# zwyang6/ExCEL

Measured on AMD Instinct MI355X. Metric: images/sec (CAM+PAR refine, 448x448), higher is better.
Workload: dtype bf16x3 (fp32 as bf16 hi+lo, fp32 accumulate)

## Files before the change

excel_amd/_lib.py:

```python
import ctypes as C
import os

_HERE = os.path.dirname(os.path.abspath(__file__))
LIB_PATH = os.path.join(_HERE, "csrc", "libexcel_hip.so")

c_f = C.c_void_p
c_i = C.c_int
c_ll = C.c_longlong
c_sz = C.c_size_t


class VitConfig(C.Structure):
    _fields_ = [("width", c_i), ("layers", c_i), ("heads", c_i), ("patch", c_i), ("out_dim", c_i),
                ("n_surgery", c_i), ("pos_grid", c_i)]


class VitBlockWeights(C.Structure):
    _fields_ = [(n, C.c_void_p) for n in (
        "ln1_w", "ln1_b", "in_proj_w", "in_proj_b", "out_proj_w", "out_proj_b",
        "ln2_w", "ln2_b", "fc1_w", "fc1_b", "fc2_w", "fc2_b")]


class VitWeights(C.Structure):
    _fields_ = [(n, C.c_void_p) for n in (
        "conv1_w", "class_emb", "pos_emb", "ln_pre_w", "ln_pre_b", "ln_post_w", "ln_post_b", "proj")] + \
        [("blocks", C.POINTER(VitBlockWeights))]


class DecoderConfig(C.Structure):
    _fields_ = [(n, c_i) for n in ("vit_layers", "vit_width", "embed", "dec_layers", "heads", "num_classes")]


class FuseLayerWeights(C.Structure):
    _fields_ = [(n, C.c_void_p) for n in ("proj_w", "proj_b", "proj2_w", "proj2_b")]


class DecoderBlockWeights(C.Structure):
    _fields_ = VitBlockWeights._fields_


class DecoderWeights(C.Structure):
    _fields_ = [("fuse", C.POINTER(FuseLayerWeights)), ("fuse_w", C.c_void_p), ("fuse_b", C.c_void_p),
                ("blocks", C.POINTER(DecoderBlockWeights)), ("pred_w", C.c_void_p), ("pred_b", C.c_void_p)]


class TextConfig(C.Structure):
    _fields_ = [(n, c_i) for n in ("vocab_size", "context_length", "width", "layers", "heads", "embed_dim")]


class TextWeights(C.Structure):
    _fields_ = [(n, C.c_void_p) for n in ("token_embedding", "positional_embedding", "ln_final_w", "ln_final_b", "text_projection")] + \
        [("blocks", C.POINTER(DecoderBlockWeights))]


class RaggedInfo(C.Structure):
    _fields_ = [("B", C.c_int32), ("total_tiles", C.c_int32), ("total_pix", C.c_int64), ("total_label_pix", C.c_int64),
                ("max_plane_pix", C.c_int64), ("table_ints", C.c_int64)]


class AugParams(C.Structure):
    _fields_ = [("ratio", C.c_double), ("flip", C.c_int32), ("h_pad", C.c_int32), ("w_pad", C.c_int32),
                ("cand_h", C.c_int32 * 10), ("cand_w", C.c_int32 * 10)]


class TrainAugInfo(C.Structure):
    _fields_ = [("B", C.c_int32), ("S", C.c_int32), ("max_h", C.c_int32), ("max_w2", C.c_int32), ("table_ints", C.c_int64),
                ("workspace_bytes", C.c_int64), ("total_label_pix", C.c_int64)]


SIGNATURES = {
    "excel_last_error": (C.c_char_p, []),
    "excel_abi_version": (c_i, []),
    "excel_build_id": (C.c_char_p, []),
    "excel_gemm_f32": (c_i, [c_f, c_f, c_f, c_f, c_f, c_i, c_i, c_i, c_i, c_i, c_i, c_i, c_i, c_i, c_i,
                             c_ll, c_ll, c_ll, c_ll, c_f]),
    "excel_split_bf16": (c_i, [c_f, c_f, c_ll, c_i, c_f]),
    "excel_gemm_bf16x3": (c_i, [c_f, c_f, c_f, c_f, c_f, c_i, c_i, c_i, c_i, c_i, c_f]),
    "excel_split_f16": (c_i, [c_f, c_f, c_ll, c_i, c_f]),
    "excel_gemm_f16x3": (c_i, [c_f, c_f, c_f, c_f, c_f, c_i, c_i, c_i, c_i, c_i, c_f]),
    "excel_pack_f16": (c_i, [c_f, c_f, c_ll, c_i, c_f, c_f]),
    "excel_gemm_f16x2": (c_i, [c_f, c_f, c_f, c_f, c_f, c_f, c_i, c_i, c_i, c_i, c_i, c_f]),
    "excel_gemm_plan": (c_i, [c_i, c_i, c_i, c_i, c_i, c_i, c_i, c_i, c_i, C.POINTER(C.c_int32)]),
    "excel_attn_plan": (c_i, [c_i, c_i, c_i, c_i, c_i, c_i, C.POINTER(C.c_int32)]),
    "excel_layernorm": (c_i, [c_f, c_f, c_f, c_f, c_i, c_i, C.c_float, c_f]),
    "excel_vit_create": (c_i, [C.POINTER(VitConfig), C.POINTER(VitWeights), C.POINTER(C.c_void_p)]),
    "excel_vit_destroy": (None, [C.c_void_p]),
    "excel_vit_workspace_bytes": (c_sz, [C.c_void_p, c_i, c_i]),
    "excel_vit_set_gemm_mode": (c_i, [C.c_void_p, c_i]),
    "excel_vit_get_gemm_mode": (c_i, [C.c_void_p]),
    "excel_vit_weights_fp16_exact": (c_i, [C.c_void_p]),
    "excel_vit_forward": (c_i, [C.c_void_p, c_f, c_i, c_i, c_f, c_sz, c_f, c_f, c_f, c_i, c_f, c_i, c_f, c_f]),
    "excel_vit_forward_ex": (c_i, [C.c_void_p, c_f, c_i, c_i, c_f, c_sz, c_f, c_f, c_f, c_i, c_f, c_i, c_f, c_f, c_i, c_f]),
    "excel_feature_affinity_workspace_bytes": (c_sz, [c_i, c_i, c_i]),
    "excel_feature_affinity": (c_i, [c_f, c_i, c_i, c_i, C.c_float, C.c_float, c_i, c_f, c_f, c_f]),
    "excel_feature_affinity_grouped_workspace_bytes": (c_sz, [c_i, c_i, c_i, c_i]),
    "excel_feature_affinity_grouped": (c_i, [c_f, c_i, c_i, c_i, c_i, c_i, C.c_float, C.c_float, c_i, c_f, c_f, c_f]),
    "excel_attn_select_workspace_bytes": (c_sz, [c_i, c_i]),
    "excel_attn_select_mean": (c_i, [c_f, c_i, c_i, c_i, c_i, c_i, c_f, c_f, c_f, c_f]),
    "excel_decoder_create": (c_i, [C.POINTER(DecoderConfig), C.POINTER(DecoderWeights), C.POINTER(C.c_void_p)]),
    "excel_decoder_destroy": (None, [C.c_void_p]),
    "excel_decoder_workspace_bytes": (c_sz, [C.c_void_p, c_i, c_i]),
    "excel_decoder_forward": (c_i, [C.c_void_p, c_f, c_i, c_i, c_f, c_sz, c_f, c_f, c_f]),
    "excel_text_create": (c_i, [C.POINTER(TextConfig), C.POINTER(TextWeights), C.POINTER(C.c_void_p)]),
    "excel_text_destroy": (None, [C.c_void_p]),
    "excel_text_workspace_bytes": (c_sz, [C.c_void_p, c_i]),
    "excel_text_encode": (c_i, [C.c_void_p, c_f, c_i, c_f, c_f, c_sz, c_f]),
    "excel_prompt_ensemble": (c_i, [c_f, c_i, c_i, c_f, c_f]),
    "excel_decoder_train_workspace_bytes": (c_sz, [C.c_void_p, c_i, c_i]),
    "excel_decoder_forward_train": (c_i, [C.c_void_p, c_f, c_i, c_i, c_f, c_sz, c_f, c_f, C.c_float, C.c_uint, c_f]),
    "excel_decoder_train_attn_fts": (c_i, [C.c_void_p, c_i, c_i, c_f, c_sz, c_f, c_f]),
    "excel_decoder_backward": (c_i, [C.c_void_p, c_f, c_i, c_i, c_f, c_sz, c_f, c_f, C.POINTER(DecoderWeights), C.c_float, C.c_uint, c_f]),
    "excel_adamw_step": (c_i, [c_f, c_f, c_f, c_f, c_ll, C.c_float, C.c_float, C.c_float, C.c_float, C.c_float, c_i, c_f]),
    "excel_train_losses_workspace_bytes": (c_sz, [c_i, c_i, c_i, c_i]),
    "excel_train_losses": (c_i, [c_f, c_f, c_f, c_f, c_i, c_i, c_i, c_i, c_i, c_i, c_i, c_i, C.c_float, C.c_float, c_f, c_f, c_f, c_f, c_f]),
    "excel_lam_to_label": (c_i, [c_f, c_f, c_f, c_i, c_i, c_i, c_i, C.c_float, C.c_float, C.c_float, c_i, c_i, c_f, c_f, c_f]),
    "excel_normalize_img_u8": (c_i, [c_f, c_i, c_i, c_i, C.POINTER(C.c_double), C.POINTER(C.c_double), c_f, c_f]),
    "excel_denormalize_img": (c_i, [c_f, c_i, c_i, c_i, C.POINTER(C.c_float), C.POINTER(C.c_float), c_f, c_f, c_f]),
    "excel_seg_scale_accumulate": (c_i, [c_f, c_f, c_i, c_i, c_i, c_i, c_i, c_i, c_i, c_i, C.c_float, c_f]),
    "excel_cam_workspace_bytes": (c_sz, [c_i, c_i, c_i]),
    "excel_patch_text_cam_workspace_bytes": (c_sz, [c_i, c_i, c_i, c_i]),
    "excel_patch_text_cam": (c_i, [c_f, c_f, c_i, c_i, c_i, c_i, c_i, C.c_float, c_i, c_f, c_f, c_f, c_f, c_f]),
    "excel_clip_feature_surgery": (c_i, [c_f, c_f, c_i, c_i, c_i, c_i, c_i, C.c_float, c_f, c_f, c_f, c_f]),
    "excel_dcrf_workspace_bytes": (c_sz, [c_i, c_i, c_i]),
    "excel_dcrf_inference": (c_i, [c_f, c_f, c_i, c_i, c_i, c_i, c_i, C.c_float, C.c_float, C.c_float, C.c_float, C.c_float, c_f, c_f, c_f]),
    "excel_dcrf_ragged_workspace_bytes": (c_i, [c_ll, c_i, C.POINTER(c_sz)]),
    "excel_dcrf_inference_ragged": (c_i, [c_f, c_f, c_i, c_f, C.POINTER(RaggedInfo), c_i, c_i, C.c_float, C.c_float, C.c_float, C.c_float, C.c_float,
                                          c_f, c_f, c_f, c_f]),
    "excel_dcrf_lam_ragged_workspace_bytes": (c_i, [C.POINTER(C.c_int32), C.POINTER(C.c_int32), c_i, C.POINTER(c_sz)]),
    "excel_dcrf_lam_ragged": (c_i, [c_f, c_f, c_f, C.POINTER(C.c_int32), c_f, c_f, C.POINTER(RaggedInfo), c_i, c_i, c_i, C.c_float, C.c_float,
                                    C.c_float, C.c_float, C.c_float, c_f, c_f, c_f, c_f]),
    "excel_attn_layer_mean": (c_i, [c_f, c_i, c_i, c_i, c_i, c_i, c_f, c_f]),
    "excel_trans_mat_workspace_bytes": (c_sz, [c_i, c_i]),
    "excel_compute_trans_mat": (c_i, [c_f, c_i, c_i, c_f, c_f, c_f]),
    "excel_cls_compact": (c_i, [c_f, c_i, c_i, c_i, c_f, c_f, c_f, c_f]),
    "excel_scoremap_box_mask": (c_i, [c_f, c_f, c_f, c_i, c_i, c_i, c_i, C.c_double, c_f, c_f, c_f]),
    "excel_refine_workspace_bytes": (c_sz, [c_i, c_i, c_i]),
    "excel_refine_cams_with_aff": (c_i, [c_f, c_f, c_f, c_f, c_i, c_i, c_i, c_i, C.c_double, c_f, c_f, c_f]),
    "excel_cam_upsample_bkg": (c_i, [c_f, c_f, c_i, c_i, c_i, c_i, c_i, c_f, c_f, c_i, c_f]),
    "excel_par_workspace_bytes": (c_sz, [c_i, c_i, c_i, c_i, c_i]),
    "excel_par_forward": (c_i, [c_f, c_i, c_i, c_f, c_f, c_i, c_i, c_i, c_i, C.POINTER(C.c_int32), c_i, c_i,
                                C.c_float, C.c_float, c_f, c_f, c_i, c_f]),
    "excel_ragged_plan": (c_i, [C.POINTER(C.c_int32), c_i, C.POINTER(RaggedInfo), C.POINTER(C.c_int32)]),
    "excel_normalize_resize_u8_ragged": (c_i, [c_f, c_f, c_i, c_i, C.POINTER(C.c_double), C.POINTER(C.c_double), c_f, c_f]),
    "excel_normalize_resize_u8_ragged_mirror": (c_i, [c_f, c_f, c_i, c_i, C.POINTER(C.c_double), C.POINTER(C.c_double), c_f, c_f]),
    "excel_cam_upsample_bkg_ragged": (c_i, [c_f, c_f, c_f, C.POINTER(RaggedInfo), c_i, c_i, c_f, c_f, c_i, c_f]),
    "excel_par_ragged_workspace_bytes": (c_sz, [c_ll, c_i]),
    "excel_par_forward_ragged": (c_i, [c_f, c_i, c_i, c_f, c_f, c_f, C.POINTER(RaggedInfo), c_i, C.POINTER(C.c_int32), c_i, c_i,
                                       C.c_float, C.c_float, c_f, c_f, c_f]),
    "excel_argmax_label_ragged": (c_i, [c_f, c_f, c_f, c_f, C.POINTER(RaggedInfo), c_i, c_i, c_f, c_f]),
    "excel_seg_msc_fuse_ragged": (c_i, [C.POINTER(C.c_void_p), C.POINTER(C.c_int32), C.POINTER(C.c_int32), c_i, c_i, c_f, C.POINTER(RaggedInfo),
                                        c_f, c_f, c_f]),
    "excel_seg_resize_argmax_ragged": (c_i, [c_f, c_f, C.POINTER(RaggedInfo), c_f, C.POINTER(RaggedInfo), c_i, c_f, c_f]),
    "excel_seg_resize_argmax_uniform": (c_i, [c_f, c_i, c_i, c_i, c_i, c_f, C.POINTER(RaggedInfo), c_f, c_f]),
    "excel_seg_softmax_resize": (c_i, [c_f, c_i, c_i, c_i, c_i, c_i, c_f, c_f]),
    "excel_seg_softmax_resize_ragged": (c_i, [c_f, c_f, C.POINTER(RaggedInfo), c_f, C.POINTER(RaggedInfo), c_i, c_f, c_f]),
    "excel_cam_overlay_ragged": (c_i, [c_f, c_f, c_i, c_f, c_f, c_f, C.POINTER(RaggedInfo), c_i, c_f, c_f, c_f]),
    "excel_cam_overlay": (c_i, [c_f, c_f, c_i, c_i, c_i, c_i, c_f, c_f, c_f]),
    "excel_train_panels_plan": (c_i, [c_i, c_i, c_i, c_i, c_i, C.POINTER(C.c_int64)]),
    "excel_train_panels": (c_i, [c_f, c_f, c_f, c_f, c_f, c_f, c_f, c_i, c_i, c_i, c_i, c_i, c_i, c_i, C.POINTER(C.c_float), C.POINTER(C.c_float),
                                 c_f, c_f, c_f, c_sz, c_f]),
    "excel_png_labels_bound_bytes": (c_sz, [c_i, c_i]),
    "excel_png_labels_workspace_bytes": (c_sz, [c_i, c_i]),
    "excel_png_encode_labels_ragged": (c_i, [c_f, c_f, C.POINTER(RaggedInfo), C.POINTER(C.c_int32), c_f, c_f, c_sz, c_f, c_f, c_sz, c_f]),
    "excel_jpeg_rgb_arena_bytes": (c_sz, [C.POINTER(C.c_int32), c_i]),
    "excel_jpeg_rgb_workspace_bytes": (c_sz, [C.POINTER(C.c_int32), c_i]),
    "excel_jpeg_encode_rgb_ragged": (c_i, [c_f, C.POINTER(C.c_int64), C.POINTER(C.c_int32), c_i, c_i, c_f, c_sz, c_f, c_f, c_sz, c_f]),
    "excel_train_aug_plan": (c_i, [C.POINTER(C.c_int32), C.POINTER(AugParams), c_i, c_i, C.POINTER(TrainAugInfo), C.POINTER(C.c_int32)]),
    "excel_train_augment_workspace_bytes": (c_sz, [C.POINTER(TrainAugInfo)]),
    "excel_train_augment": (c_i, [c_f, c_f, c_f, C.POINTER(TrainAugInfo), C.POINTER(C.c_double), C.POINTER(C.c_double), c_f, c_f, c_f, c_f, c_f]),
    "excel_train_augment_image": (c_i, [c_f, c_f, C.POINTER(TrainAugInfo), C.POINTER(C.c_double), C.POINTER(C.c_double), c_f, c_f, c_f, c_f]),
    "excel_argmax_label": (c_i, [c_f, c_f, c_f, c_i, c_i, c_i, c_ll, c_f, c_f, c_f]),
    "excel_confusion_accumulate": (c_i, [c_f, c_f, c_ll, c_i, c_f, c_f]),
    "excel_nonfinite_count": (c_i, [c_f, c_i, c_ll, c_f, c_i, c_f]),
    "excel_confusion_accumulate_masked": (c_i, [c_f, c_f, c_i, c_ll, c_f, C.POINTER(RaggedInfo), c_f, c_i, c_f, c_f]),
    "excel_attr_aggregate": (c_i, [c_f, c_f, c_i, c_i, c_i, c_i, C.c_double, c_f, c_f]),
    "excel_bilinear_resize": (c_i, [c_f, c_f, c_ll, c_i, c_i, c_i, c_i, c_i, c_f]),
    "excel_pos_embed_resize": (c_i, [c_f, c_i, c_i, c_i, c_f, c_f]),
    "excel_flip_max_normalize": (c_i, [c_f, c_f, c_i, c_i, c_i, c_f]),
    "excel_lam_scale_accumulate": (c_i, [c_f, c_f, c_i, c_i, c_i, c_i, c_i, c_i, c_f]),
    "excel_plane_minmax_normalize": (c_i, [c_f, c_ll, c_ll, c_f]),
    "excel_lam_tta_fuse": (c_i, [C.POINTER(C.c_void_p), C.POINTER(C.c_int32), c_i, c_i, c_i, c_i, c_i, c_f, c_f]),
    "excel_prof_enable": (c_i, [c_i]),
    "excel_prof_set_mask": (c_i, [C.c_ulonglong]),
    "excel_prof_set_sampling": (c_i, [c_i]),
    "excel_prof_num_categories": (c_i, []),
    "excel_prof_category_name": (C.c_char_p, [c_i]),
    "excel_prof_collect": (c_i, [C.POINTER(C.c_double), C.POINTER(C.c_longlong), C.POINTER(C.c_double)]),
}

_lib = None


def lib():
    global _lib
    if _lib is not None:
        return _lib
    import torch
    if not os.path.exists(LIB_PATH):
        raise RuntimeError(
            f"excel_amd: {LIB_PATH} is missing - the HIP extension is the only compute path. "
            "Build it with `python -m excel_amd.build` (or __graft_entry__.build()).")
    handle = C.CDLL(LIB_PATH)
    for name, (res, args) in SIGNATURES.items():
        fn = getattr(handle, name)
        fn.restype = res
        fn.argtypes = args
    _lib = handle
    return _lib


def build_id():
    return lib().excel_build_id().decode()


def check(rc, what):
    if rc != 0:
        msg = lib().excel_last_error()
        raise RuntimeError(f"{what} failed (rc={rc}): {msg.decode() if msg else '?'}")
```

excel_amd/csrc/abi.hip:

```cpp
#include "../../include/excel_hip.h"
#include "common.h"
#include "excel_internal.h"

#include <stdarg.h>
#include <map>
#include <vector>

static thread_local char g_err[512] = "";

void excel_set_error(const char* fmt, ...) {
    va_list ap;
    va_start(ap, fmt);
    vsnprintf(g_err, sizeof(g_err), fmt, ap);
    va_end(ap);
}

extern "C" const char* excel_last_error(void) { return g_err; }
extern "C" int excel_abi_version(void) { return 4; }
#ifndef EXCEL_BUILD_ID
#define EXCEL_BUILD_ID "unstamped"
#endif
extern "C" const char* excel_build_id(void) { return EXCEL_BUILD_ID; }

bool g_excel_prof_on = false;
// ... 580 lines not shown
    EXCEL_CHECK_ARG((P % 4) == 0, "compute_trans_mat: P must be a multiple of 4 (P=%d)", P);
    char* base = (char*)workspace;
    const size_t mat = align_up((size_t)B * P * P * sizeof(float), 256);
    float* T = (float*)base;
    float* Tsym = (float*)(base + mat);
    float* cs = (float*)(base + 2 * mat);
    TRY(excel_launch_trans_mat_sym(w_aff, T, Tsym, cs, B, P, ST(stream)));
    GemmArgs ga = gemm_args(Tsym, Tsym, trans_out, nullptr, nullptr, P, P, P, P, P, P, 0, GEMM_ACT_NONE);
    ga.sA = ga.sB = ga.sC = (long long)P * P;
    return excel_launch_gemm(ga, true, B, ST(stream));
}

extern "C" int excel_cls_compact(const float* onehot, int B, int F, int Smax, int32_t* cls_idx, int32_t* ncls, int32_t* nchan,
                                 void* stream) {
    EXCEL_CHECK_ARG(onehot && cls_idx && ncls && Smax >= 1, "cls_compact: bad argument");
    return excel_launch_cls_compact(onehot, B, F, Smax, cls_idx, ncls, nchan, ST(stream));
}

extern "C" int excel_scoremap_box_mask(const float* attr, const int32_t* cls_idx, const int32_t* ncls, int B, int g, int F, int Smax,
                                       double caa_thre, float* v_out, uint8_t* mask_out, void* stream) {
    EXCEL_CHECK_ARG(attr && cls_idx && ncls && v_out, "scoremap_box_mask: null argument");
    return excel_launch_bbox_mask(attr, cls_idx, ncls, B, g, F, Smax, caa_thre, v_out, mask_out, ST(stream));
}

extern "C" size_t excel_refine_workspace_bytes(int B, int P, int Smax) {
    return 2 * align_up((size_t)B * P * P * sizeof(float), 256) + align_up((size_t)B * P * sizeof(float), 256) +
           2 * align_up((size_t)B * Smax * P * sizeof(float), 256);
}

extern "C" int excel_refine_cams_with_aff(const float* attr, const float* w_aff, const int32_t* cls_idx, const int32_t* ncls, int B,
                                          int g, int F, int Smax, double caa_thre, float* refined, void* workspace, void* stream) {
    EXCEL_CHECK_ARG(attr && w_aff && cls_idx && ncls && refined && workspace, "refine_cams_with_aff: null argument");
    const int P = g * g;
    char* base = (char*)workspace;
    const size_t mat = align_up((size_t)B * P * P * sizeof(float), 256);
    const size_t vec = align_up((size_t)B * Smax * P * sizeof(float), 256);
    float* T = (float*)base;
    float* Tsym = (float*)(base + mat);
    float* cs = (float*)(base + 2 * mat);
    float* v = (float*)(base + 2 * mat + align_up((size_t)B * P * sizeof(float), 256));
    float* u = (float*)((char*)v + vec);
    hipStream_t st = ST(stream);
    TRY(excel_launch_trans_mat_sym(w_aff, T, Tsym, cs, B, P, st));
    TRY(excel_launch_bbox_mask(attr, cls_idx, ncls, B, g, F, Smax, caa_thre, v, nullptr, st));
    TRY(excel_launch_matvec(Tsym, v, ncls, u, B, P, Smax, st));
    TRY(excel_launch_matvec(Tsym, u, ncls, refined, B, P, Smax, st));
    return EXCEL_OK;
}

extern "C" int excel_cam_upsample_bkg(const float* refined, const int32_t* ncls, int B, int g, int Smax, int H, int W, float* cams,
                                      void* workspace, int flags, void* stream) {
    EXCEL_CHECK_ARG(refined && ncls && cams && workspace, "cam_upsample_bkg: null argument");
    return excel_launch_cam_upsample_bkg(refined, ncls, (float*)workspace, cams, B, g, Smax, H, W, (flags & EXCEL_CAMS_ZERO_UNUSED) ? 1 : 0, ST(stream));
}

extern "C" int excel_ragged_plan(const int32_t* hw, int B, excel_ragged_info* info, int32_t* table) {
    EXCEL_CHECK_ARG(hw && info && B >= 1, "ragged_plan: bad argument");
    long long pix = 0, lab = 0, tiles = 0, max_plane = 0;
    for (int b = 0; b < B; ++b) {
        const long long H = hw[2 * b], W = hw[2 * b + 1];
        EXCEL_CHECK_ARG(H >= 1 && W >= 1, "ragged_plan: image %d has size %lld x %lld", b, H, W);
        const long long Wp = (W + 3) / 4 * 4, plane = H * Wp, nt = ((W + 63) / 64) * ((H + 15) / 16);
        if (table) {
            int32_t* rec = table + EXCEL_RAG_REC * b;
            rec[0] = (int32_t)H; rec[1] = (int32_t)W; rec[2] = (int32_t)pix; rec[3] = (int32_t)tiles; rec[4] = (int32_t)lab; rec[5] = rec[6] = rec[7] = 0;
            for (long long t = 0; t < nt; ++t) table[EXCEL_RAG_REC * (B + 1) + tiles + t] = b;
        }
        pix += plane; lab += H * W; tiles += nt;
        if (plane > max_plane) max_plane = plane;
        EXCEL_CHECK_ARG(pix < (1LL << 31) && 3 * lab < (1LL << 31) && tiles < (1LL << 31), "ragged_plan: batch too large for 32-bit offsets");
    }
    if (table) {
        int32_t* rec = table + EXCEL_RAG_REC * B;
        rec[0] = rec[1] = 0; rec[2] = (int32_t)pix; rec[3] = (int32_t)tiles; rec[4] = (int32_t)lab; rec[5] = rec[6] = rec[7] = 0;
    }
    info->B = B; info->total_tiles = (int32_t)tiles; info->total_pix = pix; info->total_label_pix = lab; info->max_plane_pix = max_plane;
    info->table_ints = EXCEL_RAG_REC * (long long)(B + 1) + tiles;
    return EXCEL_OK;
}

static TileGeo ragged_geo(const int32_t* table, int B) {
    TileGeo g;
    g.tab = table; g.B = B; g.H = g.W = 0;
    return g;
}
static TileGeo uniform_geo(int B, int H, int W) {
    TileGeo g;
    g.tab = nullptr; g.B = B; g.H = H; g.W = W;
    return g;
}

extern "C" int excel_normalize_resize_u8_ragged(const uint8_t* hwc, const int32_t* table, int B, int S, const double* mean3, const double* std3,
                                                float* out, void* stream) {
    EXCEL_CHECK_ARG(hwc && table && out && mean3 && std3 && B > 0 && S > 0, "normalize_resize_u8_ragged: bad argument");
    return excel_launch_normalize_resize_u8_ragged(hwc, out, ragged_geo(table, B), S, mean3, std3, ST(stream));
}

extern "C" int excel_normalize_resize_u8_ragged_mirror(const uint8_t* hwc, const int32_t* table, int B, int S, const double* mean3,
                                                       const double* std3, float* out, void* stream) {
    EXCEL_CHECK_ARG(hwc && table && out && mean3 && std3 && B > 0 && S > 0, "normalize_resize_u8_ragged_mirror: bad argument");
    return excel_launch_normalize_resize_u8_ragged_mirror(hwc, out, ragged_geo(table, B), S, mean3, std3, ST(stream));
}

extern "C" int excel_cam_upsample_bkg_ragged(const float* refined, const int32_t* ncls, const int32_t* table, const excel_ragged_info* info, int g,
                                             int Smax, float* cams, void* workspace, int flags, void* stream) {
    EXCEL_CHECK_ARG(refined && ncls && table && info && cams && workspace, "cam_upsample_bkg_ragged: null argument");
    EXCEL_CHECK_ARG((((uintptr_t)cams) & 15) == 0, "cam_upsample_bkg_ragged: cams must be 16-byte aligned");
    return excel_launch_cam_upsample_bkg_ragged(refined, ncls, (float*)workspace, cams, g, Smax, ragged_geo(table, info->B), info->total_tiles,
                                                (flags & EXCEL_CAMS_ZERO_UNUSED) ? 1 : 0, ST(stream));
}

int excel_aug_plan(const int32_t* hw, const excel_aug_params* prm, int B, int S, excel_train_aug_info* info, int32_t* table);
int excel_launch_train_augment(const unsigned char* hwc, const unsigned char* labels, const int* table, const excel_train_aug_info& info,
                               const double* mean, const double* stdv, float* img, unsigned char* label, int* img_box, void* workspace,
                               hipStream_t st);
int excel_launch_train_augment_image(const unsigned char* hwc, const int* table, const excel_train_aug_info& info, const double* mean,
                                     const double* stdv, float* img, int* img_box, void* workspace, hipStream_t st);
extern "C" int excel_train_aug_plan(const int32_t* hw, const excel_aug_params* params, int B, int S, excel_train_aug_info* info, int32_t* table) {
    return excel_aug_plan(hw, params, B, S, info, table);
}

extern "C" size_t excel_train_augment_workspace_bytes(const excel_train_aug_info* info) {
    return info ? (size_t)info->workspace_bytes : 0;
}

extern "C" int excel_train_augment(const uint8_t* hwc, const uint8_t* labels, const int32_t* table, const excel_train_aug_info* info,
                                   const double* mean3, const double* std3, float* img, uint8_t* label, int32_t* img_box, void* workspace,
                                   void* stream) {
    EXCEL_CHECK_ARG(hwc && labels && table && info && mean3 && std3 && img && label && img_box && workspace, "train_augment: null argument");
    EXCEL_CHECK_ARG(info->B >= 1 && info->S >= 1 && info->max_h >= 1 && info->max_w2 >= 1 && info->workspace_bytes > 0,
                    "train_augment: info was not filled by excel_train_aug_plan");
    return excel_launch_train_augment(hwc, labels, table, *info, mean3, std3, img, label, img_box, workspace, ST(stream));
}

extern "C" int excel_train_augment_image(const uint8_t* hwc, const int32_t* table, const excel_train_aug_info* info, const double* mean3,
                                         const double* std3, float* img, int32_t* img_box, void* workspace, void* stream) {
    EXCEL_CHECK_ARG(hwc && table && info && mean3 && std3 && img && img_box && workspace, "train_augment_image: null argument");
    EXCEL_CHECK_ARG(info->B >= 1 && info->S >= 1 && info->max_h >= 1 && info->max_w2 >= 1 && info->workspace_bytes > 0,
                    "train_augment_image: info was not filled by excel_train_aug_plan");
    return excel_launch_train_augment_image(hwc, table, *info, mean3, std3, img, img_box, workspace, ST(stream));
}

extern "C" size_t excel_par_workspace_bytes(int B, int Cmax, int H, int W, int ndil) {
    const size_t hw = (size_t)H * W;
    return align_up((size_t)B * 8 * ndil * hw * sizeof(float), 256) + align_up((size_t)B * Cmax * hw * sizeof(float), 256) +
           align_up((size_t)B * 3 * hw * sizeof(float), 256);
}

template <class Step>
static int par_jacobi(const float* masks, float* out, float* pp, int n_iter, Step step) {
    const float* cur = masks;
    for (int it = 0; it < n_iter; ++it) {
        float* dst = (((n_iter - 1 - it) & 1) == 0) ? out : pp;
        TRY(step(cur, dst));
        cur = dst;
    }
    return EXCEL_OK;
}

extern "C" int excel_par_forward(const float* imgs, int h, int w, const float* masks, const int32_t* nchan, int B, int Cmax, int H,
                                 int W, const int32_t* dilations, int ndil, int n_iter, float w1, float w2, float* out,
                                 void* workspace, int flags, void* stream) {
    EXCEL_CHECK_ARG(imgs && masks && out && workspace && dilations, "par_forward: null argument");
    EXCEL_CHECK_ARG(n_iter >= 0 && ndil >= 1 && ndil <= 8, "par_forward: bad n_iter/ndil");
    EXCEL_CHECK_ARG(B > 0 && Cmax > 0 && H > 0 && W > 0 && h > 0 && w > 0, "par_forward: bad shape");
    const size_t hw = (size_t)H * W;
    char* base = (char*)workspace;
    float* aff = (float*)base;
    float* pp = (float*)(base + align_up((size_t)B * 8 * ndil * hw * sizeof(float), 256));
    float* guide = (float*)((char*)pp + align_up((size_t)B * Cmax * hw * sizeof(float), 256));
    hipStream_t st = ST(stream);
    const float* gimg = imgs;
    if (h != H || w != W) {
        TRY(excel_launch_bilinear_ac(imgs, guide, B * 3, h, w, H, W, st));
        gimg = guide;
    }
    const TileGeo geo = uniform_geo(B, H, W);
    const bool recompute = !(flags & EXCEL_PAR_STREAM_AFFINITIES) && n_iter > 0 && (W % 4) == 0 && (((uintptr_t)pp & 15) == 0) &&
                           excel_par_guide_supported(gimg, aff, masks, out, Cmax, (long long)hw, W, dilations, ndil);
    TRY(excel_launch_par_affinity(gimg, aff, geo, 0, dilations, ndil, w1, w2, st, recompute ? 1 : 0));
    if (n_iter == 0) {
        hipMemcpyAsync(out, masks, sizeof(float) * (size_t)B * Cmax * hw, hipMemcpyDeviceToDevice, st);
        return EXCEL_OK;
    }
    if (recompute)
        return par_jacobi(masks, out, pp, n_iter, [&](const float* cur, float* dst) {
            return excel_launch_par_iterate_guide(gimg, aff, cur, dst, nchan, Cmax, geo, 0, dilations, ndil, w1, w2, st);
        });
    return par_jacobi(masks, out, pp, n_iter, [&](const float* cur, float* dst) {
        return excel_launch_par_iterate(aff, cur, dst, nchan, B, Cmax, H, W, dilations, ndil, st);
    });
}

extern "C" size_t excel_par_ragged_workspace_bytes(long long total_pix, int Cmax) {
    return align_up((size_t)5 * total_pix * sizeof(float), 256) + align_up((size_t)Cmax * total_pix * sizeof(float), 256) +
           align_up((size_t)3 * total_pix * sizeof(float), 256);
}

extern "C" int excel_par_forward_ragged(const float* imgs, int h, int w, const float* masks, const int32_t* nchan, const int32_t* table,
                                        const excel_ragged_info* info, int Cmax, const int32_t* dilations, int ndil, int n_iter, float w1,
                                        float w2, float* out, void* workspace, void* stream) {
    EXCEL_CHECK_ARG(imgs && masks && out && workspace && dilations && table && info, "par_forward_ragged: null argument");
    EXCEL_CHECK_ARG(n_iter >= 1 && Cmax > 0 && h > 0 && w > 0 && info->B > 0, "par_forward_ragged: bad n_iter / shape");
    const size_t tp = (size_t)info->total_pix;
    char* base = (char*)workspace;
    float* stats = (float*)base;
    float* pp = (float*)(base + align_up(5 * tp * sizeof(float), 256));
    float* guide = (float*)((char*)pp + align_up((size_t)Cmax * tp * sizeof(float), 256));
    hipStream_t st = ST(stream);
    const TileGeo geo = ragged_geo(table, info->B);
    EXCEL_CHECK_ARG(excel_par_guide_supported(guide, stats, masks, out, Cmax, info->max_plane_pix, 4, dilations, ndil) && (((uintptr_t)pp & 15) == 0),
                    "par_forward_ragged: needs dilations [1,2,4,8,12,24], 16-byte aligned buffers and max(Cmax,5) * H * Wp * 4 < 2^31 per image "
                    "(Wp = W rounded up to 4)");
    TRY(excel_launch_bilinear_ac_ragged(imgs, guide, h, w, geo, info->total_tiles, st));
    TRY(excel_launch_par_affinity(guide, stats, geo, info->total_tiles, dilations, ndil, w1, w2, st, 1));
    return par_jacobi(masks, out, pp, n_iter, [&](const float* cur, float* dst) {
        return excel_launch_par_iterate_guide(guide, stats, cur, dst, nchan, Cmax, geo, info->total_tiles, dilations, ndil, w1, w2, st);
    });
}

extern "C" int excel_argmax_label_ragged(const float* cams, const int32_t* nchan, const int32_t* cls_idx, const int32_t* table,
                                         const excel_ragged_info* info, int Smax, int Cmax, uint8_t* labels_u8, void* stream) {
    EXCEL_CHECK_ARG(cams && table && info && labels_u8, "argmax_label_ragged: null argument");
    return excel_launch_argmax_label_ragged(cams, nchan, cls_idx, Smax, Cmax, ragged_geo(table, info->B), info->total_tiles, labels_u8, ST(stream));
}

extern "C" int excel_argmax_label(const float* cams, const int32_t* nchan, const int32_t* cls_idx, int B, int Smax, int Cmax,
                                  long long HW, uint8_t* labels_u8, int64_t* labels_i64, void* stream) {
    EXCEL_CHECK_ARG(cams && (labels_u8 || labels_i64), "argmax_label: null argument");
    return excel_launch_argmax_label(cams, nchan, cls_idx, B, Smax, Cmax, HW, labels_u8, (long long*)labels_i64, ST(stream));
}

extern "C" int excel_confusion_accumulate(const uint8_t* gt, const uint8_t* pred, long long n, int num_classes, int64_t* hist,
                                          void* stream) {
    EXCEL_CHECK_ARG(gt && pred && hist && n >= 0, "confusion_accumulate: null argument");
    if (n == 0) return EXCEL_OK;
    return excel_launch_confusion(gt, pred, n, num_classes, (unsigned long long*)hist, ST(stream));
}

extern "C" int excel_attr_aggregate(const float* text, const float* bank, int F, int T, int C, int K, double topK, float* out,
                                    void* stream) {
    EXCEL_CHECK_ARG(text && bank && out, "attr_aggregate: null argument");
    const int drop = (int)((1.0 - topK) * (double)K);
    return excel_launch_attr_aggregate(text, bank, F, T, C, K, drop, out, ST(stream));
}

extern "C" int excel_bilinear_resize(const float* in, float* out, long long planes, int h, int w, int H, int W, int align_corners,
                                     void* stream) {
    EXCEL_CHECK_ARG(in && out && planes > 0 && h > 0 && w > 0 && H > 0 && W > 0, "bilinear_resize: bad argument");
    return excel_launch_bilinear_resize(in, out, planes, h, w, H, W, align_corners, ST(stream));
}

extern "C" int excel_pos_embed_resize(const float* pos, int side, int g, int D, float* out, void* stream) {
    EXCEL_CHECK_ARG(pos && out && side > 0 && g > 0, "pos_embed_resize: bad argument");
    hipLaunchKernelGGL(pos_resize_kernel, dim3((unsigned)cdivl((long long)(g * g + 1) * D, 256)), dim3(256), 0, ST(stream), pos, out, side, g, D);
    EXCEL_CHECK_LAUNCH("pos_resize");
    return EXCEL_OK;
}

extern "C" int excel_flip_max_normalize(const float* attr, float* out, int B, int g, int F, void* stream) {
    EXCEL_CHECK_ARG(attr && out, "flip_max_normalize: null argument");
    return excel_launch_flip_max_normalize(attr, out, B, g, F, ST(stream));
}

extern "C" int excel_lam_scale_accumulate(const float* maps, float* acc, int B, int g, int F, int H, int W, int init, void* stream) {
    EXCEL_CHECK_ARG(maps && acc && B > 0 && g > 0, "lam_scale_accumulate: bad argument");
    return excel_launch_lam_scale_accumulate(maps, acc, B, g, F, H, W, init, ST(stream));
}

extern "C" int excel_plane_minmax_normalize(float* lam, long long planes, long long HW, void* stream) {
    EXCEL_CHECK_ARG(lam && planes > 0 && HW > 0, "plane_minmax_normalize: bad argument");
    return excel_launch_plane_minmax_normalize(lam, planes, HW, ST(stream));
}
```

excel_amd/csrc/excel_internal.h:

```cpp
#pragma once
#include <hip/hip_runtime.h>

enum { GEMM_ACT_NONE = 0, GEMM_ACT_QUICKGELU = 1, GEMM_ACT_RELU = 2 };
enum { GEMM_OUT_PLAIN = 0, GEMM_OUT_QKV_HEADMAJOR = 1, GEMM_OUT_SPLIT_BF16 = 2 };

struct GemmArgs {
    const float* A;
    const float* B;
    float* C;
    const float* bias;
    const float* res;
    int M, N, K;
    int Kld;
    int lda, ldb, ldc, ldr;
    long long sA, sB, sC, sR, sBias;
    int zdiv;
    long long sA2, sB2, sC2;
    int act;
    int out_mode;
    int tokN, heads, hd;
    float alpha;
};


struct GemmBfArgs {
    const unsigned short* A;
    const unsigned short* B;
    float* C;
    unsigned short* Cs;
    const float* bias;
    const float* res;
    int M, N, K;
    int lda, ldb, ldc, ldr;
    int act, out_mode;
    int tokN, heads, hd;
    unsigned short* qkv_split;
    int dbg;
    int batch;
    long long sA, sB, sC, sCs;
    int mix_tall, mix_short;
    int mix_first;
    int w_lo_zero;
    const unsigned short* Bh;
    int ldbh;
};

struct GemmShape {
    int M, N, K, lda, ldb, ldc, ldr, hd, out_mode, has_residual, batch;
    int f16;
    int w_lo_zero;
    int half_ok;
};
enum { GEMM_8WAVE = 0, GEMM_8WAVE_MIXED = 1, GEMM_W4 = 2, GEMM_W4_MIX = 3 };
struct GemmPlan {
    int kernel;
    int tile;
    int nt_m;
    int x2;
    int tall, shrt, second;
    int grid_x, grid_y, block;
};
constexpr int GEMM_W4_BN = 256;
GemmPlan gemm_plan(const GemmShape& s, int n_cu);
enum { ATTN_STRIP = 0, ATTN_TWOPASS_SPLIT = 1, ATTN_TWOPASS_F32 = 2 };
constexpr int ATTN_STRIP_MAX_TILES = 40;
struct AttnPlan {
    int path;
    int ntiles;
    int ntw, nw, nw_full;
    int rp_ntypes;
    int rp_grid[3];
    int grid[3], block;
    int split_c;
};
AttnPlan attn_plan(int B, int H, int N, int gemm_mode, int surgery, int want_w);
inline bool gemm_half_ok(bool aligned, int N, int K, int ldbh) {
    return aligned && ldbh >= K && (ldbh & 7) == 0 && (long long)N * ldbh * 2 < 0x7fffffffLL;
}

int excel_launch_gemm(const GemmArgs& p, bool b_kmajor, int batch, hipStream_t stream);
int excel_launch_attn_rowpass_f32(const float* qkvh, float* out, float* stats, int B, int H, int N, int hd, float scale,
                                  const AttnPlan& plan, hipStream_t st, int flash_nq);
int excel_launch_attn_accum_f32(const float* qkvh, const float* stats, float* a_sum, float* w_aff, float* attn_out, int B, int H,
                                int N, int NP, int hd, float scale, int surgery, float w_scale, float aff_scale, int aff_init,
                                const AttnPlan& plan, hipStream_t st, const float* ex_attn);

int excel_launch_trans_mat_sym(const float* W, float* T, float* Tsym, float* cs, int B, int P, hipStream_t st);
int excel_launch_cls_compact(const float* onehot, int B, int F, int Smax, int* cls_idx, int* ncls, int* nchan, hipStream_t st);
int excel_launch_bbox_mask(const float* attr, const int* cls_idx, const int* ncls, int B, int g, int F, int Smax, double thre,
                           float* v_out, unsigned char* mask_out, hipStream_t st);
int excel_launch_matvec(const float* T, const float* v, const int* ncls, float* u, int B, int P, int Smax, hipStream_t st);
int excel_launch_cam_upsample_bkg(const float* r, const int* ncls, float* rn, float* cams, int B, int g, int Smax, int H, int W,
                                  int zero_unused, hipStream_t st);
struct TileGeo;
int excel_launch_par_affinity(const float* img, float* aff, const TileGeo& geo, int total_tiles, const int* dil, int ndil, float w1, float w2,
                              hipStream_t st, int compact = 0);
int excel_par_guide_supported(const void* guide, const void* stats, const void* in, const void* out, int Cmax, long long max_plane, int Wp,
                              const int* dil, int ndil);
int excel_launch_par_iterate_guide(const float* guide, const float* stats, const float* in, float* out, const int* nchan, int Cmax,
                                   const TileGeo& geo, int total_tiles, const int* dil, int ndil, float w1, float w2, hipStream_t st);
int excel_launch_par_iterate(const float* aff, const float* in, float* out, const int* nchan, int B, int Cmax, int H, int W,
                             const int* dil, int ndil, hipStream_t st);
int excel_launch_bilinear_ac_ragged(const float* in, float* out, int h, int w, const TileGeo& geo, int total_tiles, hipStream_t st);
int excel_launch_argmax_label_ragged(const float* cams, const int* nchan, const int* cls_idx, int Smax, int Cmax, const TileGeo& geo,
                                     int total_tiles, unsigned char* lab8, hipStream_t st);
int excel_launch_cam_upsample_bkg_ragged(const float* r, const int* ncls, float* rn, float* cams, int g, int Smax, const TileGeo& geo,
                                         int total_tiles, int zero_unused, hipStream_t st);
int excel_launch_normalize_resize_u8_ragged(const unsigned char* hwc, float* out, const TileGeo& geo, int S, const double* mean, const double* stdv,
                                            hipStream_t st);
int excel_launch_normalize_resize_u8_ragged_mirror(const unsigned char* hwc, float* out, const TileGeo& geo, int S, const double* mean,
                                                   const double* stdv, hipStream_t st);
int excel_launch_bilinear_ac(const float* in, float* out, int planes, int h, int w, int H, int W, hipStream_t st);
int excel_launch_argmax_label(const float* cams, const int* nchan, const int* cls_idx, int B, int Smax, int Cmax, long long HW,
                              unsigned char* lab8, long long* lab64, hipStream_t st);
int excel_launch_confusion(const unsigned char* gt, const unsigned char* pred, long long n, int nc, unsigned long long* hist,
                           hipStream_t st);
int excel_launch_attr_aggregate(const float* text, const float* bank, int F, int T, int C, int K, int drop, float* out,
                                hipStream_t st);
int excel_launch_bilinear_resize(const float* in, float* out, long long planes, int h, int w, int H, int W, int align_corners,
                                 hipStream_t st);
int excel_launch_flip_max_normalize(const float* attr, float* out, int B, int g, int F, hipStream_t st);
int excel_launch_lam_scale_accumulate(const float* maps, float* acc, int B, int g, int F, int H, int W, int init, hipStream_t st);
int excel_launch_plane_minmax_normalize(float* lam, long long planes, long long HW, hipStream_t st);
int excel_launch_seg_scale_accumulate(const float* segs, float* acc, int B, int nc, int h, int w, int H, int W, int flip_mean, int init,
                                      float scale, hipStream_t st);
int excel_launch_denormalize(const float* img, unsigned char* out8, float* outf, int B, long long HW, const float* mean, const float* stdv,
                             hipStream_t st);
int excel_launch_normalize_u8(const unsigned char* hwc, float* out, int B, long long HW, const double* mean, const double* stdv, hipStream_t st);
int excel_launch_lam_to_label(const float* cam, const float* cls, const int* box, int B, int F, int H, int W, float bkg, float high, float low,
                              int ignore_mid, int ignore, float* valid, unsigned char* lab, hipStream_t st);
size_t excel_train_losses_ws_bytes(int B, int nc, int H, int W);
int excel_launch_train_losses(const float* seg, const float* attn_pred, const unsigned char* pseudo, const unsigned char* aff_labels, int B, int nc,
                              int g_h, int g_w, int H, int W, int radius, int ignore, float w_seg, float w_diver, float* losses, float* d_seg,
                              float* d_attn_pred, void* ws, hipStream_t st);
size_t excel_feature_affinity_ws_bytes(int B, int C, int P);
int excel_launch_feature_affinity(const float* feats, int B, int C, int P, float beta, float gamma, int mode, float* out, void* ws,
                                  hipStream_t st);
size_t excel_feature_affinity_grouped_ws_bytes(int B, int C, int P, int group);
int excel_launch_feature_affinity_grouped(const float* feats, int B, int C, int P, int group, int member_stride, float beta, float gamma,
                                          int mode, float* out, void* ws, hipStream_t st);
size_t excel_attn_select_ws_bytes(int B, int n_layers);
int excel_launch_attn_select_mean(const float* attn, int Lw, int B, int N, int first_layer, int n_layers, const float* seg_attn,
                                  float* out, void* ws, hipStream_t st);

namespace excel_bf16 {
#include "excel_split_api.inc"
}
namespace excel_f16 {
#include "excel_split_api.inc"
}
#ifdef EXCEL_SPLIT_F16
#define EXCEL_SPLIT_NS excel_f16
#else
#define EXCEL_SPLIT_NS excel_bf16
#endif
using namespace excel_bf16;

struct BilinearTap { int y0, y1, x0, x1; float ly, lx; };
__device__ __forceinline__ BilinearTap bilinear_tap(int x, int y, int h, int w, int H, int W, int align_corners) {
    float fy, fx;
    if (align_corners) {
        fy = ((H > 1) ? (float)(h - 1) / (float)(H - 1) : 0.f) * (float)y;
        fx = ((W > 1) ? (float)(w - 1) / (float)(W - 1) : 0.f) * (float)x;
    } else {
        fy = fmaxf(__fsub_rn(__fmul_rn((float)h / (float)H, (float)y + 0.5f), 0.5f), 0.f);
        fx = fmaxf(__fsub_rn(__fmul_rn((float)w / (float)W, (float)x + 0.5f), 0.5f), 0.f);
    }
    BilinearTap t;
    t.y0 = min((int)fy, h - 1); t.x0 = min((int)fx, w - 1);
    t.y1 = min(t.y0 + 1, h - 1); t.x1 = min(t.x0 + 1, w - 1);
    t.ly = fy - (float)t.y0; t.lx = fx - (float)t.x0;
    return t;
}
__device__ __forceinline__ float bilinear_blend(const BilinearTap& t, float p00, float p01, float p10, float p11) {
    const float top = fmaf(t.lx, p01, __fmul_rn(1.f - t.lx, p00));
    const float bot = fmaf(t.lx, p11, __fmul_rn(1.f - t.lx, p10));
    return fmaf(t.ly, bot, __fmul_rn(1.f - t.ly, top));
}
```

excel_amd/csrc/par.hip:

```cpp
#include <stdlib.h>
#include <type_traits>
#include <utility>
#include "common.h"
#include "excel_internal.h"

struct ParDil {
    int d[8];
    float pos_sm[64];
};

#define PAR_LOG2E_3 0.48089834696298783f
#ifndef PAR_MASK_DEPTH
#define PAR_MASK_DEPTH 1
#endif

template <int ND, bool RAGGED>
__global__ __launch_bounds__(256) void par_affinity_kernel(const float* __restrict__ img, float* __restrict__ aff, ParDil dl, TileGeo geo,
                                                           float w1, int COMPACT) {
    constexpr int NT = 8 * ND;
    int b, H, W, Wp, x, y;
    long long base, HW;
    const int wave = __builtin_amdgcn_readfirstlane((int)(threadIdx.x >> 6));
    if (RAGGED) {
        const Tile t = tile_of<true>(geo);
        b = t.b; H = t.H; W = t.W; Wp = t.Wp; base = t.base; HW = t.HW;
        x = t.x0 + (threadIdx.x & 63);
        y = t.y0 + blockIdx.y * 4 + wave;
    } else {
        b = blockIdx.z; H = geo.H; W = geo.W; Wp = geo.W; HW = (long long)H * W; base = (long long)b * HW;
        x = blockIdx.x * 64 + (threadIdx.x & 63);
        y = blockIdx.y * 4 + wave;
    }
    if (y >= H) return;
    const bool in_x = x < W;
    const int xc = min(x, W - 1);
    int xo[ND][2];
#pragma unroll
    for (int di = 0; di < ND; ++di) { xo[di][0] = max(xc - dl.d[di], 0); xo[di][1] = min(xc + dl.d[di], W - 1); }
    float acc[NT];
#pragma unroll
    for (int t = 0; t < NT; ++t) acc[t] = 0.f;
    const long long pix = (long long)y * Wp + x;
    float* st = aff + 5 * base + pix;
#pragma unroll 1
    for (int c = 0; c < 3; ++c) {
        const float* ch = img + 3 * base + c * HW;
        const float* row0 = ch + (long long)y * Wp;
        const float ctr = row0[xc];
        float nb[NT];
        float sum = 0.f;
#pragma unroll
        for (int di = 0; di < ND; ++di) {
            const int d = dl.d[di];
            const float* rup = ch + (long long)max(y - d, 0) * Wp;
            const float* rdn = ch + (long long)min(y + d, H - 1) * Wp;
            nb[di * 8 + 0] = rup[xo[di][0]]; nb[di * 8 + 1] = rup[xc]; nb[di * 8 + 2] = rup[xo[di][1]];
            nb[di * 8 + 3] = row0[xo[di][0]]; nb[di * 8 + 4] = row0[xo[di][1]];
            nb[di * 8 + 5] = rdn[xo[di][0]]; nb[di * 8 + 6] = rdn[xc]; nb[di * 8 + 7] = rdn[xo[di][1]];
#pragma unroll
            for (int k = 0; k < 8; ++k) sum += nb[di * 8 + k];
        }
        const float mean = sum / (float)NT;
        float var = 0.f;
#pragma unroll
        for (int t = 0; t < NT; ++t) { const float dv = nb[t] - mean; var = fmaf(dv, dv, var); }
        const float den = sqrtf(var / (float)(NT - 1)) + 1e-8f;
        const float k = 1.f / (den * w1);
        const float k2 = __fmul_rn(k * k, PAR_LOG2E_3);
        if (COMPACT && in_x) st[c * HW] = k2;
#pragma unroll
        for (int t = 0; t < NT; ++t) {
            const float dv = nb[t] - ctr;
            acc[t] = fmaf(-(dv * dv), k2, acc[t]);
        }
    }
    float m = -INFINITY;
#pragma unroll
    for (int t = 0; t < NT; ++t) m = fmaxf(m, acc[t]);
    float s = 0.f;
#pragma unroll
    for (int t = 0; t < NT; ++t) { acc[t] = __builtin_amdgcn_exp2f(__fsub_rn(acc[t], m)); s += acc[t]; }
    const float inv_s = 1.f / s;
    if (!in_x) return;
    if (COMPACT) {
        st[3 * HW] = m;
        st[4 * HW] = inv_s;
        return;
    }
    float* out = aff + (long long)NT * base + pix;
#pragma unroll
    for (int t = 0; t < NT; ++t) out[(long long)t * HW] = fmaf(acc[t], inv_s, dl.pos_sm[t]);
}

#define PAR_CCH 8
__global__ __launch_bounds__(256) void par_iterate_stream_kernel(const float* __restrict__ aff, const float* __restrict__ in,
                                                                 float* __restrict__ out, const int* __restrict__ nchan, ParDil dl,
                                                                 int ndil, int Cmax, int H, int W) {
    const int b = blockIdx.z;
    const int x = blockIdx.x * 64 + (threadIdx.x & 63);
    const int y = blockIdx.y * 4 + (threadIdx.x >> 6);
    if (x >= W || y >= H) return;
    const int nch = nchan ? min(nchan[b], Cmax) : Cmax;
    const long long HW = (long long)H * W;
    const float* a = aff + (long long)b * 8 * ndil * HW + (long long)y * W + x;
    const float* ib = in + (long long)b * Cmax * HW;
    float* ob = out + (long long)b * Cmax * HW + (long long)y * W + x;
    const int dils[8] = {dl.d[0], dl.d[1], dl.d[2], dl.d[3], dl.d[4], dl.d[5], dl.d[6], dl.d[7]};
    for (int c0 = 0; c0 < nch; c0 += PAR_CCH) {
        float acc[PAR_CCH];
#pragma unroll
        for (int c = 0; c < PAR_CCH; ++c) acc[c] = 0.f;
#pragma unroll 1
        for (int di = 0; di < ndil; ++di) {
            int d = dils[0];
#pragma unroll
            for (int q = 1; q < 8; ++q) d = (di == q) ? dils[q] : d;
#pragma unroll
            for (int k = 0; k < 8; ++k) {
                const int dy = (k < 3) ? -1 : (k < 5 ? 0 : 1);
                const int dx = (k == 0 || k == 3 || k == 5) ? -1 : ((k == 1 || k == 6) ? 0 : 1);
                const int yy = min(max(y + dy * d, 0), H - 1);
                const int xx = min(max(x + dx * d, 0), W - 1);
                const float wgt = a[(long long)(di * 8 + k) * HW];
                const float* src = ib + (long long)yy * W + xx;
#pragma unroll
                for (int c = 0; c < PAR_CCH; ++c)
                    if (c0 + c < nch) acc[c] = fmaf(src[(long long)(c0 + c) * HW], wgt, acc[c]);
            }
        }
#pragma unroll
        for (int c = 0; c < PAR_CCH; ++c)
            if (c0 + c < nch) ob[(long long)(c0 + c) * HW] = acc[c];
    }
}

#define PG_TP 128
template <int DI> struct ParD { static constexpr int v = DI == 0 ? 1 : DI == 1 ? 2 : DI == 2 ? 4 : DI == 3 ? 8 : DI == 4 ? 12 : 24; };
template <class F, int... I> __device__ __forceinline__ void static_for_seq(F&& f, std::integer_sequence<int, I...>) { (f(std::integral_constant<int, I>{}), ...); }
template <int N, class F> __device__ __forceinline__ void static_for(F&& f) { static_for_seq(f, std::make_integer_sequence<int, N>{}); }
template <int OFF> __device__ __forceinline__ f32x2 lds_read8_imm(unsigned base) {
    static_assert(OFF >= 0 && OFF < 65536 && (OFF & 7) == 0, "ds_read_b64 immediate offset");
    f32x2 v;
    asm volatile("ds_read_b64 %0, %1 offset:%2" : "=v"(v) : "v"(base), "n"(OFF) : "memory");
    return v;
}

template <bool RAGGED>
__global__ __launch_bounds__(512, 4) void par_iterate_guide_kernel(const float* __restrict__ guide, const float* __restrict__ stats,
                                                                    const float* __restrict__ in, float* __restrict__ out,
                                                                    const int* __restrict__ nchan, ParDil dl, int Cmax, TileGeo geo, int dbg) {
    constexpr int ND = 6, HALO = 24, TR = 16 + 2 * HALO, TP = PG_TP, NG = 3 * ND;
    __shared__ __attribute__((aligned(1024))) float tile[2 * TR * TP];
    Tile tg;
    if (RAGGED) {
        tg = tile_of_ragged(geo, (EXCEL_DBG(dbg) & 32) ? (int)blockIdx.x : xcd_remap(blockIdx.x, gridDim.x));
    } else {
        tg = tile_of<false>(geo);
        if (!(EXCEL_DBG(dbg) & 32)) {
            const int nx = gridDim.x, ny = gridDim.y, per = nx * ny;
            const int id = xcd_remap(blockIdx.x + nx * (blockIdx.y + ny * blockIdx.z), per * (int)gridDim.z);
            const int bb = id / per, rem = id - bb * per, tyy = rem / nx;
            tg.b = bb; tg.x0 = (rem - tyy * nx) * 64; tg.y0 = tyy * 16; tg.base = (long long)bb * tg.HW; tg.lab = tg.base;
        }
    }
    const int b = tg.b, x0 = tg.x0, y0 = tg.y0, H = tg.H, W = tg.W, Wp = tg.Wp;
    const long long HW = tg.HW;
    const int tid = threadIdx.x, lane = tid & 63, tx = tid & 31, ty = tid >> 5;
    const int wave = __builtin_amdgcn_readfirstlane(tid >> 6);
    const int px = x0 + 2 * tx, py = y0 + ty;
    const int nch = nchan ? min(nchan[b], Cmax) : Cmax;
    const long long pix = (long long)min(py, H - 1) * Wp + min(px, Wp - 2);
    const float* st_b = stats + 5 * tg.base + pix;

    typedef __attribute__((address_space(3))) unsigned char* lds_bptr;
    const __amdgpu_buffer_rsrc_t rs_g = __builtin_amdgcn_make_buffer_rsrc((void*)(guide + 3 * tg.base), 0, (int)(3 * HW * 4), 0x00020000);
    const __amdgpu_buffer_rsrc_t rs_m = __builtin_amdgcn_make_buffer_rsrc((void*)(in + (long long)Cmax * tg.base), 0, (int)((long long)Cmax * HW * 4), 0x00020000);
    const int xoffA = min(max(x0 - HALO + lane, 0), W - 1) * 4, xoffB = min(max(x0 - HALO + 64 + lane, 0), W - 1) * 4;
    const unsigned tile_b = lds_addr(tile);
    constexpr int RPW = TR / 8;
#ifdef PAR_ALL_INTERIOR
    const bool interior = true;
#else
    const bool interior = x0 - HALO >= 0 && x0 + 64 + HALO <= W;
#endif
    const int x4off = min(x0 - HALO + 4 * (lane & 31), Wp - 4) * 4;
    auto stage = [&](int p, int buf) {
        const bool is_g = p < 3;
        const int plane_off = (is_g ? p : p - 3) * (int)(HW * 4);
        unsigned dst = tile_b + (buf * TR + wave * RPW) * (TP * 4);
        asm volatile("" : "+s"(dst));
        if ((EXCEL_DBG(dbg) & 8) && (wave == 0 || wave == 7)) return;
        if (interior) {
            int half = lane >> 5;
            asm volatile("" : "+v"(half));
#pragma unroll
            for (int j = 0; j < RPW / 2; ++j) {
                const int gy = min(max(y0 - HALO + wave * RPW + 2 * j + half, 0), H - 1);
                const int voff = gy * Wp * 4 + x4off;
                if (is_g) __builtin_amdgcn_raw_ptr_buffer_load_lds(rs_g, (lds_bptr)(unsigned long long)(dst + j * (2 * TP * 4)), 16, voff, plane_off, 0, 0);
                else __builtin_amdgcn_raw_ptr_buffer_load_lds(rs_m, (lds_bptr)(unsigned long long)(dst + j * (2 * TP * 4)), 16, voff, plane_off, 0, 0);
            }
            return;
        }
#pragma unroll 4
        for (int rr = 0; rr < RPW; ++rr) {
            const int gy = min(max(y0 - HALO + wave * RPW + rr, 0), H - 1);
            const int soff = plane_off + gy * Wp * 4;
            if (is_g) {
                __builtin_amdgcn_raw_ptr_buffer_load_lds(rs_g, (lds_bptr)(unsigned long long)(dst + rr * (TP * 4)), 4, xoffA, soff, 0, 0);
                __builtin_amdgcn_raw_ptr_buffer_load_lds(rs_g, (lds_bptr)(unsigned long long)(dst + rr * (TP * 4) + 256), 4, xoffB, soff, 0, 0);
            } else {
                __builtin_amdgcn_raw_ptr_buffer_load_lds(rs_m, (lds_bptr)(unsigned long long)(dst + rr * (TP * 4)), 4, xoffA, soff, 0, 0);
                __builtin_amdgcn_raw_ptr_buffer_load_lds(rs_m, (lds_bptr)(unsigned long long)(dst + rr * (TP * 4) + 256), 4, xoffB, soff, 0, 0);
            }
        }
    };

    f32x2 wall[ND][8];
#pragma unroll
    for (int di = 0; di < ND; ++di)
#pragma unroll
        for (int k = 0; k < 8; ++k) wall[di][k] = f32x2{0.f, 0.f};

    const unsigned org = tile_b + (ty * TP + 2 * tx) * 4;
    auto taps = [&](auto depth_c, int buf, auto&& fn, auto&& pin) {
        constexpr int DEPTH = decltype(depth_c)::value, NS = DEPTH + 1;
        unsigned base = org + buf * (TR * TP * 4);
        asm volatile("" : "+v"(base));
        f32x2 sl[NS][3];
        auto nreads = [](int G) constexpr { return (G % 3 != 1 || G / 3 == 0) ? 3 : 2; };
        auto issue = [&](auto g) {
            constexpr int G = decltype(g)::value, r = G % 3, d = ParD<G / 3>::v, s = G % NS;
            constexpr int row = (HALO + (r - 1) * d) * TP * 4, cl = (d == 1) ? HALO - 2 : HALO - d, cr = (d == 1) ? HALO + 2 : HALO + d;
            sl[s][0] = lds_read8_imm<row + cl * 4>(base);
            if constexpr (r != 1 || d == 1) sl[s][1] = lds_read8_imm<row + HALO * 4>(base);
            sl[s][2] = lds_read8_imm<row + cr * 4>(base);
        };
        static_for<DEPTH>([&](auto g) { issue(g); });
        static_for<NG>([&](auto g) {
            constexpr int G = decltype(g)::value, di = G / 3, r = G % 3, d = ParD<di>::v, s = G % NS;
            constexpr bool mid = (r != 1 || d == 1);
            if constexpr (G + DEPTH < NG) issue(std::integral_constant<int, G + DEPTH>{});
            constexpr int last = (G + DEPTH < NG) ? G + DEPTH : NG - 1;
            constexpr int nxt = [&]() constexpr { int n = 0; for (int q = G + 1; q <= last; ++q) n += nreads(q); return n; }();
            static_assert(nxt <= 15, "lgkmcnt is a 4-bit counter");
            if constexpr (mid) asm volatile("s_waitcnt lgkmcnt(%3)" : "+v"(sl[s][0]), "+v"(sl[s][1]), "+v"(sl[s][2]) : "n"(nxt) : "memory");
            else asm volatile("s_waitcnt lgkmcnt(%2)" : "+v"(sl[s][0]), "+v"(sl[s][2]) : "n"(nxt) : "memory");
            constexpr int k0 = (r == 0) ? 0 : (r == 1 ? 3 : 5);
            const f32x2 L = sl[s][0], R = sl[s][2];
            if constexpr (d == 1) {
                const f32x2 M = sl[s][1];
                fn(di, k0, f32x2{L[1], M[0]});
                if constexpr (r != 1) fn(di, k0 + 1, M);
                fn(di, k0 + (r != 1 ? 2 : 1), f32x2{M[1], R[0]});
            } else {
                fn(di, k0, L);
                if constexpr (r != 1) fn(di, k0 + 1, sl[s][1]);
                fn(di, k0 + (r != 1 ? 2 : 1), R);
            }
            pin();
            __builtin_amdgcn_sched_barrier(0);
        });
    };

    auto far_taps = [&](const float* plane) -> f32x2 {
        f32x2 sum = {0.f, 0.f};
        const int yu = max(py - 24, 0), yd = min(py + 24, H - 1), ym = min(py, H - 1);
        const int xl = max(min(px, Wp - 2) - 24, 0), xr = min(min(px, Wp - 2) + 24, Wp - 2), xm = min(px, Wp - 2);
        const int ys[8] = {yu, yu, yu, ym, ym, yd, yd, yd}, xs[8] = {xl, xm, xr, xl, xr, xl, xm, xr};
#pragma unroll
        for (int k = 0; k < 8; ++k) {
            const float2 v = *reinterpret_cast<const float2*>(plane + (long long)ys[k] * Wp + (xs[k] & ~1));
            sum += f32x2{v.x, v.y};
        }
        return sum;
    };
    const int np = 3 + nch;
    auto stat_load = [&](int plane) -> f32x2 { return *reinterpret_cast<const f32x2*>(st_b + (long long)plane * HW); };
    f32x2 st_nxt = stat_load(0), st_nx2 = f32x2{0.f, 0.f};
    __builtin_amdgcn_sched_barrier(0);
    stage(0, 0);
#pragma unroll 1
    for (int p = 0; p < 3; ++p) {
        asm volatile("s_waitcnt vmcnt(0)" : "+v"(st_nxt) :: "memory");
        __builtin_amdgcn_s_barrier();
        const f32x2 nk2 = -st_nxt;
        st_nxt = stat_load(p + 1);
        if (p == 2) st_nx2 = stat_load(4);
        f32x2 ctr;
        asm volatile("ds_read_b64 %0, %1 offset:%2" : "=v"(ctr) : "v"(org + (p & 1) * (TR * TP * 4)), "n"((HALO * TP + HALO) * 4) : "memory");
        __builtin_amdgcn_sched_barrier(0);
        stage(p + 1, (p + 1) & 1);
        asm volatile("s_waitcnt lgkmcnt(0)" : "+v"(ctr) :: "memory");
        if (EXCEL_DBG(dbg) & 1) continue;
        f32x2 nctr = -ctr;
        if (EXCEL_DBG(dbg) & 16) nctr += 1e-30f * far_taps(guide + 3 * tg.base + (long long)p * HW);
        asm volatile("" : "+v"(nctr));
        taps(std::integral_constant<int, 1>{}, p & 1, [&](int di, int k, const f32x2 nb) {
            const f32x2 dv = nb + nctr;
            wall[di][k] = __builtin_elementwise_fma(dv * dv, nk2, wall[di][k]);
        }, [] {});
    }
    if (!(EXCEL_DBG(dbg) & 2)) {
        f32x2 nm2 = -st_nxt;
        asm volatile("" : "+v"(nm2));
        const f32x2 is2 = st_nx2;
#pragma unroll
        for (int di = 0; di < ND; ++di)
#pragma unroll
            for (int k = 0; k < 8; ++k) {
                const f32x2 z = wall[di][k] + nm2;
                const f32x2 e = {__builtin_amdgcn_exp2f(z[0]), __builtin_amdgcn_exp2f(z[1])};
                const float ps = dl.pos_sm[di * 8 + k];
                wall[di][k] = __builtin_elementwise_fma(e, is2, f32x2{ps, ps});
            }
    }
    const bool valid = px < W && py < H;
    float* out_px = out + (long long)Cmax * tg.base + (long long)py * Wp + px;
#ifndef PAR_STORE_WAIT
#define PAR_STORE_WAIT 1
#endif
    const bool wstore = PAR_STORE_WAIT && __builtin_amdgcn_ballot_w64(valid) != 0 && !EXCEL_DBG(dbg);
    for (int p = 3; p < np; ++p) {
        if (p > 3 && wstore) asm volatile("s_waitcnt vmcnt(1)" ::: "memory");
        else asm volatile("s_waitcnt vmcnt(0)" ::: "memory");
        __builtin_amdgcn_s_barrier();
        if (p + 1 < np) stage(p + 1, (p + 1) & 1);
        if (EXCEL_DBG(dbg) & 4) continue;
        f32x2 acc = {0.f, 0.f};
        if (EXCEL_DBG(dbg) & 16) acc = 1e-30f * far_taps(in + (long long)Cmax * tg.base + (long long)(p - 3) * HW);
        taps(std::integral_constant<int, PAR_MASK_DEPTH>{}, p & 1, [&](int di, int k, const f32x2 nb) { acc = __builtin_elementwise_fma(nb, wall[di][k], acc); },
             [&] { asm volatile("" : "+v"(acc)); });
        if (valid) *reinterpret_cast<f32x2*>(out_px + (long long)(p - 3) * HW) = acc;
    }
}

template <bool RAGGED>
__global__ __launch_bounds__(512, 4) void par_stats_tile_kernel(const float* __restrict__ guide, float* __restrict__ stats, TileGeo geo, float w1) {
    constexpr int ND = 6, HALO = 24, TR = 16 + 2 * HALO, TP = PG_TP, NG = 3 * ND, NT = 8 * ND;
    __shared__ __attribute__((aligned(1024))) float tile[2 * TR * TP];
    const Tile tg = tile_of<RAGGED>(geo);
    const int x0 = tg.x0, y0 = tg.y0, H = tg.H, W = tg.W, Wp = tg.Wp;
    const long long HW = tg.HW;
    const int tid = threadIdx.x, lane = tid & 63, tx = tid & 31, ty = tid >> 5;
    const int wave = __builtin_amdgcn_readfirstlane(tid >> 6);
    const int px = x0 + 2 * tx, py = y0 + ty;

    typedef __attribute__((address_space(3))) unsigned char* lds_bptr;
    const __amdgpu_buffer_rsrc_t rs_g = __builtin_amdgcn_make_buffer_rsrc((void*)(guide + 3 * tg.base), 0, (int)(3 * HW * 4), 0x00020000);
    const int xoffA = min(max(x0 - HALO + lane, 0), W - 1) * 4, xoffB = min(max(x0 - HALO + 64 + lane, 0), W - 1) * 4;
    const unsigned tile_b = lds_addr(tile);
    constexpr int RPW = TR / 8;
    const bool interior = x0 - HALO >= 0 && x0 + 64 + HALO <= W;
    const int x4off = min(x0 - HALO + 4 * (lane & 31), Wp - 4) * 4;
    auto stage = [&](int p, int buf) {
        const int plane_off = p * (int)(HW * 4);
        unsigned dst = tile_b + (buf * TR + wave * RPW) * (TP * 4);
        asm volatile("" : "+s"(dst));
        if (interior) {
            int half = lane >> 5;
            asm volatile("" : "+v"(half));
#pragma unroll
            for (int j = 0; j < RPW / 2; ++j) {
                const int gy = min(max(y0 - HALO + wave * RPW + 2 * j + half, 0), H - 1);
                __builtin_amdgcn_raw_ptr_buffer_load_lds(rs_g, (lds_bptr)(unsigned long long)(dst + j * (2 * TP * 4)), 16, gy * Wp * 4 + x4off, plane_off, 0, 0);
            }
            return;
        }
#pragma unroll 4
        for (int rr = 0; rr < RPW; ++rr) {
            const int gy = min(max(y0 - HALO + wave * RPW + rr, 0), H - 1);
            const int soff = plane_off + gy * Wp * 4;
            __builtin_amdgcn_raw_ptr_buffer_load_lds(rs_g, (lds_bptr)(unsigned long long)(dst + rr * (TP * 4)), 4, xoffA, soff, 0, 0);
            __builtin_amdgcn_raw_ptr_buffer_load_lds(rs_g, (lds_bptr)(unsigned long long)(dst + rr * (TP * 4) + 256), 4, xoffB, soff, 0, 0);
        }
    };

    f32x2 acc[ND][8];
#pragma unroll
    for (int di = 0; di < ND; ++di)
#pragma unroll
        for (int k = 0; k < 8; ++k) acc[di][k] = f32x2{0.f, 0.f};

    const unsigned org = tile_b + (ty * TP + 2 * tx) * 4;
    auto taps = [&](int buf, auto&& fn, auto&& pin) {
        unsigned base = org + buf * (TR * TP * 4);
        asm volatile("" : "+v"(base));
        f32x2 sl[2][3];
        auto issue = [&](auto g) {
            constexpr int G = decltype(g)::value, r = G % 3, d = ParD<G / 3>::v, s = G & 1;
            constexpr int row = (HALO + (r - 1) * d) * TP * 4, cl = (d == 1) ? HALO - 2 : HALO - d, cr = (d == 1) ? HALO + 2 : HALO + d;
            sl[s][0] = lds_read8_imm<row + cl * 4>(base);
            if constexpr (r != 1 || d == 1) sl[s][1] = lds_read8_imm<row + HALO * 4>(base);
            sl[s][2] = lds_read8_imm<row + cr * 4>(base);
        };
        issue(std::integral_constant<int, 0>{});
        static_for<NG>([&](auto g) {
            constexpr int G = decltype(g)::value, di = G / 3, r = G % 3, d = ParD<di>::v, s = G & 1;
            constexpr bool mid = (r != 1 || d == 1);
            if constexpr (G + 1 < NG) {
                issue(std::integral_constant<int, G + 1>{});
                constexpr int nxt = ((G + 1) % 3 != 1 || ParD<(G + 1) / 3>::v == 1) ? 3 : 2;
                if constexpr (mid) asm volatile("s_waitcnt lgkmcnt(%3)" : "+v"(sl[s][0]), "+v"(sl[s][1]), "+v"(sl[s][2]) : "n"(nxt) : "memory");
                else asm volatile("s_waitcnt lgkmcnt(%2)" : "+v"(sl[s][0]), "+v"(sl[s][2]) : "n"(nxt) : "memory");
            } else {
                asm volatile("s_waitcnt lgkmcnt(0)" : "+v"(sl[s][0]), "+v"(sl[s][1]), "+v"(sl[s][2])::"memory");
            }
            constexpr int k0 = (r == 0) ? 0 : (r == 1 ? 3 : 5);
            const f32x2 L = sl[s][0], R = sl[s][2];
            if constexpr (d == 1) {
                const f32x2 M = sl[s][1];
                fn(di, k0, f32x2{L[1], M[0]});
                if constexpr (r != 1) fn(di, k0 + 1, M);
                fn(di, k0 + (r != 1 ? 2 : 1), f32x2{M[1], R[0]});
            } else {
                fn(di, k0, L);
                if constexpr (r != 1) fn(di, k0 + 1, sl[s][1]);
                fn(di, k0 + (r != 1 ? 2 : 1), R);
            }
            pin();
            __builtin_amdgcn_sched_barrier(0);
        });
    };

    const bool valid = px < W && py < H;
    float* st_px = stats + 5 * tg.base + (long long)py * Wp + px;
    stage(0, 0);
#pragma unroll 1
    for (int p = 0; p < 3; ++p) {
        asm volatile("s_waitcnt vmcnt(0)" ::: "memory");
        __builtin_amdgcn_s_barrier();
        if (p + 1 < 3) stage(p + 1, (p + 1) & 1);
        f32x2 ctr;
        asm volatile("ds_read_b64 %0, %1 offset:%2\n\ts_waitcnt lgkmcnt(0)" : "=v"(ctr) : "v"(org + (p & 1) * (TR * TP * 4)), "n"((HALO * TP + HALO) * 4) : "memory");
        f32x2 sum = {0.f, 0.f};
        taps(p & 1, [&](int, int, const f32x2 nb) { sum += nb; }, [&] { asm volatile("" : "+v"(sum)); });
        const f32x2 mean = {sum[0] / (float)NT, sum[1] / (float)NT};
        f32x2 nmean = -mean;
        asm volatile("" : "+v"(nmean));
        f32x2 var = {0.f, 0.f};
        taps(p & 1, [&](int, int, const f32x2 nb) { const f32x2 dv = nb + nmean; var = __builtin_elementwise_fma(dv, dv, var); },
             [&] { asm volatile("" : "+v"(var)); });
        f32x2 k2;
#pragma unroll
        for (int q = 0; q < 2; ++q) {
            const float den = sqrtf(var[q] / (float)(NT - 1)) + 1e-8f;
            const float k = 1.f / (den * w1);
            k2[q] = __fmul_rn(k * k, PAR_LOG2E_3);
        }
        if (valid) *reinterpret_cast<f32x2*>(st_px + (long long)p * HW) = k2;
        f32x2 nk2 = -k2, nctr = -ctr;
        asm volatile("" : "+v"(nctr));
        taps(p & 1, [&](int di, int k, const f32x2 nb) {
            const f32x2 dv = nb + nctr;
            acc[di][k] = __builtin_elementwise_fma(dv * dv, nk2, acc[di][k]);
        }, [] {});
    }
    f32x2 m = {-INFINITY, -INFINITY};
#pragma unroll
    for (int di = 0; di < ND; ++di)
#pragma unroll
        for (int k = 0; k < 8; ++k) { m[0] = fmaxf(m[0], acc[di][k][0]); m[1] = fmaxf(m[1], acc[di][k][1]); }
    f32x2 nm = -m;
    asm volatile("" : "+v"(nm));
    f32x2 ssum = {0.f, 0.f};
#pragma unroll
    for (int di = 0; di < ND; ++di)
#pragma unroll
        for (int k = 0; k < 8; ++k) {
            const f32x2 z = acc[di][k] + nm;
            ssum += f32x2{__builtin_amdgcn_exp2f(z[0]), __builtin_amdgcn_exp2f(z[1])};
        }
    if (valid) {
        *reinterpret_cast<f32x2*>(st_px + 3 * HW) = m;
        *reinterpret_cast<f32x2*>(st_px + 4 * HW) = f32x2{1.f / ssum[0], 1.f / ssum[1]};
    }
}

__device__ __forceinline__ float bilinear_ac_px(const float* __restrict__ p, int h, int w, int H, int W, int x, int y) {
    const float sy = (H > 1) ? (float)(h - 1) / (float)(H - 1) : 0.f;
    const float sx = (W > 1) ? (float)(w - 1) / (float)(W - 1) : 0.f;
    const float fy = sy * (float)y, fx = sx * (float)x;
    const int y0 = min((int)fy, h - 1), x0 = min((int)fx, w - 1);
    const int y1 = min(y0 + 1, h - 1), x1 = min(x0 + 1, w - 1);
    const float ly = fy - (float)y0, lx = fx - (float)x0;
    const float top = fmaf(lx, p[y0 * w + x1], __fmul_rn(1.f - lx, p[y0 * w + x0]));
// ... 41 lines not shown
    const int b = blockIdx.y;
    const long long i = (long long)blockIdx.x * 256 + threadIdx.x;
    if (i >= HW) return;
    const int nch = nchan ? min(nchan[b], Cmax) : Cmax;
    const int key = argmax_key(cams + (long long)b * Cmax * HW + i, HW, nch, cls_idx ? cls_idx + (long long)b * Smax : nullptr);
    if (lab8) lab8[(long long)b * HW + i] = (unsigned char)key;
    if (lab64) lab64[(long long)b * HW + i] = key;
}

__global__ __launch_bounds__(256) void argmax_label_ragged_kernel(const float* __restrict__ cams, const int* __restrict__ nchan,
                                                                  const int* __restrict__ cls_idx, int Smax, int Cmax, TileGeo geo,
                                                                  unsigned char* __restrict__ lab8) {
    const Tile t = tile_of<true>(geo);
    const int x = t.x0 + (threadIdx.x & 63);
    if (x >= t.W) return;
    const int nch = nchan ? min(nchan[t.b], Cmax) : Cmax;
    const int* cls_row = cls_idx ? cls_idx + (long long)t.b * Smax : nullptr;
    const float* cb = cams + (long long)Cmax * t.base;
#pragma unroll
    for (int r = 0; r < 4; ++r) {
        const int y = t.y0 + (threadIdx.x >> 6) + 4 * r;
        if (y < t.H) lab8[t.lab + (long long)y * t.W + x] = (unsigned char)argmax_key(cb + (long long)y * t.Wp + x, t.HW, nch, cls_row);
    }
}

#define CONF_MAXBINS 8192
__global__ __launch_bounds__(256) void confusion_kernel(const unsigned char* __restrict__ gt, const unsigned char* __restrict__ pred,
                                                        long long n, int nc, unsigned long long* __restrict__ hist, int head) {
    __shared__ unsigned int lh[CONF_MAXBINS];
    const int bins = nc * nc;
    for (int i = threadIdx.x; i < bins; i += 256) lh[i] = 0;
    __syncthreads();
    if (head > 0 && blockIdx.x == 0 && threadIdx.x < head && threadIdx.x < n) {
        const int g = gt[threadIdx.x], p = pred[threadIdx.x];
        if (g < nc && p < nc) atomicAdd(&lh[g * nc + p], 1u);
    }
    if (head >= 0) {
        gt += head; pred += head; n -= head;
        if (n < 0) n = 0;
    }
    const long long stride = (long long)gridDim.x * 256 * 16;
    for (long long base = ((long long)blockIdx.x * 256 + threadIdx.x) * 16; base < n; base += stride) {
        if (head >= 0 && base + 16 <= n) {
            const uint4 g4 = *reinterpret_cast<const uint4*>(gt + base);
            const uint4 p4 = *reinterpret_cast<const uint4*>(pred + base);
            const unsigned int gw[4] = {g4.x, g4.y, g4.z, g4.w}, pw[4] = {p4.x, p4.y, p4.z, p4.w};
#pragma unroll
            for (int k = 0; k < 16; ++k) {
                const int g = (gw[k >> 2] >> (8 * (k & 3))) & 255, p = (pw[k >> 2] >> (8 * (k & 3))) & 255;
                if (g < nc && p < nc) atomicAdd(&lh[g * nc + p], 1u);
            }
        } else {
            const long long end = (base + 16 < n) ? base + 16 : n;
            for (long long j = base; j < end; ++j) {
                const int g = gt[j], p = pred[j];
                if (g < nc && p < nc) atomicAdd(&lh[g * nc + p], 1u);
            }
        }
    }
    __syncthreads();
    for (int i = threadIdx.x; i < bins; i += 256)
        if (lh[i]) atomicAdd(&hist[i], (unsigned long long)lh[i]);
}

static int make_dil(const int* dil, int ndil, float w1, float w2, ParDil* out) {
    EXCEL_CHECK_ARG(ndil >= 1 && ndil <= 8, "PAR: 1..8 dilations supported (got %d)", ndil);
    const int nt = 8 * ndil;
    double pos[64], mean = 0.0;
    for (int i = 0; i < 8; ++i) out->d[i] = 0;
    for (int i = 0; i < ndil; ++i) {
        EXCEL_CHECK_ARG(dil[i] >= 1, "PAR: dilations must be >= 1 (got %d)", dil[i]);
        out->d[i] = dil[i];
        for (int k = 0; k < 8; ++k) {
            const bool diag = (k == 0 || k == 2 || k == 5 || k == 7);
            pos[i * 8 + k] = (double)(float)((diag ? (float)sqrt(2.0) : 1.f) * (float)dil[i]);
            mean += pos[i * 8 + k];
        }
    }
    mean /= nt;
    double var = 0.0;
    for (int t = 0; t < nt; ++t) var += (pos[t] - mean) * (pos[t] - mean);
    const double sd = (nt > 1) ? sqrt(var / (nt - 1)) : 0.0;
    double z[64], zm = -1e300, zs = 0.0;
    for (int t = 0; t < nt; ++t) {
        const double a = pos[t] / (sd + 1e-8) / (double)w1;
        z[t] = -(a * a);
        if (z[t] > zm) zm = z[t];
    }
    for (int t = 0; t < nt; ++t) { z[t] = exp(z[t] - zm); zs += z[t]; }
    for (int t = 0; t < 64; ++t) out->pos_sm[t] = (t < nt) ? (float)((double)w2 * (z[t] / zs)) : 0.f;
    return EXCEL_OK;
}

#define ND_SWITCH(nd, CALL)                 \
    switch (nd) {                           \
        case 1: CALL(1); break;             \
        case 2: CALL(2); break;             \
        case 3: CALL(3); break;             \
        case 4: CALL(4); break;             \
        case 5: CALL(5); break;             \
        case 6: CALL(6); break;             \
        case 7: CALL(7); break;             \
        default: CALL(8); break;            \
    }

static bool par_dil_ok(const int* dil, int ndil) {
    static const int want[6] = {1, 2, 4, 8, 12, 24};
    if (ndil != 6) return false;
    for (int i = 0; i < 6; ++i)
        if (dil[i] != want[i]) return false;
    return true;
}
int excel_launch_par_affinity(const float* img, float* aff, const TileGeo& geo, int total_tiles, const int* dil, int ndil, float w1, float w2,
                              hipStream_t st, int compact) {
    ProfScope prof__(PROF_PAR_AFFINITY, st);
    ParDil dl;
    int rc = make_dil(dil, ndil, w1, w2, &dl);
    if (rc) return rc;
    const bool tiled = compact && par_dil_ok(dil, ndil) && ((((uintptr_t)img | (uintptr_t)aff) & 15) == 0) &&
                       (geo.tab ? true : (geo.W % 4 == 0 && geo.W >= 8 && 5LL * geo.H * geo.W * 4 < (1LL << 31)));
    if (geo.tab) {
        EXCEL_CHECK_ARG(compact && ndil == 6, "par_affinity: ragged batches use the compact statistics of the 6-dilation kernel");
        if (tiled) hipLaunchKernelGGL((par_stats_tile_kernel<true>), dim3(total_tiles), dim3(512), 0, st, img, aff, geo, w1);
        else hipLaunchKernelGGL((par_affinity_kernel<6, true>), dim3(total_tiles, 4), dim3(256), 0, st, img, aff, dl, geo, w1, 1);
    } else if (tiled) {
        hipLaunchKernelGGL((par_stats_tile_kernel<false>), dim3(cdiv(geo.W, 64), cdiv(geo.H, 16), geo.B), dim3(512), 0, st, img, aff, geo, w1);
    } else {
#define CALL(N) hipLaunchKernelGGL((par_affinity_kernel<N, false>), dim3(cdiv(geo.W, 64), cdiv(geo.H, 4), geo.B), dim3(256), 0, st, img, aff, dl, geo, w1, compact ? 1 : 0)
        ND_SWITCH(ndil, CALL)
#undef CALL
    }
    EXCEL_CHECK_LAUNCH("par_affinity");
    return EXCEL_OK;
}

int excel_launch_par_iterate(const float* aff, const float* in, float* out, const int* nchan, int B, int Cmax, int H, int W,
                             const int* dil, int ndil, hipStream_t st) {
    ProfScope prof__(PROF_PAR_ITERATE, st);
    ParDil dl;
    int rc = make_dil(dil, ndil, 0.3f, 0.01f, &dl);
    if (rc) return rc;
    hipLaunchKernelGGL(par_iterate_stream_kernel, dim3(cdiv(W, 64), cdiv(H, 4), B), dim3(256), 0, st, aff, in, out, nchan, dl, ndil, Cmax, H, W);
    EXCEL_CHECK_LAUNCH("par_iterate");
    return EXCEL_OK;
}

int excel_par_guide_supported(const void* guide, const void* stats, const void* in, const void* out, int Cmax, long long max_plane, int Wp,
                              const int* dil, int ndil) {
    const bool vec = (Wp % 4) == 0 && Wp >= 4 && ((((uintptr_t)guide | (uintptr_t)stats | (uintptr_t)in | (uintptr_t)out) & 15) == 0);
    const long long planes = Cmax > 5 ? Cmax : 5;
    return (vec && par_dil_ok(dil, ndil) && planes * max_plane * 4 < (1LL << 31)) ? 1 : 0;
}

int excel_launch_par_iterate_guide(const float* guide, const float* stats, const float* in, float* out, const int* nchan, int Cmax,
                                   const TileGeo& geo, int total_tiles, const int* dil, int ndil, float w1, float w2, hipStream_t st) {
    EXCEL_CHECK_ARG(par_dil_ok(dil, ndil), "par_iterate_guide: unsupported dilation set");
    ProfScope prof__(PROF_PAR_ITERATE, st);
    ParDil dl;
    int rc = make_dil(dil, ndil, w1, w2, &dl);
    if (rc) return rc;
    int dbg = 0;
#ifdef EXCEL_DEV
    static const int env_dbg = getenv("EXCEL_PAR_DBG") ? atoi(getenv("EXCEL_PAR_DBG")) : 0;
    dbg = env_dbg;
#endif
    if (geo.tab)
        hipLaunchKernelGGL((par_iterate_guide_kernel<true>), dim3(total_tiles), dim3(512), 0, st, guide, stats, in, out, nchan, dl, Cmax, geo, dbg);
    else
        hipLaunchKernelGGL((par_iterate_guide_kernel<false>), dim3(cdiv(geo.W, 64), cdiv(geo.H, 16), geo.B), dim3(512), 0, st, guide, stats,
                           in, out, nchan, dl, Cmax, geo, dbg);
    EXCEL_CHECK_LAUNCH("par_iterate_guide");
    return EXCEL_OK;
}

int excel_launch_bilinear_ac(const float* in, float* out, int planes, int h, int w, int H, int W, hipStream_t st) {
    ProfScope prof__(PROF_OTHER, st);
    const long long n = (long long)planes * H * W;
    hipLaunchKernelGGL(bilinear_ac_kernel, dim3((unsigned)cdivl(n, 256)), dim3(256), 0, st, in, out, planes, h, w, H, W);
    EXCEL_CHECK_LAUNCH("bilinear_ac");
    return EXCEL_OK;
}

int excel_launch_bilinear_ac_ragged(const float* in, float* out, int h, int w, const TileGeo& geo, int total_tiles, hipStream_t st) {
    ProfScope prof__(PROF_OTHER, st);
    hipLaunchKernelGGL(bilinear_ac_ragged_kernel, dim3(total_tiles, 3), dim3(256), 0, st, in, out, h, w, geo);
    EXCEL_CHECK_LAUNCH("bilinear_ac_ragged");
    return EXCEL_OK;
}

int excel_launch_argmax_label(const float* cams, const int* nchan, const int* cls_idx, int B, int Smax, int Cmax, long long HW,
                              unsigned char* lab8, long long* lab64, hipStream_t st) {
    ProfScope prof__(PROF_ARGMAX, st);
    hipLaunchKernelGGL(argmax_label_kernel, dim3((unsigned)cdivl(HW, 256), B), dim3(256), 0, st, cams, nchan, cls_idx, Smax, Cmax, HW, lab8, lab64);
    EXCEL_CHECK_LAUNCH("argmax_label");
    return EXCEL_OK;
}

int excel_launch_argmax_label_ragged(const float* cams, const int* nchan, const int* cls_idx, int Smax, int Cmax, const TileGeo& geo,
                                     int total_tiles, unsigned char* lab8, hipStream_t st) {
    ProfScope prof__(PROF_ARGMAX, st);
    hipLaunchKernelGGL(argmax_label_ragged_kernel, dim3(total_tiles), dim3(256), 0, st, cams, nchan, cls_idx, Smax, Cmax, geo, lab8);
    EXCEL_CHECK_LAUNCH("argmax_label_ragged");
    return EXCEL_OK;
}

int excel_launch_confusion(const unsigned char* gt, const unsigned char* pred, long long n, int nc, unsigned long long* hist,
                           hipStream_t st) {
    ProfScope prof__(PROF_CONFUSION, st);
    EXCEL_CHECK_ARG(nc >= 1 && nc * nc <= CONF_MAXBINS, "confusion: num_classes %d too large", nc);
    const int mg = (int)((16 - ((uintptr_t)gt & 15)) & 15), mp = (int)((16 - ((uintptr_t)pred & 15)) & 15);
    const int head = (mg == mp) ? mg : -1;
    const int blocks = (int)((cdivl(n, 256 * 16) < 2048) ? cdivl(n, 256 * 16) : 2048);
    hipLaunchKernelGGL(confusion_kernel, dim3(blocks > 0 ? blocks : 1), dim3(256), 0, st, gt, pred, n, nc, hist, head);
    EXCEL_CHECK_LAUNCH("confusion");
    return EXCEL_OK;
}
```

excel_amd/ops.py:

```python
import ctypes as C
import os

import torch

from . import _lib
from ._lib import check, lib

PAR_DILATIONS = (1, 2, 4, 8, 12, 24)


def _p(t, dtype=torch.float32):
    if t is None:
        return None
    if not t.is_cuda:
        raise RuntimeError("excel_amd ops need GPU tensors (the HIP library is the only compute path)")
    if t.dtype != dtype:
        raise TypeError(f"expected {dtype}, got {t.dtype}")
    if not t.is_contiguous():
        raise ValueError("tensor must be contiguous")
    return C.c_void_p(t.data_ptr())


def _stream():
    return C.c_void_p(torch.cuda.current_stream().cuda_stream)
# ... 548 lines not shown

def seg_softmax_resize_ragged(planes, src_plan, dst_plan, nc):
    if src_plan.B != dst_plan.B:
        raise ValueError(f"seg_softmax_resize_ragged: plans of {src_plan.B} and {dst_plan.B} images")
    if planes.numel() != nc * src_plan.total_pix:
        raise ValueError(f"seg_softmax_resize_ragged: planes must hold nc * total_pix = {nc * src_plan.total_pix} floats")
    prob = torch.empty((nc * dst_plan.total_label_pix,), dtype=torch.float32, device=planes.device)
    check(lib().excel_seg_softmax_resize_ragged(_p(planes), _p(src_plan.table, torch.int32), C.byref(src_plan.info), _p(dst_plan.table, torch.int32),
                                                C.byref(dst_plan.info), int(nc), _p(prob), _stream()), "excel_seg_softmax_resize_ragged")
    return prob


def clip_feature_surgery(image_features, text_features, num_fg=None, t=2.0, want_full=True):
    image_features = f32c(image_features)
    text_features = f32c(text_features)
    B, N, Cc = image_features.shape
    T = text_features.shape[0]
    dev = image_features.device
    full = torch.empty((B, N, T), dtype=torch.float32, device=dev) if want_full else None
    F_ = T if num_fg is None else num_fg
    sl = torch.empty((B, N - 1, F_), dtype=torch.float32, device=dev) if num_fg is not None else None
    ws = _ws(lib().excel_cam_workspace_bytes(B, N, T), dev)
    check(lib().excel_clip_feature_surgery(_p(image_features), _p(text_features), B, N, Cc, T, F_, float(t), _p(full), _p(sl),
                                           _p(ws, torch.uint8), _stream()), "excel_clip_feature_surgery")
    return full, sl


def patch_text_cam(x_raw, text_features, num_fg=None, t=2.0, want_full=False, want_features=False, mode="bf16x3"):
    x_raw = f32c(x_raw)
    text_features = f32c(text_features)
    B, N, Cc = x_raw.shape
    T = text_features.shape[0]
    dev = x_raw.device
    full = torch.empty((B, N, T), dtype=torch.float32, device=dev) if want_full else None
    F_ = T if num_fg is None else num_fg
    sl = torch.empty((B, N - 1, F_), dtype=torch.float32, device=dev) if num_fg is not None else None
    feats = torch.empty_like(x_raw) if want_features else None
    if full is None and sl is None:
        raise ValueError("patch_text_cam: nothing to compute (want_full=False and num_fg=None)")
    ws = _ws(lib().excel_patch_text_cam_workspace_bytes(B, N, Cc, T), dev)
    check(lib().excel_patch_text_cam(_p(x_raw), _p(text_features), B, N, Cc, T, F_, float(t), GEMM_MODES["f16x3" if mode == "f16x2" else mode], _p(full), _p(sl),
                                     _p(feats), _p(ws, torch.uint8), _stream()), "excel_patch_text_cam")
    return full, sl, feats


def attn_layer_mean(attn, n_layers=6):
    attn = f32c(attn)
    Lw, B, N, _ = attn.shape
    n = min(n_layers, Lw)
    out = torch.empty((B, N - 1, N - 1), dtype=torch.float32, device=attn.device)
    check(lib().excel_attn_layer_mean(_p(attn), Lw, B, N, Lw - n, n, _p(out), _stream()), "excel_attn_layer_mean")
    return out


def attn_select_mean(attn, seg_attn, n_layers=6):
    attn = f32c(attn)
    seg_attn = f32c(seg_attn)
    Lw, B, N, _ = attn.shape
    n = min(n_layers, Lw)
    if tuple(seg_attn.shape) != (B, N - 1, N - 1):
        raise ValueError(f"seg_attn must be [B,P,P] = {(B, N - 1, N - 1)}, got {tuple(seg_attn.shape)}")
    out = torch.empty((B, N - 1, N - 1), dtype=torch.float32, device=attn.device)
    ws = _ws(lib().excel_attn_select_workspace_bytes(B, n), attn.device)
    check(lib().excel_attn_select_mean(_p(attn), Lw, B, N, Lw - n, n, _p(seg_attn), _p(out), _p(ws, torch.uint8), _stream()),
          "excel_attn_select_mean")
    return out


def feature_affinity(feats, mode, beta=1.0, gamma=3.0):
    feats = f32c(feats)
    feats = feats.reshape(feats.shape[0], feats.shape[1], -1)
    B, Cc, P = feats.shape
    out = torch.empty((B, P, P), dtype=torch.float32, device=feats.device)
    ws = _ws(lib().excel_feature_affinity_workspace_bytes(B, Cc, P), feats.device)
    check(lib().excel_feature_affinity(_p(feats), B, Cc, P, float(beta), float(gamma), {"sigmoid": 0, "mask_softmax": 1}[mode],
                                       _p(out), _p(ws, torch.uint8), _stream()), "excel_feature_affinity")
    return out


def feature_affinity_grouped(feats, mode, group, member_stride=1, beta=1.0, gamma=3.0, out=None):
    feats = f32c(feats)
    feats = feats.reshape(feats.shape[0], feats.shape[1], -1)
    B, Cc, P = feats.shape
    out = _out(out, (B, P, P), torch.float32, feats.device)
    ws = _ws(lib().excel_feature_affinity_grouped_workspace_bytes(B, Cc, P, int(group)), feats.device)
    check(lib().excel_feature_affinity_grouped(_p(feats), B, Cc, P, int(group), int(member_stride), float(beta), float(gamma),
                                               {"sigmoid": 0, "mask_softmax": 1}[mode], _p(out), _p(ws, torch.uint8), _stream()),
          "excel_feature_affinity_grouped")
    return out


def compute_trans_mat(w_aff):
    single = w_aff.dim() == 2
    w = f32c(w_aff[None] if single else w_aff)
    B, P, _ = w.shape
    out = torch.empty_like(w)
    ws = _ws(lib().excel_trans_mat_workspace_bytes(B, P), w.device)
    check(lib().excel_compute_trans_mat(_p(w), B, P, _p(out), _p(ws, torch.uint8), _stream()), "excel_compute_trans_mat")
    return out[0] if single else out


def cls_compact(onehot, smax, want_nchan=False):
    onehot = f32c(onehot)
    B, F_ = onehot.shape
    idx = torch.empty((B, smax), dtype=torch.int32, device=onehot.device)
    n = torch.empty((B,), dtype=torch.int32, device=onehot.device)
    nch = torch.empty((B,), dtype=torch.int32, device=onehot.device) if want_nchan else None
    check(lib().excel_cls_compact(_p(onehot), B, F_, smax, _p(idx, torch.int32), _p(n, torch.int32), _p(nch, torch.int32),
                                  _stream()), "excel_cls_compact")
    return (idx, n, nch) if want_nchan else (idx, n)


def scoremap_box_mask(attr, cls_idx, ncls, g, caa_thre=0.79, want_mask=False):
    attr = f32c(attr)
    B, P, F_ = attr.shape
    smax = cls_idx.shape[1]
    v = torch.zeros((B, smax, P), dtype=torch.float32, device=attr.device)
    m = torch.zeros((B, smax, P), dtype=torch.uint8, device=attr.device) if want_mask else None
    check(lib().excel_scoremap_box_mask(_p(attr), _p(cls_idx, torch.int32), _p(ncls, torch.int32), B, g, F_, smax, float(caa_thre),
                                        _p(v), _p(m, torch.uint8), _stream()), "excel_scoremap_box_mask")
    return v, m


def refine_cams_with_aff_batched(attr, w_aff, cls_idx, ncls, g, caa_thre=0.79):
    attr = f32c(attr)
    w_aff = f32c(w_aff)
    B, P, F_ = attr.shape
    smax = cls_idx.shape[1]
    out = torch.zeros((B, smax, P), dtype=torch.float32, device=attr.device)
    ws = _ws(lib().excel_refine_workspace_bytes(B, P, smax), attr.device)
    check(lib().excel_refine_cams_with_aff(_p(attr), _p(w_aff), _p(cls_idx, torch.int32), _p(ncls, torch.int32), B, g, F_, smax,
                                           float(caa_thre), _p(out), _p(ws, torch.uint8), _stream()), "excel_refine_cams_with_aff")
    return out


def _out(out, shape, dtype, device, zero=False):
    if out is not None:
        if tuple(out.shape) != tuple(shape) or out.dtype != dtype or not out.is_contiguous():
            raise ValueError(f"out= must be a contiguous {dtype} tensor of shape {tuple(shape)}, got {out.dtype} {tuple(out.shape)}")
        return out
    return (torch.zeros if zero else torch.empty)(shape, dtype=dtype, device=device)


def cam_upsample_bkg(refined, ncls, g, H, W, out=None, zero_unused=True):
    refined = f32c(refined)
    B, smax, P = refined.shape
    cams = _out(out, (B, smax + 1, H, W), torch.float32, refined.device)
    ws = _ws(B * smax * P * 4, refined.device)
    check(lib().excel_cam_upsample_bkg(_p(refined), _p(ncls, torch.int32), B, g, smax, H, W, _p(cams), _p(ws, torch.uint8),
                                       1 if zero_unused else 0, _stream()), "excel_cam_upsample_bkg")
    return cams


def par_forward(imgs, masks, dilations=PAR_DILATIONS, num_iter=20, nchan=None, w1=0.3, w2=0.01, stream_affinities=False, out=None, ws=None):
    imgs = f32c(imgs)
    masks = f32c(masks)
    B, Cmax, H, W = masks.shape
    assert imgs.shape[0] == B and imgs.shape[1] == 3
    h, w = imgs.shape[-2:]
    out = _out(out, masks.shape, torch.float32, masks.device, zero=nchan is not None)
    dil = (C.c_int32 * len(dilations))(*dilations)
    need = lib().excel_par_workspace_bytes(B, Cmax, H, W, len(dilations))
    if ws is None or ws.numel() < need:
        ws = _ws(need, masks.device)
    check(lib().excel_par_forward(_p(imgs), h, w, _p(masks), _p(nchan, torch.int32), B, Cmax, H, W, dil, len(dilations), num_iter,
                                  w1, w2, _p(out), _p(ws, torch.uint8), 1 if stream_affinities else 0, _stream()), "excel_par_forward")
    return out


class RaggedPlan:

    def __init__(self, hw, device):
        import numpy as np
        hw = np.ascontiguousarray(np.asarray(hw, np.int32).reshape(-1, 2))
        self.hw = hw
        self.B = int(hw.shape[0])
        self.info = _lib.RaggedInfo()
        ptr = hw.ctypes.data_as(C.POINTER(C.c_int32))
        check(lib().excel_ragged_plan(ptr, self.B, C.byref(self.info), None), "excel_ragged_plan")
        table = np.empty(int(self.info.table_ints), np.int32)
        check(lib().excel_ragged_plan(ptr, self.B, C.byref(self.info), table.ctypes.data_as(C.POINTER(C.c_int32))), "excel_ragged_plan")
        self.table_host = table
        rec = table[:8 * (self.B + 1)].reshape(self.B + 1, 8)
        self.poff = rec[:, 2].astype(np.int64)
        self.loff = rec[:, 4].astype(np.int64)
        self.total_pix = int(self.info.total_pix)
        self.total_label_pix = int(self.info.total_label_pix)
        self.total_tiles = int(self.info.total_tiles)
        self.table = torch.from_numpy(table).to(device, non_blocking=True) if device is not None else None

    def planes(self, packed, b, K):
        H, W = int(self.hw[b, 0]), int(self.hw[b, 1])
        Wp = (W + 3) // 4 * 4
        o = K * int(self.poff[b])
        return packed[o:o + K * H * Wp].view(K, H, Wp)[:, :, :W]

    def label(self, packed_u8, b):
        H, W = int(self.hw[b, 0]), int(self.hw[b, 1])
        o = int(self.loff[b])
        return packed_u8[o:o + H * W].view(H, W)


def normalize_resize_u8_ragged(hwc_packed, plan, S, mean=(123.675, 116.28, 103.53), std=(58.395, 57.12, 57.375), out=None):
    if hwc_packed.dtype != torch.uint8 or hwc_packed.numel() != 3 * plan.total_label_pix:
        raise ValueError(f"hwc_packed must hold {3 * plan.total_label_pix} uint8 values")
    out = _out(out, (plan.B, 3, S, S), torch.float32, hwc_packed.device)
    m, s = (C.c_double * 3)(*mean), (C.c_double * 3)(*std)
    check(lib().excel_normalize_resize_u8_ragged(_p(hwc_packed, torch.uint8), _p(plan.table, torch.int32), plan.B, S, m, s, _p(out), _stream()),
          "excel_normalize_resize_u8_ragged")
    return out


def normalize_resize_u8_ragged_mirror(hwc_packed, plan, S, mean=(123.675, 116.28, 103.53), std=(58.395, 57.12, 57.375), out=None):
    if hwc_packed.dtype != torch.uint8 or hwc_packed.numel() != 3 * plan.total_label_pix:
        raise ValueError(f"hwc_packed must hold {3 * plan.total_label_pix} uint8 values")
    out = _out(out, (2 * plan.B, 3, S, S), torch.float32, hwc_packed.device)
    m, s = (C.c_double * 3)(*mean), (C.c_double * 3)(*std)
    check(lib().excel_normalize_resize_u8_ragged_mirror(_p(hwc_packed, torch.uint8), _p(plan.table, torch.int32), plan.B, S, m, s, _p(out),
                                                        _stream()), "excel_normalize_resize_u8_ragged_mirror")
    return out


CAM_OVERLAY_MODES = {"max": 0, "per_class": 1}
_CAM_TABLES = {}


def cam_overlay_tables(alpha, device, mean=(123.675, 116.28, 103.53), std=(58.395, 57.12, 57.375)):
    key = (float(alpha), tuple(mean), tuple(std), str(device))
    t = _CAM_TABLES.get(key)
    if t is None:
        from .utils import imutils
        t = _CAM_TABLES[key] = torch.from_numpy(imutils.cam_overlay_tables(alpha, mean, std)).to(device)
    return t


def _pinned_upload(a, dtype, device):
    import numpy as np
    h = torch.from_numpy(np.ascontiguousarray(a)).to(dtype).pin_memory()
    return h.to(device, non_blocking=True)


def cam_overlay_ragged(hwc_packed, cams, plan, Cmax, ncls, mode="max", alpha=None, mean=(123.675, 116.28, 103.53),
                       std=(58.395, 57.12, 57.375)):
    import numpy as np
    if mode not in CAM_OVERLAY_MODES:
        raise ValueError(f"mode must be one of {sorted(CAM_OVERLAY_MODES)}, got {mode!r}")
    if alpha is None:
        alpha = 0.5 if mode == "max" else 0.6
    ncls = np.asarray(ncls, np.int64).reshape(-1)
    if ncls.shape[0] != plan.B or (ncls < 0).any() or (ncls > Cmax - 1).any():
        raise ValueError(f"ncls: need {plan.B} values in [0, Cmax - 1 = {Cmax - 1}], got {ncls.tolist()}")
    if hwc_packed.dtype != torch.uint8 or hwc_packed.numel() != 3 * plan.total_label_pix:
        raise ValueError(f"hwc_packed must hold {3 * plan.total_label_pix} uint8 values")
    if cams.numel() < Cmax * plan.total_pix:
        raise ValueError(f"cams must hold Cmax * total_pix = {Cmax * plan.total_pix} floats, got {cams.numel()}")
    dev = hwc_packed.device
    hw = plan.hw.astype(np.int64)
    if mode == "max":
        off = 3 * plan.loff[:plan.B]
        nbytes = 3 * plan.total_label_pix
    else:
        sizes = 3 * ncls * hw[:, 0] * hw[:, 1]
        off = np.concatenate([[0], np.cumsum(sizes)])[:plan.B]
        nbytes = int(sizes.sum())
    out = torch.empty(max(int(nbytes), 1), dtype=torch.uint8, device=dev)[:int(nbytes)]
    if nbytes == 0:
        return out, off
    n_dev = _pinned_upload(ncls, torch.int32, dev)
    off_dev = _pinned_upload(off, torch.int64, dev) if mode == "per_class" else None
    tabs = cam_overlay_tables(alpha, dev, mean, std)
    check(lib().excel_cam_overlay_ragged(_p(hwc_packed, torch.uint8), _p(cams[:Cmax * plan.total_pix]), Cmax, _p(n_dev, torch.int32),
                                         _p(off_dev, torch.int64), _p(plan.table, torch.int32), C.byref(plan.info), CAM_OVERLAY_MODES[mode],
                                         _p(tabs, torch.float64), _p(out, torch.uint8), _stream()), "excel_cam_overlay_ragged")
    return out, off


def cam_overlay(hwc, cams, mode="max", alpha=None, mean=(123.675, 116.28, 103.53), std=(58.395, 57.12, 57.375)):
    if mode not in CAM_OVERLAY_MODES:
        raise ValueError(f"mode must be one of {sorted(CAM_OVERLAY_MODES)}, got {mode!r}")
    if alpha is None:
        alpha = 0.5 if mode == "max" else 0.6
    cams = f32c(cams)
    k, H, W = cams.shape[0] - 1, cams.shape[1], cams.shape[2]
    if hwc.dtype != torch.uint8 or tuple(hwc.shape) != (H, W, 3):
        raise ValueError(f"hwc must be uint8 [{H},{W},3], got {hwc.dtype} {tuple(hwc.shape)}")
    if mode == "max" and k == 0:
        return None
    out = torch.empty((H, W, 3) if mode == "max" else (k, H, W, 3), dtype=torch.uint8, device=cams.device)
    if out.numel() == 0:
        return out
    tabs = cam_overlay_tables(alpha, cams.device, mean, std)
    check(lib().excel_cam_overlay(_p(hwc.contiguous(), torch.uint8), _p(cams), k, H, W, CAM_OVERLAY_MODES[mode], _p(tabs, torch.float64),
                                  _p(out, torch.uint8), _stream()), "excel_cam_overlay")
    return out


TRAIN_PANELS = ("img1", "cam1", "pseu_aff", "pseu_mid", "seg_gt", "seg_pred")
TB_MEAN, TB_STD = (0.485, 0.456, 0.406), (0.229, 0.224, 0.225)
_PANEL_TABLES = {}


def train_panels_plan(B, S, g, panels=TRAIN_PANELS, nrow=2):
    unknown = [n for n in panels if n not in TRAIN_PANELS]
    if unknown:
        raise ValueError(f"unknown panels {unknown}; known: {list(TRAIN_PANELS)}")
    mask = sum(1 << TRAIN_PANELS.index(n) for n in set(panels))
    out = (C.c_int64 * (3 * len(TRAIN_PANELS) + 1))()
    check(lib().excel_train_panels_plan(int(B), int(nrow), int(S), int(g), mask, out), "excel_train_panels_plan")
    plan = {n: (int(out[3 * k]), int(out[3 * k + 1]), int(out[3 * k + 2])) for k, n in enumerate(TRAIN_PANELS) if (mask >> k) & 1}
    return plan, int(out[3 * len(TRAIN_PANELS)])


class TrainPanels(dict):
    buffer = None
    plan = None

    def host(self):
        buf = self.buffer.cpu().numpy()
        return {n: buf[off:off + 3 * Hg * Wg].reshape(Hg, Wg, 3) for n, (Hg, Wg, off) in self.plan.items()}

# ... 104 lines not shown
    if ws is None:
        ws = _ws(ws_need, dev)
    table = torch.empty((plan.B, 2), dtype=torch.int64, device=dev)
    check(lib().excel_png_encode_labels_ragged(_p(labels_flat.contiguous().view(-1), torch.uint8), _p(plan.table, torch.int32), C.byref(plan.info),
                                               hw.ctypes.data_as(C.POINTER(C.c_int32)), _p(_png_palette(palette, dev), torch.uint8),
                                               _p(out, torch.uint8), out.numel(), _p(table, torch.int64), _p(ws, torch.uint8), ws.numel(),
                                               _stream()), "excel_png_encode_labels_ragged")
    return out[:need], table


JPEG_HEADER_BYTES = 623


def _jpeg_items(items):
    import numpy as np
    it = np.asarray(items, np.int64).reshape(-1, 3)
    if it.shape[0] < 1:
        raise ValueError("jpeg_encode_rgb_ragged needs at least one image")
    return np.ascontiguousarray(it[:, 0]), np.ascontiguousarray(it[:, 1:].astype(np.int32))


def jpeg_rgb_arena_bytes(hw):
    import numpy as np
    hw = np.ascontiguousarray(np.asarray(hw, np.int32).reshape(-1, 2))
    return int(lib().excel_jpeg_rgb_arena_bytes(hw.ctypes.data_as(C.POINTER(C.c_int32)), hw.shape[0]))


def jpeg_rgb_workspace_bytes(hw):
    import numpy as np
    hw = np.ascontiguousarray(np.asarray(hw, np.int32).reshape(-1, 2))
    return int(lib().excel_jpeg_rgb_workspace_bytes(hw.ctypes.data_as(C.POINTER(C.c_int32)), hw.shape[0]))


def jpeg_encode_rgb_ragged(rgb_flat, items, quality=75, out=None, ws=None):
    off, hw = _jpeg_items(items)
    if rgb_flat.dtype != torch.uint8 or rgb_flat.dim() != 1 or not rgb_flat.is_contiguous():
        raise ValueError("rgb_flat must be a flat contiguous uint8 tensor")
    ends = off + 3 * hw[:, 0].astype("int64") * hw[:, 1].astype("int64")
    if (off < 0).any() or int(ends.max()) > rgb_flat.numel():
        raise ValueError(f"items reach byte {int(ends.max())} of a buffer of {rgb_flat.numel()} bytes (or hold a negative offset)")
    dev = rgb_flat.device
    n = int(hw.shape[0])
    hw_p, off_p = hw.ctypes.data_as(C.POINTER(C.c_int32)), off.ctypes.data_as(C.POINTER(C.c_int64))
    if out is None:
        out = torch.empty(max(int(lib().excel_jpeg_rgb_arena_bytes(hw_p, n)), 1), dtype=torch.uint8, device=dev)
    elif out.dtype != torch.uint8 or out.dim() != 1 or not out.is_contiguous():
        raise ValueError("out= must be a flat contiguous uint8 tensor")
    if ws is None:
        ws = _ws(max(int(lib().excel_jpeg_rgb_workspace_bytes(hw_p, n)), 1), dev)
    table = torch.empty((n, 2), dtype=torch.int64, device=dev)
    check(lib().excel_jpeg_encode_rgb_ragged(_p(rgb_flat, torch.uint8), off_p, hw_p, n, int(quality), _p(out, torch.uint8), out.numel(),
                                             _p(table, torch.int64), _p(ws, torch.uint8), ws.numel(), _stream()), "excel_jpeg_encode_rgb_ragged")
    return out, table


AUG_CANDIDATES = 10
AUG_PARAMS_DTYPE = None


def aug_params_dtype():
    import numpy as np
    global AUG_PARAMS_DTYPE
    if AUG_PARAMS_DTYPE is None:
        AUG_PARAMS_DTYPE = np.dtype([("ratio", "<f8"), ("flip", "<i4"), ("h_pad", "<i4"), ("w_pad", "<i4"),
                                     ("cand_h", "<i4", (AUG_CANDIDATES,)), ("cand_w", "<i4", (AUG_CANDIDATES,))], align=True)
        assert AUG_PARAMS_DTYPE.itemsize == C.sizeof(_lib.AugParams)
    return AUG_PARAMS_DTYPE


class TrainAugPlan:

    def __init__(self, hw, params, S, device):
        import numpy as np
        hw = np.ascontiguousarray(np.asarray(hw, np.int32).reshape(-1, 2))
        params = np.ascontiguousarray(params, dtype=aug_params_dtype())
        if params.shape != (hw.shape[0],):
            raise ValueError(f"params: {params.shape[0] if params.ndim else 0} records for {hw.shape[0]} images")
        self.B, self.S = int(hw.shape[0]), int(S)
        self.hw, self.params = hw, params
        self.info = _lib.TrainAugInfo()
        hp = hw.ctypes.data_as(C.POINTER(C.c_int32))
        pp = params.ctypes.data_as(C.POINTER(_lib.AugParams))
        check(lib().excel_train_aug_plan(hp, pp, self.B, self.S, C.byref(self.info), None), "excel_train_aug_plan")
        table = np.empty(int(self.info.table_ints), np.int32)
        check(lib().excel_train_aug_plan(hp, pp, self.B, self.S, C.byref(self.info), table.ctypes.data_as(C.POINTER(C.c_int32))),
              "excel_train_aug_plan")
        self.table_host = table
        self.workspace_bytes = int(lib().excel_train_augment_workspace_bytes(C.byref(self.info)))
        self.table = None
        if device is not None:
            self.table = torch.from_numpy(table).pin_memory().to(device, non_blocking=True)


def train_augment(images_u8, plan, labels_u8, params, crop_size, mean=(123.675, 116.28, 103.53), std=(58.395, 57.12, 57.375),
                  aug_plan=None):
    S = int(crop_size)
    if S <= 0:
        raise ValueError("crop_size must be positive")
    dev = images_u8.device
    if aug_plan is None:
        aug_plan = TrainAugPlan(plan.hw, params, S, dev)
    if aug_plan.S != S or aug_plan.B != plan.B or aug_plan.table is None:
        raise ValueError("aug_plan was built for another batch / crop size, or without a device table")
    n = int(aug_plan.info.total_label_pix)
    if images_u8.dtype != torch.uint8 or images_u8.numel() != 3 * n:
        raise ValueError(f"images_u8 must hold {3 * n} uint8 values")
    if labels_u8.dtype != torch.uint8 or labels_u8.numel() != n:
        raise ValueError(f"labels_u8 must hold {n} uint8 values")
    B = plan.B
    img = torch.empty((B, 3, S, S), dtype=torch.float32, device=dev)
    label = torch.empty((B, S, S), dtype=torch.uint8, device=dev)
    box = torch.empty((B, 4), dtype=torch.int32, device=dev)
    ws = _ws(aug_plan.workspace_bytes, dev)
    m, s = (C.c_double * 3)(*mean), (C.c_double * 3)(*std)
    check(lib().excel_train_augment(_p(images_u8, torch.uint8), _p(labels_u8, torch.uint8), _p(aug_plan.table, torch.int32),
                                    C.byref(aug_plan.info), m, s, _p(img), _p(label, torch.uint8), _p(box, torch.int32),
                                    _p(ws, torch.uint8), _stream()), "excel_train_augment")
    return img, label, box


def train_augment_image(images_u8, plan, params, crop_size, aug_plan=None, mean=(123.675, 116.28, 103.53), std=(58.395, 57.12, 57.375)):
    S = int(crop_size)
    if S <= 0:
        raise ValueError("crop_size must be positive")
    dev = images_u8.device
    if aug_plan is None:
        aug_plan = TrainAugPlan(plan.hw, params, S, dev)
    if aug_plan.S != S or aug_plan.B != plan.B or aug_plan.table is None:
        raise ValueError("aug_plan was built for another batch / crop size, or without a device table")
    n = int(aug_plan.info.total_label_pix)
    if images_u8.dtype != torch.uint8 or images_u8.numel() != 3 * n:
        raise ValueError(f"images_u8 must hold {3 * n} uint8 values")
    B = plan.B
    img = torch.empty((B, 3, S, S), dtype=torch.float32, device=dev)
    box = torch.empty((B, 4), dtype=torch.int32, device=dev)
    ws = _ws(aug_plan.workspace_bytes, dev)
    m, s = (C.c_double * 3)(*mean), (C.c_double * 3)(*std)
    check(lib().excel_train_augment_image(_p(images_u8, torch.uint8), _p(aug_plan.table, torch.int32), C.byref(aug_plan.info), m, s,
                                          _p(img), _p(box, torch.int32), _p(ws, torch.uint8), _stream()), "excel_train_augment_image")
    return img, box


def cam_upsample_bkg_ragged(refined, ncls, g, plan, out=None, zero_unused=True):
    refined = f32c(refined)
    B, smax, P = refined.shape
    assert B == plan.B
    cams = _out(out, ((smax + 1) * plan.total_pix,), torch.float32, refined.device)
    ws = _ws(B * smax * P * 4, refined.device)
    check(lib().excel_cam_upsample_bkg_ragged(_p(refined), _p(ncls, torch.int32), _p(plan.table, torch.int32), C.byref(plan.info), g, smax,
                                              _p(cams), _p(ws, torch.uint8), 1 if zero_unused else 0, _stream()), "excel_cam_upsample_bkg_ragged")
    return cams


def par_forward_ragged(imgs, masks, plan, Cmax, dilations=PAR_DILATIONS, num_iter=20, nchan=None, w1=0.3, w2=0.01, out=None, ws=None):
    imgs = f32c(imgs)
    assert imgs.shape[0] == plan.B and imgs.shape[1] == 3 and masks.numel() == Cmax * plan.total_pix
    h, w = imgs.shape[-2:]
    out = _out(out, masks.shape, torch.float32, masks.device, zero=True)
    dil = (C.c_int32 * len(dilations))(*dilations)
    need = lib().excel_par_ragged_workspace_bytes(plan.total_pix, Cmax)
    if ws is None or ws.numel() < need:
        ws = _ws(need, masks.device)
    check(lib().excel_par_forward_ragged(_p(imgs), h, w, _p(masks), _p(nchan, torch.int32), _p(plan.table, torch.int32), C.byref(plan.info), Cmax,
                                         dil, len(dilations), num_iter, w1, w2, _p(out), _p(ws, torch.uint8), _stream()), "excel_par_forward_ragged")
    return out


def argmax_label_ragged(cams, plan, Cmax, nchan=None, cls_idx=None, out=None):
    smax = cls_idx.shape[1] if cls_idx is not None else Cmax - 1
    lab = _out(out, (plan.total_label_pix,), torch.uint8, cams.device)
    check(lib().excel_argmax_label_ragged(_p(cams), _p(nchan, torch.int32), _p(cls_idx, torch.int32), _p(plan.table, torch.int32), C.byref(plan.info),
                                          smax, Cmax, _p(lab, torch.uint8), _stream()), "excel_argmax_label_ragged")
    return lab


def argmax_label(cams, nchan=None, cls_idx=None, want_i64=False):
    cams = f32c(cams)
    B, Cmax, H, W = cams.shape
    smax = cls_idx.shape[1] if cls_idx is not None else Cmax - 1
    l8 = torch.empty((B, H, W), dtype=torch.uint8, device=cams.device)
    l64 = torch.empty((B, H, W), dtype=torch.int64, device=cams.device) if want_i64 else None
    check(lib().excel_argmax_label(_p(cams), _p(nchan, torch.int32), _p(cls_idx, torch.int32), B, smax, Cmax, H * W,
                                   _p(l8, torch.uint8), _p(l64, torch.int64), _stream()), "excel_argmax_label")
    return (l8, l64) if want_i64 else l8


def confusion_accumulate(gt_u8, pred_u8, num_classes, hist=None):
    gt = gt_u8.contiguous().view(-1)
    pr = pred_u8.contiguous().view(-1)
    assert gt.numel() == pr.numel()
    if hist is None:
        hist = torch.zeros((num_classes, num_classes), dtype=torch.int64, device=gt.device)
    check(lib().excel_confusion_accumulate(_p(gt, torch.uint8), _p(pr, torch.uint8), gt.numel(), num_classes,
                                           _p(hist, torch.int64), _stream()), "excel_confusion_accumulate")
    return hist


def nonfinite_count(x, out=None, init=True):
    B = int(x.shape[0])
    if out is None:
        if not init:
            raise ValueError("nonfinite_count: init=False adds to an existing counter: pass out=")
        out = torch.empty((B,), dtype=torch.int32, device=x.device)
    if out.numel() != B:
        raise ValueError(f"nonfinite_count: out holds {out.numel()} counters for {B} images")
    check(lib().excel_nonfinite_count(_p(x), B, x.numel() // B, _p(out, torch.int32), 1 if init else 0, _stream()), "excel_nonfinite_count")
    return out


def confusion_accumulate_masked(gt_u8, pred_u8, num_classes, skip, hist=None, plan=None):
    gt = gt_u8.contiguous()
    pr = pred_u8.contiguous()
    assert gt.numel() == pr.numel()
    B = plan.B if plan is not None else int(gt.shape[0])
    if skip.numel() != B:
        raise ValueError(f"confusion_accumulate_masked: skip holds {skip.numel()} flags for {B} images")
    if plan is not None and gt.numel() != plan.total_label_pix:
        raise ValueError(f"confusion_accumulate_masked: {gt.numel()} pixels, the plan holds {plan.total_label_pix}")
    if hist is None:
        hist = torch.zeros((num_classes, num_classes), dtype=torch.int64, device=gt.device)
    check(lib().excel_confusion_accumulate_masked(_p(gt, torch.uint8), _p(pr, torch.uint8), B, gt.numel() // B,
                                                  _p(plan.table, torch.int32) if plan is not None else None,
                                                  C.byref(plan.info) if plan is not None else None, _p(skip, torch.int32), num_classes,
                                                  _p(hist, torch.int64), _stream()), "excel_confusion_accumulate_masked")
    return hist


def attr_aggregate(text_features, bank, num_fg, topK=0.9):
    text_features = f32c(text_features)
    bank = f32c(bank)
    T, Cc = text_features.shape
    K = bank.shape[1]
    out = torch.empty((Cc, T), dtype=torch.float32, device=text_features.device)
    check(lib().excel_attr_aggregate(_p(text_features), _p(bank), num_fg, T, Cc, K, float(topK), _p(out), _stream()),
          "excel_attr_aggregate")
    return out


def bilinear_resize(x, H, W, align_corners=False):
    x = f32c(x)
    h, w = x.shape[-2:]
    planes = x.numel() // (h * w)
    out = torch.empty(x.shape[:-2] + (H, W), dtype=torch.float32, device=x.device)
    check(lib().excel_bilinear_resize(_p(x), _p(out), planes, h, w, H, W, 1 if align_corners else 0, _stream()),
          "excel_bilinear_resize")
    return out


def pos_embed_resize(pos, g):
    pos = f32c(pos)
    side = int(round((pos.shape[0] - 1) ** 0.5))
    D = pos.shape[1]
    out = torch.empty((g * g + 1, D), dtype=torch.float32, device=pos.device)
    check(lib().excel_pos_embed_resize(_p(pos), side, g, D, _p(out), _stream()), "excel_pos_embed_resize")
    return out


def flip_max_normalize(attr, g):
    attr = f32c(attr)
    B2, P, F_ = attr.shape
    out = torch.empty((B2 // 2, P, F_), dtype=torch.float32, device=attr.device)
    check(lib().excel_flip_max_normalize(_p(attr), _p(out), B2 // 2, g, F_, _stream()), "excel_flip_max_normalize")
    return out


def lam_scale_accumulate(maps, acc, g, H, W, init):
    maps = f32c(maps)
    B2, P, F_ = maps.shape
    if acc is None:
        acc = torch.empty((B2 // 2, F_, H, W), dtype=torch.float32, device=maps.device)
        init = True
    check(lib().excel_lam_scale_accumulate(_p(maps), _p(acc), B2 // 2, g, F_, H, W, 1 if init else 0, _stream()),
          "excel_lam_scale_accumulate")
    return acc


def plane_minmax_normalize_(lam):
    H, W = lam.shape[-2:]
    check(lib().excel_plane_minmax_normalize(_p(lam), lam.numel() // (H * W), H * W, _stream()), "excel_plane_minmax_normalize")
    return lam


TTA_MAX_SCALES = 8
TTA_MAX_GRID = 48


def lam_tta_fuse(maps, grids, g_out, flip, out=None):
    maps = [f32c(m) for m in maps]
    grids = [int(g) for g in grids]
    ns = len(maps)
    if not 1 <= ns <= TTA_MAX_SCALES:
        raise ValueError(f"lam_tta_fuse: {ns} scales, need 1..{TTA_MAX_SCALES}")
    if len(grids) != ns:
        raise ValueError("lam_tta_fuse: one grid size per scale")
    g_out = int(g_out)
    if not 1 <= g_out <= TTA_MAX_GRID:
        raise ValueError(f"lam_tta_fuse: g_out = {g_out} outside [1, {TTA_MAX_GRID}]")
    nb = int(maps[0].shape[0]) if maps[0].dim() == 3 else 0
    F_ = int(maps[0].shape[2]) if maps[0].dim() == 3 else 0
    if flip and nb % 2:
        raise ValueError(f"lam_tta_fuse: flip needs [2B, P, F] maps (image, then mirrored image), got {nb} images")
    B = nb // 2 if flip else nb
    if B < 1 or F_ < 1:
        raise ValueError(f"lam_tta_fuse: need B >= 1 and F >= 1, got maps of shape {tuple(maps[0].shape)}")
    for m, g in zip(maps, grids):
        if not 1 <= g <= TTA_MAX_GRID:
            raise ValueError(f"lam_tta_fuse: grid {g} outside [1, {TTA_MAX_GRID}]")
        if tuple(m.shape) != (nb, g * g, F_):
            raise ValueError(f"lam_tta_fuse: the maps of grid {g} must be [{nb}, {g * g}, {F_}], got {tuple(m.shape)}")
    if out is None:
        out = torch.empty((B, g_out * g_out, F_), dtype=torch.float32, device=maps[0].device)
    elif tuple(out.shape) != (B, g_out * g_out, F_):
        raise ValueError(f"lam_tta_fuse: out must be [{B}, {g_out * g_out}, {F_}], got {tuple(out.shape)}")
    ptrs = (C.c_void_p * ns)(*[_p(m).value for m in maps])
    gs = (C.c_int32 * ns)(*grids)
    check(lib().excel_lam_tta_fuse(ptrs, gs, ns, 1 if flip else 0, B, F_, g_out, _p(out), _stream()), "excel_lam_tta_fuse")
    return out

# ... 178 lines not shown
```

excel_amd/pipeline.py:

```python
import contextlib

import torch

from . import ops

GUARD_MODES = (None, "skip", "observe")
TTA_MAX_SCALES = ops.TTA_MAX_SCALES
TTA_MAX_GRID = ops.TTA_MAX_GRID


def _check_tta_scales(scales):
    scales = [float(s) for s in scales]
    if 1.0 not in scales:
        raise ValueError(f"cam scales {scales}: scale 1.0 must be one of them (it supplies the affinity of the random walk)")
    if len(scales) > TTA_MAX_SCALES:
        raise ValueError(f"cam scales {scales}: {len(scales)} scales, at most {TTA_MAX_SCALES}")
    return scales


def tta_sizes(S, scales):
    scales = _check_tta_scales(scales)
    out, seen = [], {}
    for s in [1.0] + [s for s in scales if s != 1.0] + [1.0] * (scales.count(1.0) - 1):
        S_s = int(S) if s == 1.0 else int(s * S) // 16 * 16
# ... 4 lines not shown
        if S_s in seen:
            raise ValueError(f"cam scale {s}: rounds to the same network size {S_s} as scale {seen[S_s]} at resize size {S}")
        seen[S_s] = s
        out.append((S_s, S_s // 16))
    return out


def _refuse_tta(who, tta_scales, tta_flip):
    if tta_flip or (tta_scales is not None and tuple(float(x) for x in tta_scales) != (1.0,)):
        raise ValueError(f"{who} has no flip / multi-scale fuse (tta_scales={tta_scales}, tta_flip={tta_flip}): the option belongs to the "
                         "training-free regime (TrainingFreePipeline.run_batch / run_batch_ragged)")


class GuardTicket:

    def __init__(self, host, event):
        self._host, self._event = host, event

    def ready(self):
        return self._event.query()

    def flags(self):
        self._event.synchronize()
        return self._host.numpy()


class TrainingFreePipeline:
    def __init__(self, model, num_classes=21, dilations=ops.PAR_DILATIONS, num_iter=20, caa_thre=0.79, smax=6, guard=None,
                 tta_scales=None, tta_flip=False):
        if guard not in GUARD_MODES:
            raise ValueError(f"guard must be one of {GUARD_MODES} (got {guard!r})")
        self.guard = guard
        self.last_flags = self.last_guard = None
        self.tta_flip = bool(tta_flip)
        self.tta_scales = tuple(float(x) for x in tta_scales) if tta_scales is not None else (1.0,)
        self.tta = self.tta_flip or self.tta_scales != (1.0,)
        if self.tta:
            _check_tta_scales(self.tta_scales)
        self.model = model
        self.num_classes = num_classes
        self.dilations = tuple(dilations)
        self.num_iter = num_iter
        self.caa_thre = caa_thre
        self.smax = smax
        self.hist = None
        self._bufs = {}

    @property
    def device(self):
        return torch.device(getattr(self.model, "device", "cuda"))

    def reset(self):
        self.drain()
        self.hist = None

    def _buf(self, name, numel, dtype=torch.float32, device=None):
        key = (name, torch.cuda.current_stream().cuda_stream)
        b = self._bufs.get(key)
        if b is None or b.numel() < numel or b.dtype != dtype:
            self._bufs.pop(key, None)
            b = None
            b = self._bufs[key] = torch.empty(int(numel), dtype=dtype, device=device)
        return b[:int(numel)]

    def _guard_count(self, *tensors):
        if self.guard is None:
            return None
        B = tensors[0].shape[0]
        flags = self._buf("guard", B, torch.int32, tensors[0].device)
        for i, t in enumerate(tensors):
            ops.nonfinite_count(t, out=flags, init=(i == 0))
        host = torch.empty((B,), dtype=torch.int32, pin_memory=True)
        host.copy_(flags, non_blocking=True)
        ev = torch.cuda.Event()
        ev.record()
        self.last_flags, self.last_guard = flags, GuardTicket(host, ev)
        return flags

    def _score(self, gts, labels, flags, plan=None):
        if self.guard == "skip":
            return ops.confusion_accumulate_masked(gts, labels, self.num_classes, flags, self.hist, plan=plan)
        return ops.confusion_accumulate(gts, labels, self.num_classes, self.hist)

    def _no_guard(self, what):
        if self.guard is not None:
            raise ValueError(f"{what} has no overflow guard (guard={self.guard!r}): it is a bench / training path - use run_batch or "
                             "run_batch_ragged, or build the pipeline with guard=None")

    @contextlib.contextmanager
    def exact_mode(self):
        h = self.model.encoder.visual.handle()
        before = h.gemm_mode()
        h.set_gemm_mode("f32")
        try:
            yield self
        finally:
            h.set_gemm_mode(before)

    def _no_tta(self, what):
        if self.tta:
            raise ValueError(f"{what} has no flip / multi-scale fuse (tta_scales={self.tta_scales}, tta_flip={self.tta_flip}): use "
                             "run_batch or run_batch_ragged, or build the pipeline without tta_scales / tta_flip")

    def _tta_uniform_input(self, inputs, S_s):
        x = inputs if S_s == inputs.shape[-1] else ops.bilinear_resize(inputs, S_s, S_s, align_corners=False)
        return torch.cat([x, x.flip(-1)], 0) if self.tta_flip else x

    def _tta_ragged_input(self, hwc_packed, plan, S_s, name):
        nb = plan.B * (2 if self.tta_flip else 1)
        out = self._buf(name, nb * 3 * S_s * S_s, device=hwc_packed.device).view(nb, 3, S_s, S_s)
        if self.tta_flip:
            return ops.normalize_resize_u8_ragged_mirror(hwc_packed, plan, S_s, out=out)
        return ops.normalize_resize_u8_ragged(hwc_packed, plan, S_s, out=out)

    def _tta_maps(self, x, P1):
        n, P_s = x.shape[0], (x.shape[-1] // 16) ** 2
        step = max(1, min(n, n * P1 // P_s))
        if step >= n:
            return self.model.attr_maps(x)
        return torch.cat([self.model.attr_maps(x[lo:lo + step]) for lo in range(0, n, step)], 0)

    def _tta_attr(self, S, make_input):
        g = S // 16
        maps, grids, attn_w = [], [], None
        for S_s, g_s in tta_sizes(S, self.tta_scales):
            x = make_input(S_s)
            B = x.shape[0] // 2 if self.tta_flip else x.shape[0]
            if attn_w is None:
                _, _, m, attn_w, _ = self.model(x[:B])
                if self.tta_flip:
                    m = torch.cat([m, self._tta_maps(x[B:], g * g)], 0)
            else:
                m = self._tta_maps(x, g * g)
            maps.append(m)
            grids.append(g_s)
        return ops.lam_tta_fuse(maps, grids, g, self.tta_flip), attn_w

    @torch.no_grad()
    def run_batch(self, inputs, cls_labels, gts=None, label_hw=None, return_intermediates=False):
        B, _, S, _ = inputs.shape
        g = S // 16
        H, W = (gts.shape[-2:] if gts is not None else (label_hw or (S, S)))
        if self.tta:
            attr, attn_w = self._tta_attr(S, lambda S_s: self._tta_uniform_input(inputs, S_s))
        else:
            _, _, attr, attn_w, _ = self.model(inputs)
        idx, ncls, nchan = ops.cls_compact(cls_labels, self.smax, want_nchan=True)
        refined = ops.refine_cams_with_aff_batched(attr, attn_w.w_aff, idx, ncls, g, self.caa_thre)
        flags = self._guard_count(attr, attn_w.w_aff, refined)
        C = self.smax + 1
        if return_intermediates:
            cams = ops.cam_upsample_bkg(refined, ncls, g, H, W)
            par_out = ops.par_forward(inputs, cams, self.dilations, self.num_iter, nchan=nchan)
        else:
            dev = inputs.device
            cams = ops.cam_upsample_bkg(refined, ncls, g, H, W, out=self._buf("cams", B * C * H * W, device=dev).view(B, C, H, W),
                                        zero_unused=False)
            ws = self._buf("par_ws", ops.lib().excel_par_workspace_bytes(B, C, H, W, len(self.dilations)), torch.uint8, dev)
            par_out = ops.par_forward(inputs, cams, self.dilations, self.num_iter, nchan=nchan, ws=ws,
                                      out=self._buf("par_out", B * C * H * W, device=dev).view(B, C, H, W))
        labels = ops.argmax_label(par_out, nchan, idx)
        if gts is not None:
            self.hist = self._score(gts, labels, flags)
        if return_intermediates:
            return labels, dict(attr=attr, w_aff=attn_w.w_aff, refined=refined, cams=cams, par_out=par_out,
                                cls_idx=idx, ncls=ncls)
        return labels

    @torch.no_grad()
    def run_batch_ragged(self, hwc_packed, plan, cls_labels, gts_packed=None, S=448, return_intermediates=False):
        dev = hwc_packed.device
        B = plan.B
        g = S // 16
        if self.tta:
            first = []

            def make(S_s):
                x = self._tta_ragged_input(hwc_packed, plan, S_s, "inputs" if not first else "tta_inputs")
                first.append(x)
                return x
            attr, attn_w = self._tta_attr(S, make)
            inputs = first[0][:B]
        else:
            inputs = ops.normalize_resize_u8_ragged(hwc_packed, plan, S, out=self._buf("inputs", B * 3 * S * S, device=dev).view(B, 3, S, S))
            _, _, attr, attn_w, _ = self.model(inputs)
        idx, ncls, nchan = ops.cls_compact(cls_labels, self.smax, want_nchan=True)
        refined = ops.refine_cams_with_aff_batched(attr, attn_w.w_aff, idx, ncls, g, self.caa_thre)
        flags = self._guard_count(attr, attn_w.w_aff, refined)
        return self._ragged_back_half(inputs, plan, g, refined, idx, ncls, nchan, gts_packed, return_intermediates,
                                      dict(attr=attr, w_aff=attn_w.w_aff), flags)

    def _ragged_back_half(self, inputs, plan, g, refined, idx, ncls, nchan, gts_packed, return_intermediates, inter, flags=None):
        dev = inputs.device
        C = self.smax + 1
        keep = return_intermediates
        cams = ops.cam_upsample_bkg_ragged(refined, ncls, g, plan, zero_unused=keep,
                                           out=None if keep else self._buf("cams", C * plan.total_pix, device=dev))
        self.last_cams = cams
        self.last_nchan, self.last_cls_idx = nchan, idx
        ws = self._buf("par_ws", ops.lib().excel_par_ragged_workspace_bytes(plan.total_pix, C), torch.uint8, dev)
        par_out = ops.par_forward_ragged(inputs, cams, plan, C, self.dilations, self.num_iter, nchan=nchan, ws=ws,
                                         out=None if keep else self._buf("par_out", C * plan.total_pix, device=dev))
        labels = ops.argmax_label_ragged(par_out, plan, C, nchan, idx)
        if gts_packed is not None:
            self.hist = self._score(gts_packed, labels, flags, plan=plan)
        if return_intermediates:
            return labels, dict(inputs=inputs.clone(), refined=refined, cams=cams, par_out=par_out, cls_idx=idx, ncls=ncls, **inter)
        return labels

    @torch.no_grad()
    def run_batch_split(self, inputs, cls_labels, gts=None, label_hw=None, nsplit=2):
        self._no_guard("run_batch_split")
        self._no_tta("run_batch_split")
        B, _, S, _ = inputs.shape
        nsplit = max(1, min(nsplit, B))
        if nsplit == 1:
            return self.run_batch(inputs, cls_labels, gts, label_hw)
        if len(getattr(self, "_sub", ())) != nsplit:
            self._sub = [dict(stream=torch.cuda.Stream(), hist=None) for _ in range(nsplit)]
        cur = torch.cuda.current_stream()
        H, W = (gts.shape[-2:] if gts is not None else (label_hw or (S, S)))
        labels = torch.empty((B, H, W), dtype=torch.uint8, device=inputs.device)
        step = -(-B // nsplit)
        for i, sub in enumerate(self._sub):
            lo, hi = i * step, min(B, (i + 1) * step)
            if lo >= hi:
                continue
            st = sub["stream"]
            st.wait_stream(cur)
            with torch.cuda.stream(st):
                for t in (inputs, cls_labels, labels) + ((gts,) if gts is not None else ()):
                    t.record_stream(st)
                main_hist, self.hist = self.hist, sub["hist"]
                try:
                    part = self.run_batch(inputs[lo:hi], cls_labels[lo:hi], None if gts is None else gts[lo:hi], (H, W))
                    sub["hist"] = self.hist
                finally:
                    self.hist = main_hist
                labels[lo:hi].copy_(part)
        return labels

    def _streams(self):
        if not hasattr(self, "_sa"):
            self._sa = torch.cuda.Stream()
            self._sb = torch.cuda.Stream()
            self._sb_done = None
        return self._sa, self._sb

    @torch.no_grad()
    def run_batch_overlapped(self, inputs, cls_labels, gts=None, label_hw=None):
        self._no_guard("run_batch_overlapped")
        self._no_tta("run_batch_overlapped")
        sa, sb = self._streams()
        cur = torch.cuda.current_stream()
        B, _, S, _ = inputs.shape
        g = S // 16
        H, W = (gts.shape[-2:] if gts is not None else (label_hw or (S, S)))
        sa.wait_stream(cur)
        with torch.cuda.stream(sa):
            inputs.record_stream(sa)
            cls_labels.record_stream(sa)
            _, _, attr, attn_w, _ = self.model(inputs)
            idx, ncls, nchan = ops.cls_compact(cls_labels, self.smax, want_nchan=True)
            refined = ops.refine_cams_with_aff_batched(attr, attn_w.w_aff, idx, ncls, g, self.caa_thre)
            cams = ops.cam_upsample_bkg(refined, ncls, g, H, W)
            ready = torch.cuda.Event()
            ready.record(sa)
        with torch.cuda.stream(sb):
            sb.wait_event(ready)
            for t in (cams, nchan, idx, inputs) + ((gts,) if gts is not None else ()):
                t.record_stream(sb)
            par_out = ops.par_forward(inputs, cams, self.dilations, self.num_iter, nchan=nchan)
            labels = ops.argmax_label(par_out, nchan, idx)
            if gts is not None:
                self.hist = ops.confusion_accumulate(gts, labels, self.num_classes, self.hist)
        return labels

    def drain(self):
        cur = torch.cuda.current_stream()
        if hasattr(self, "_sa"):
            cur.wait_stream(self._sa)
            cur.wait_stream(self._sb)
        for sub in getattr(self, "_sub", ()):
            cur.wait_stream(sub["stream"])
            if sub["hist"] is not None:
                self.hist = sub["hist"] if self.hist is None else self.hist + sub["hist"]
                sub["hist"] = None


class OptimisedLamPipeline(TrainingFreePipeline):

    def __init__(self, model, num_classes=21, dilations=ops.PAR_DILATIONS, num_iter=20, caa_thre=0.79, smax=6, attn_layers=6, guard=None,
                 tta_scales=None, tta_flip=False):
        _refuse_tta("OptimisedLamPipeline", tta_scales, tta_flip)
        if getattr(model, "_dec", None) is None:
            raise ValueError("OptimisedLamPipeline needs the trained decoder head: build ExCEL_model(..., decoder_state_dict=) "
                             "(--training_free false --model_path)")
        super().__init__(model, num_classes=num_classes, dilations=dilations, num_iter=num_iter, caa_thre=caa_thre, smax=smax, guard=guard)
        self.attn_layers = attn_layers

    def _tower(self, imgs, n_attn_out=0):
        return self.model.encoder.encode_image(imgs, True, None, want_w_aff=True, aff_layers=6, n_attn_out=n_attn_out, want_feats=True,
                                               feats_as_reference=True, want_raw=True, want_features=False)

    @torch.no_grad()
    def run_batch_ragged(self, hwc_packed, plan, cls_labels, gts_packed=None, S=448, return_intermediates=False):
        dev = hwc_packed.device
        B = plan.B
        g = S // 16
        model = self.model
        dec = model._dec
        inputs2 = ops.normalize_resize_u8_ragged_mirror(hwc_packed, plan, S,
                                                        out=self._buf("inputs2", 2 * B * 3 * S * S, device=dev).view(2 * B, 3, S, S))
        inputs = inputs2[:B]
        r = self._tower(inputs, n_attn_out=6)
        fts_x, _ = dec.forward(r["feats"], want_seg=False)
        attn_pred = ops.feature_affinity_grouped(fts_x, "sigmoid", group=1)
        w_aff = ops.attn_select_mean(r["attn"], attn_pred, self.attn_layers)
        del r
        r = self._tower(inputs2[B:])
        fts_f, _ = dec.forward(r["feats"], want_seg=False)
        del r
        ex_feats = torch.cat([fts_x, fts_f], 0)
        del fts_f
        ex_attn = ops.feature_affinity_grouped(ex_feats, "mask_softmax", group=2, member_stride=B)
        del ex_feats
        h = model.encoder.visual.handle()
        r = h.forward(inputs2, want_w_aff=False, want_raw=True, want_features=False, ex_attn=ex_attn)
        del ex_attn
        maps = ops.patch_text_cam(r["x_raw"], model._text_rows, num_fg=model.num_classes - 1, mode=h.gemm_mode())[1]
        del r
        attr = ops.flip_max_normalize(maps, g)
        del maps
        idx, ncls, nchan = ops.cls_compact(cls_labels, self.smax, want_nchan=True)
        refined = ops.refine_cams_with_aff_batched(attr, w_aff, idx, ncls, g, self.caa_thre)
        flags = self._guard_count(attr, w_aff, refined)
        return self._ragged_back_half(inputs, plan, g, refined, idx, ncls, nchan, gts_packed, return_intermediates,
                                      dict(attr=attr, w_aff=w_aff, attn_pred=attn_pred), flags)


class ValidationPipeline(TrainingFreePipeline):

    def __init__(self, model, num_classes=21, dilations=ops.PAR_DILATIONS, num_iter=20, caa_thre=0.75, smax=6, attn_layers=6, guard=None,
                 tta_scales=None, tta_flip=False):
        _refuse_tta("ValidationPipeline", tta_scales, tta_flip)
        if getattr(model, "_dec", None) is None:
            raise ValueError("ValidationPipeline needs the decoder head: build ExCEL_model(..., decoder_state_dict=)")
        if guard is not None:
            raise ValueError(f"ValidationPipeline has no overflow guard (guard={guard!r}): the in-training validation pass scores two "
                             "histograms per step and is out of the guard's scope")
        super().__init__(model, num_classes=num_classes, dilations=dilations, num_iter=num_iter, caa_thre=caa_thre, smax=smax)
        self.attn_layers = attn_layers
        self.hist_seg = None

    def reset(self):
        super().reset()
        self.hist_seg = None

    @torch.no_grad()
    def run_batch_ragged(self, hwc_packed, plan, cls_labels, gts_packed=None, S=320, return_intermediates=False):
        dev = hwc_packed.device
        B = plan.B
        g = S // 16
        model = self.model
        h = model.encoder.visual.handle()
        inputs = ops.normalize_resize_u8_ragged(hwc_packed, plan, S, out=self._buf("inputs", B * 3 * S * S, device=dev).view(B, 3, S, S))
        r = model.encoder.encode_image(inputs, True, None, want_w_aff=True, aff_layers=6, n_attn_out=6, want_feats=True,
                                       feats_as_reference=True, want_raw=True, want_features=False)
        attr = ops.patch_text_cam(r["x_raw"], model._text_rows, num_fg=model.num_classes - 1, mode=h.gemm_mode())[1]
        fts, seg = model._dec.forward(r["feats"])
        attn_pred = ops.feature_affinity_grouped(fts, "sigmoid", group=1)
        del fts
        w_aff = ops.attn_select_mean(r["attn"], attn_pred, self.attn_layers)
        del r
        seg_labels = ops.seg_resize_argmax_uniform(seg, plan)
        if gts_packed is not None:
            self.hist_seg = ops.confusion_accumulate(gts_packed, seg_labels, self.num_classes, self.hist_seg)
        idx, ncls, nchan = ops.cls_compact(cls_labels, self.smax, want_nchan=True)
        refined = ops.refine_cams_with_aff_batched(attr, w_aff, idx, ncls, g, self.caa_thre)
        return self._ragged_back_half(inputs, plan, g, refined, idx, ncls, nchan, gts_packed, return_intermediates,
                                      dict(attr=attr, w_aff=w_aff, attn_pred=attn_pred, seg=seg, seg_labels=seg_labels))
```

include/excel_hip.h:

```cpp
#ifndef EXCEL_HIP_H
#define EXCEL_HIP_H
#include <stddef.h>
#include <stdint.h>

#ifdef __cplusplus
extern "C" {
#endif

const char* excel_last_error(void);
int excel_abi_version(void);
const char* excel_build_id(void);


int excel_gemm_f32(const float* A, const float* Bm, float* C, const float* bias, const float* residual,
                   int M, int N, int K, int lda, int ldb, int ldc, int ldr, int b_kmajor, int act,
                   int batch, long long sA, long long sB, long long sC, long long sR, void* stream);

int excel_split_bf16(const float* in, void* out, long long rows, int K, void* stream);
int excel_gemm_bf16x3(const void* A_split, const void* W_split, float* C, const float* bias, const float* residual,
                      int M, int N, int K, int act, int split_out, void* stream);
int excel_split_f16(const float* in, void* out, long long rows, int K, void* stream);
int excel_gemm_f16x3(const void* A_split, const void* W_split, float* C, const float* bias, const float* residual,
                     int M, int N, int K, int act, int split_out, void* stream);
int excel_pack_f16(const float* in, void* out, long long rows, int K, unsigned long long* inexact_dev, void* stream);
// ... 8 lines not shown
int excel_layernorm(const float* x, const float* w, const float* b, float* y, int rows, int D, float eps, void* stream);


typedef struct {
    int width, layers, heads, patch, out_dim;
    int n_surgery;
    int pos_grid;
} excel_vit_config;

typedef struct {
    const float *ln1_w, *ln1_b;
    const float *in_proj_w, *in_proj_b;
    const float *out_proj_w, *out_proj_b;
    const float *ln2_w, *ln2_b;
    const float *fc1_w, *fc1_b;
    const float *fc2_w, *fc2_b;
} excel_vit_block_weights;

typedef struct {
    const float* conv1_w;
    const float* class_emb;
    const float* pos_emb;
    const float *ln_pre_w, *ln_pre_b, *ln_post_w, *ln_post_b;
    const float* proj;
    const excel_vit_block_weights* blocks;
} excel_vit_weights;

typedef struct excel_vit* excel_vit_t;

int excel_vit_create(const excel_vit_config* cfg, const excel_vit_weights* w, excel_vit_t* out);
void excel_vit_destroy(excel_vit_t h);

int excel_vit_set_gemm_mode(excel_vit_t h, int mode);
int excel_vit_get_gemm_mode(excel_vit_t h);
int excel_vit_weights_fp16_exact(excel_vit_t h);

size_t excel_vit_workspace_bytes(excel_vit_t h, int B, int S);

int excel_vit_forward(excel_vit_t h, const float* img, int B, int S, void* workspace, size_t workspace_bytes,
                      float* image_features, float* x_raw, float* w_aff, int aff_layers,
                      float* attn_out, int n_attn_out, float* feats_out, void* stream);

#define EXCEL_VIT_FEATS_AS_REFERENCE 1
int excel_vit_forward_ex(excel_vit_t h, const float* img, int B, int S, void* workspace, size_t workspace_bytes,
                         float* image_features, float* x_raw, float* w_aff, int aff_layers,
                         float* attn_out, int n_attn_out, float* feats_out, const float* ex_attn, int flags, void* stream);

size_t excel_feature_affinity_workspace_bytes(int B, int C, int P);
int excel_feature_affinity(const float* feats, int B, int C, int P, float beta, float gamma, int mode, float* out,
                           void* workspace, void* stream);

size_t excel_feature_affinity_grouped_workspace_bytes(int B, int C, int P, int group);
int excel_feature_affinity_grouped(const float* feats, int B, int C, int P, int group, int member_stride, float beta, float gamma,
                                   int mode, float* out, void* workspace, void* stream);

typedef struct excel_decoder* excel_decoder_t;
typedef struct { int vit_layers, vit_width, embed, dec_layers, heads, num_classes; } excel_decoder_config;
typedef struct { const float *proj_w, *proj_b, *proj2_w, *proj2_b; } excel_fuse_layer_weights;
typedef struct {
    const float *ln1_w, *ln1_b, *in_proj_w, *in_proj_b, *out_proj_w, *out_proj_b, *ln2_w, *ln2_b, *fc1_w, *fc1_b, *fc2_w, *fc2_b;
} excel_decoder_block_weights;
typedef struct {
    const excel_fuse_layer_weights* fuse;
    const float *fuse_w, *fuse_b;
    const excel_decoder_block_weights* blocks;
    const float *pred_w, *pred_b;
} excel_decoder_weights;
int excel_decoder_create(const excel_decoder_config* cfg, const excel_decoder_weights* w, excel_decoder_t* out);
void excel_decoder_destroy(excel_decoder_t h);
size_t excel_decoder_workspace_bytes(excel_decoder_t h, int B, int g);
int excel_decoder_forward(excel_decoder_t h, const float* all_feats, int B, int g, void* workspace, size_t workspace_bytes,
                          float* attn_fts_out, float* seg_out, void* stream);

typedef struct excel_text* excel_text_t;
typedef struct { int vocab_size, context_length, width, layers, heads, embed_dim; } excel_text_config;
typedef struct {
    const float *token_embedding, *positional_embedding, *ln_final_w, *ln_final_b, *text_projection;
    const excel_decoder_block_weights* blocks;
} excel_text_weights;
int excel_text_create(const excel_text_config* cfg, const excel_text_weights* w, excel_text_t* out);
void excel_text_destroy(excel_text_t h);
size_t excel_text_workspace_bytes(excel_text_t h, int B);
int excel_text_encode(excel_text_t h, const int32_t* tokens, int B, float* out, void* workspace, size_t workspace_bytes, void* stream);
int excel_prompt_ensemble(const float* emb, int n, int E, float* out, void* stream);

size_t excel_train_losses_workspace_bytes(int B, int nc, int H, int W);
int excel_train_losses(const float* seg, const float* attn_pred, const unsigned char* pseudo, const unsigned char* aff_labels, int B, int nc,
                       int g_h, int g_w, int H, int W, int radius, int ignore_index, float w_seg, float w_diver, float* losses,
                       float* d_seg, float* d_attn_pred, void* workspace, void* stream);

size_t excel_decoder_train_workspace_bytes(excel_decoder_t h, int B, int g);
int excel_decoder_forward_train(excel_decoder_t h, const float* all_feats, int B, int g, void* workspace, size_t workspace_bytes,
                                float* seg_out, float* attn_pred_out, float dropout_p, unsigned dropout_seed, void* stream);
int excel_decoder_train_attn_fts(excel_decoder_t h, int B, int g, const void* workspace, size_t workspace_bytes, float* attn_fts_out,
                                 void* stream);
int excel_decoder_backward(excel_decoder_t h, const float* all_feats, int B, int g, void* workspace, size_t workspace_bytes,
                           const float* d_seg, const float* d_attn_pred, const excel_decoder_weights* grads, float dropout_p,
                           unsigned dropout_seed, void* stream);
int excel_adamw_step(float* param, const float* grad, float* exp_avg, float* exp_avg_sq, long long n, float lr, float beta1, float beta2,
                     float eps, float weight_decay, int step, void* stream);

int excel_lam_to_label(const float* cam, const float* cls_label, const int32_t* img_box, int B, int F, int H, int W, float bkg_thre,
                       float high_thre, float low_thre, int ignore_mid, int ignore_index, float* valid_cam, unsigned char* label,
                       void* stream);

int excel_normalize_img_u8(const unsigned char* hwc, int B, int H, int W, const double* mean3, const double* std3, float* out, void* stream);

int excel_denormalize_img(const float* img, int B, int H, int W, const float* mean3, const float* std3, unsigned char* out_u8,
                          float* out_f32, void* stream);

int excel_seg_scale_accumulate(const float* segs, float* acc, int B, int nc, int h, int w, int H, int W, int flip_mean, int init,
                               float scale, void* stream);


size_t excel_cam_workspace_bytes(int B, int N, int T);
int excel_clip_feature_surgery(const float* image_features, const float* text, int B, int N, int C, int T, int F,
                               float temperature, float* out_full, float* out_slice, void* workspace, void* stream);

size_t excel_patch_text_cam_workspace_bytes(int B, int N, int C, int T);
int excel_patch_text_cam(const float* x_raw, const float* text, int B, int N, int C, int T, int F, float temperature, int mode,
                         float* out_full, float* out_slice, float* image_features, void* workspace, void* stream);


size_t excel_dcrf_workspace_bytes(int H, int W, int C);
int excel_dcrf_inference(const unsigned char* rgb_hwc, const float* prob, int prob_is_energy, int H, int W, int C, int iters, float pos_w,
                         float pos_xy_std, float bi_w, float bi_xy_std, float bi_rgb_std, float* q_out, void* workspace, void* stream);



int excel_attn_layer_mean(const float* attn, int Lw, int B, int N, int first_layer, int n_layers, float* w_aff, void* stream);

size_t excel_attn_select_workspace_bytes(int B, int n_layers);
int excel_attn_select_mean(const float* attn, int Lw, int B, int N, int first_layer, int n_layers, const float* seg_attn,
                           float* w_out, void* workspace, void* stream);

size_t excel_trans_mat_workspace_bytes(int B, int P);
int excel_compute_trans_mat(const float* w_aff, int B, int P, float* trans_out, void* workspace, void* stream);

int excel_cls_compact(const float* onehot, int B, int F, int Smax, int32_t* cls_idx, int32_t* ncls, int32_t* nchan, void* stream);

int excel_scoremap_box_mask(const float* attr, const int32_t* cls_idx, const int32_t* ncls, int B, int g, int F, int Smax,
                            double caa_thre, float* v_out, uint8_t* mask_out, void* stream);

size_t excel_refine_workspace_bytes(int B, int P, int Smax);
int excel_refine_cams_with_aff(const float* attr, const float* w_aff, const int32_t* cls_idx, const int32_t* ncls,
                               int B, int g, int F, int Smax, double caa_thre, float* refined, void* workspace, void* stream);

#define EXCEL_CAMS_ZERO_UNUSED 1
int excel_cam_upsample_bkg(const float* refined, const int32_t* ncls, int B, int g, int Smax, int H, int W, float* cams,
                           void* workspace, int flags, void* stream);


#define EXCEL_PAR_STREAM_AFFINITIES 1
size_t excel_par_workspace_bytes(int B, int Cmax, int H, int W, int ndil);
int excel_par_forward(const float* imgs, int h, int w, const float* masks, const int32_t* nchan, int B, int Cmax, int H, int W,
                      const int32_t* dilations , int ndil, int n_iter, float w1, float w2, float* out,
                      void* workspace, int flags, void* stream);

int excel_argmax_label(const float* cams, const int32_t* nchan, const int32_t* cls_idx, int B, int Smax, int Cmax,
                       long long HW, uint8_t* labels_u8, int64_t* labels_i64, void* stream);

int excel_confusion_accumulate(const uint8_t* gt, const uint8_t* pred, long long n, int num_classes, int64_t* hist, void* stream);

typedef struct {
    int32_t B, total_tiles;
    int64_t total_pix;
    int64_t total_label_pix;
    int64_t max_plane_pix;
    int64_t table_ints;
} excel_ragged_info;
int excel_ragged_plan(const int32_t* hw , int B, excel_ragged_info* info , int32_t* table );

int excel_nonfinite_count(const float* x, int B, long long per_image, int32_t* count , int init, void* stream);

int excel_confusion_accumulate_masked(const uint8_t* gt, const uint8_t* pred, int B, long long per_image, const int32_t* table,
                                      const excel_ragged_info* info, const int32_t* skip , int num_classes, int64_t* hist,
                                      void* stream);

int excel_normalize_resize_u8_ragged(const uint8_t* hwc, const int32_t* table, int B, int S, const double* mean3 ,
                                     const double* std3 , float* out, void* stream);

int excel_normalize_resize_u8_ragged_mirror(const uint8_t* hwc, const int32_t* table, int B, int S, const double* mean3 ,
                                            const double* std3 , float* out, void* stream);

int excel_cam_upsample_bkg_ragged(const float* refined, const int32_t* ncls, const int32_t* table, const excel_ragged_info* info, int g,
                                  int Smax, float* cams, void* workspace, int flags, void* stream);

size_t excel_par_ragged_workspace_bytes(long long total_pix, int Cmax);
int excel_par_forward_ragged(const float* imgs, int h, int w, const float* masks, const int32_t* nchan, const int32_t* table,
                             const excel_ragged_info* info, int Cmax, const int32_t* dilations , int ndil, int n_iter, float w1,
                             float w2, float* out, void* workspace, void* stream);

int excel_argmax_label_ragged(const float* cams, const int32_t* nchan, const int32_t* cls_idx, const int32_t* table,
                              const excel_ragged_info* info, int Smax, int Cmax, uint8_t* labels_u8, void* stream);

int excel_seg_msc_fuse_ragged(const float* const* segs , const int32_t* g , const int32_t* flip_mean ,
                              int ns, int nc, const int32_t* table, const excel_ragged_info* info, float* planes, uint8_t* labels_u8,
                              void* stream);

int excel_seg_resize_argmax_ragged(const float* planes, const int32_t* src_table, const excel_ragged_info* src_info, const int32_t* dst_table,
                                   const excel_ragged_info* dst_info, int nc, uint8_t* labels_u8, void* stream);

int excel_seg_resize_argmax_uniform(const float* segs, int B, int h, int w, int nc, const int32_t* dst_table, const excel_ragged_info* dst_info,
                                    uint8_t* labels_u8, void* stream);

int excel_seg_softmax_resize(const float* planes, int h, int w, int nc, int H, int W, float* prob, void* stream);

int excel_seg_softmax_resize_ragged(const float* planes, const int32_t* src_table, const excel_ragged_info* src_info, const int32_t* dst_table,
                                    const excel_ragged_info* dst_info, int nc, float* prob, void* stream);

int excel_dcrf_ragged_workspace_bytes(long long total_label_pix, int C, size_t* bytes );
int excel_dcrf_inference_ragged(const uint8_t* hwc, const float* unary, int unary_is_energy, const int32_t* table,
                                const excel_ragged_info* info, int C, int iters, float pos_w, float pos_xy_std, float bi_w,
                                float bi_xy_std, float bi_rgb_std, uint8_t* labels_u8, float* q_out, void* workspace, void* stream);

int excel_dcrf_lam_ragged_workspace_bytes(const int32_t* hw , const int32_t* nchan , int B, size_t* bytes );
int excel_dcrf_lam_ragged(const uint8_t* hwc, const float* cams, const int32_t* nchan , const int32_t* nchan_host ,
                          const int32_t* cls_idx , const int32_t* table, const excel_ragged_info* info, int smax,
                          int Cmax, int iters, float pos_w, float pos_xy_std, float bi_w, float bi_xy_std, float bi_rgb_std,
                          uint8_t* labels_u8, float* q_out, void* workspace, void* stream);

#define EXCEL_CAM_OVERLAY_MAX 0
#define EXCEL_CAM_OVERLAY_PER_CLASS 1
int excel_cam_overlay_ragged(const uint8_t* hwc, const float* cams, int Cmax, const int32_t* ncls, const int64_t* out_off,
                             const int32_t* table, const excel_ragged_info* info, int mode, const double* tables, uint8_t* out, void* stream);
int excel_cam_overlay(const uint8_t* hwc, const float* cams, int k, int H, int W, int mode, const double* tables, uint8_t* out, void* stream);

#define EXCEL_TRAIN_PANELS 6
#define EXCEL_TRAIN_PANEL_IMG1 0
#define EXCEL_TRAIN_PANEL_CAM1 1
#define EXCEL_TRAIN_PANEL_PSEU_AFF 2
#define EXCEL_TRAIN_PANEL_PSEU_MID 3
#define EXCEL_TRAIN_PANEL_SEG_GT 4
#define EXCEL_TRAIN_PANEL_SEG_PRED 5
#define EXCEL_TRAIN_PANELS_PLAN_INTS (3 * EXCEL_TRAIN_PANELS + 1)
int excel_train_panels_plan(int B, int nrow, int S, int g, int panel_mask, int64_t* out );
int excel_train_panels(const float* img, const float* attr, const float* cls_label, const uint8_t* pseu_aff, const uint8_t* pseu_mid,
                       const uint8_t* seg_gt, const uint8_t* seg_pred, int B, int F, int P, int g, int S, int nrow, int panel_mask,
                       const float* mean , const float* std , const double* jet, const uint8_t* palette, uint8_t* out,
                       size_t out_bytes, void* stream);

size_t excel_png_labels_bound_bytes(int H, int W);
size_t excel_png_labels_workspace_bytes(int B, int max_h);
int excel_png_encode_labels_ragged(const uint8_t* labels, const int32_t* table, const excel_ragged_info* info, const int32_t* hw ,
                                   const uint8_t* palette, uint8_t* arena, size_t arena_bytes, int64_t* out_table, void* workspace,
                                   size_t workspace_bytes, void* stream);

size_t excel_jpeg_rgb_arena_bytes(const int32_t* hw , int n);
size_t excel_jpeg_rgb_workspace_bytes(const int32_t* hw , int n);
int excel_jpeg_encode_rgb_ragged(const uint8_t* rgb, const int64_t* off , const int32_t* hw , int n, int quality, uint8_t* arena,
                                 size_t arena_bytes, int64_t* out_table, void* workspace, size_t workspace_bytes, void* stream);

#define EXCEL_AUG_CANDIDATES 10
typedef struct {
    double ratio;
    int32_t flip;
    int32_t h_pad, w_pad;
    int32_t cand_h[EXCEL_AUG_CANDIDATES];
    int32_t cand_w[EXCEL_AUG_CANDIDATES];
} excel_aug_params;
typedef struct {
    int32_t B, S, max_h, max_w2;
    int64_t table_ints;
    int64_t workspace_bytes;
    int64_t total_label_pix;
} excel_train_aug_info;
#define EXCEL_AUG_REC 40
int excel_train_aug_plan(const int32_t* hw , const excel_aug_params* params , int B, int S,
                         excel_train_aug_info* info , int32_t* table );
size_t excel_train_augment_workspace_bytes(const excel_train_aug_info* info);
int excel_train_augment(const uint8_t* hwc, const uint8_t* labels, const int32_t* table, const excel_train_aug_info* info,
                        const double* mean3 , const double* std3 , float* img, uint8_t* label, int32_t* img_box,
                        void* workspace, void* stream);
int excel_train_augment_image(const uint8_t* hwc, const int32_t* table, const excel_train_aug_info* info, const double* mean3 ,
                              const double* std3 , float* img, int32_t* img_box, void* workspace, void* stream);


int excel_attr_aggregate(const float* text, const float* bank, int F, int T, int C, int K, double topK, float* out, void* stream);

int excel_bilinear_resize(const float* in, float* out, long long planes, int h, int w, int H, int W, int align_corners, void* stream);

int excel_pos_embed_resize(const float* pos, int side, int g, int D, float* out, void* stream);

int excel_flip_max_normalize(const float* attr, float* out, int B, int g, int F, void* stream);

int excel_lam_scale_accumulate(const float* maps, float* acc, int B, int g, int F, int H, int W, int init, void* stream);
int excel_plane_minmax_normalize(float* lam, long long planes, long long HW, void* stream);

int excel_lam_tta_fuse(const float* const* maps , const int32_t* g , int ns, int flip, int B, int F, int g_out,
                       float* out , void* stream);


int excel_prof_enable(int on);
int excel_prof_set_mask(unsigned long long category_mask);
int excel_prof_set_sampling(int every);
int excel_prof_num_categories(void);
const char* excel_prof_category_name(int cat);
int excel_prof_collect(double* ms , long long* launches , double* work );

#ifdef __cplusplus
}
#endif
#endif
```

Measured before the change: 1520.

## Fuse PAR affinity stats into first iteration and argmax labels into last

The first Jacobi iteration of the guided PAR kernel now computes and writes the affinity statistics itself, so the separate affinity launch is gone. The last iteration computes the argmax labels directly, optionally skipping the final plane writes. The pipeline calls the new labels entry points instead of running par_forward followed by argmax_label. This removes two kernel launches and a full pass over the stats and output planes, at the cost of a more complex kernel with extra template variants and register pressure.

After: 1522, median of 6. Within noise of the previous version (+0.1%).

```diff
diff --git a/excel_amd/_lib.py b/excel_amd/_lib.py
--- a/excel_amd/_lib.py
+++ b/excel_amd/_lib.py
@@ -140,6 +140,8 @@
     "excel_par_workspace_bytes": (c_sz, [c_i, c_i, c_i, c_i, c_i]),
     "excel_par_forward": (c_i, [c_f, c_i, c_i, c_f, c_f, c_i, c_i, c_i, c_i, C.POINTER(C.c_int32), c_i, c_i,
                                 C.c_float, C.c_float, c_f, c_f, c_i, c_f]),
+    "excel_par_forward_labels": (c_i, [c_f, c_i, c_i, c_f, c_f, c_f, c_i, c_i, c_i, c_i, c_i, C.POINTER(C.c_int32), c_i, c_i,
+                                       C.c_float, C.c_float, c_f, c_f, c_f, c_i, c_f]),
     "excel_ragged_plan": (c_i, [C.POINTER(C.c_int32), c_i, C.POINTER(RaggedInfo), C.POINTER(C.c_int32)]),
     "excel_normalize_resize_u8_ragged": (c_i, [c_f, c_f, c_i, c_i, C.POINTER(C.c_double), C.POINTER(C.c_double), c_f, c_f]),
     "excel_normalize_resize_u8_ragged_mirror": (c_i, [c_f, c_f, c_i, c_i, C.POINTER(C.c_double), C.POINTER(C.c_double), c_f, c_f]),
@@ -147,6 +149,8 @@
     "excel_par_ragged_workspace_bytes": (c_sz, [c_ll, c_i]),
     "excel_par_forward_ragged": (c_i, [c_f, c_i, c_i, c_f, c_f, c_f, C.POINTER(RaggedInfo), c_i, C.POINTER(C.c_int32), c_i, c_i,
                                        C.c_float, C.c_float, c_f, c_f, c_f]),
+    "excel_par_forward_ragged_labels": (c_i, [c_f, c_i, c_i, c_f, c_f, c_f, c_f, C.POINTER(RaggedInfo), c_i, c_i, C.POINTER(C.c_int32), c_i, c_i,
+                                              C.c_float, C.c_float, c_f, c_f, c_f, c_i, c_f]),
     "excel_argmax_label_ragged": (c_i, [c_f, c_f, c_f, c_f, C.POINTER(RaggedInfo), c_i, c_i, c_f, c_f]),
     "excel_seg_msc_fuse_ragged": (c_i, [C.POINTER(C.c_void_p), C.POINTER(C.c_int32), C.POINTER(C.c_int32), c_i, c_i, c_f, C.POINTER(RaggedInfo),
                                         c_f, c_f, c_f]),
diff --git a/excel_amd/csrc/abi.hip b/excel_amd/csrc/abi.hip
--- a/excel_amd/csrc/abi.hip
+++ b/excel_amd/csrc/abi.hip
@@ -756,15 +756,15 @@
     const float* cur = masks;
     for (int it = 0; it < n_iter; ++it) {
         float* dst = (((n_iter - 1 - it) & 1) == 0) ? out : pp;
-        TRY(step(cur, dst));
+        TRY(step(cur, dst, it));
         cur = dst;
     }
     return EXCEL_OK;
 }
 
-extern "C" int excel_par_forward(const float* imgs, int h, int w, const float* masks, const int32_t* nchan, int B, int Cmax, int H,
-                                 int W, const int32_t* dilations, int ndil, int n_iter, float w1, float w2, float* out,
-                                 void* workspace, int flags, void* stream) {
+static int par_forward_impl(const float* imgs, int h, int w, const float* masks, const int32_t* nchan, const int32_t* cls_idx, int B, int Smax,
+                            int Cmax, int H, int W, const int32_t* dilations, int ndil, int n_iter, float w1, float w2, float* out,
+                            uint8_t* labels_u8, void* workspace, int flags, void* stream) {
     EXCEL_CHECK_ARG(imgs && masks && out && workspace && dilations, "par_forward: null argument");
     EXCEL_CHECK_ARG(n_iter >= 0 && ndil >= 1 && ndil <= 8, "par_forward: bad n_iter/ndil");
     EXCEL_CHECK_ARG(B > 0 && Cmax > 0 && H > 0 && W > 0 && h > 0 && w > 0, "par_forward: bad shape");
@@ -782,18 +782,39 @@
     const TileGeo geo = uniform_geo(B, H, W);
     const bool recompute = !(flags & EXCEL_PAR_STREAM_AFFINITIES) && n_iter > 0 && (W % 4) == 0 && (((uintptr_t)pp & 15) == 0) &&
                            excel_par_guide_supported(gimg, aff, masks, out, Cmax, (long long)hw, W, dilations, ndil);
-    TRY(excel_launch_par_affinity(gimg, aff, geo, 0, dilations, ndil, w1, w2, st, recompute ? 1 : 0));
+    const bool fused = recompute && !(flags & EXCEL_PAR_SEPARATE_STATS);
+    if (!fused) TRY(excel_launch_par_affinity(gimg, aff, geo, 0, dilations, ndil, w1, w2, st, recompute ? 1 : 0));
     if (n_iter == 0) {
         hipMemcpyAsync(out, masks, sizeof(float) * (size_t)B * Cmax * hw, hipMemcpyDeviceToDevice, st);
-        return EXCEL_OK;
-    }
-    if (recompute)
-        return par_jacobi(masks, out, pp, n_iter, [&](const float* cur, float* dst) {
-            return excel_launch_par_iterate_guide(gimg, aff, cur, dst, nchan, Cmax, geo, 0, dilations, ndil, w1, w2, st);
+    } else if (recompute) {
+        const int planes = (labels_u8 && (flags & EXCEL_PAR_NO_PLANES)) ? 0 : 1;
+        return par_jacobi(masks, out, pp, n_iter, [&](const float* cur, float* dst, int it) {
+            const bool last = it == n_iter - 1;
+            return excel_launch_par_iterate_guide(gimg, aff, cur, dst, nchan, Cmax, geo, 0, dilations, ndil, w1, w2, st, fused && it == 0,
+                                                  last ? labels_u8 : nullptr, cls_idx, Smax, planes);
         });
-    return par_jacobi(masks, out, pp, n_iter, [&](const float* cur, float* dst) {
-        return excel_launch_par_iterate(aff, cur, dst, nchan, B, Cmax, H, W, dilations, ndil, st);
-    });
+    } else {
+        TRY(par_jacobi(masks, out, pp, n_iter, [&](const float* cur, float* dst, int) {
+            return excel_launch_par_iterate(aff, cur, dst, nchan, B, Cmax, H, W, dilations, ndil, st);
+        }));
+    }
+    if (labels_u8) return excel_launch_argmax_label(out, nchan, cls_idx, B, Smax, Cmax, (long long)hw, labels_u8, nullptr, st);
+    return EXCEL_OK;
+}
+
+extern "C" int excel_par_forward(const float* imgs, int h, int w, const float* masks, const int32_t* nchan, int B, int Cmax, int H,
+                                 int W, const int32_t* dilations, int ndil, int n_iter, float w1, float w2, float* out,
+                                 void* workspace, int flags, void* stream) {
+    return par_forward_impl(imgs, h, w, masks, nchan, nullptr, B, 0, Cmax, H, W, dilations, ndil, n_iter, w1, w2, out, nullptr, workspace,
+                            flags & (EXCEL_PAR_STREAM_AFFINITIES | EXCEL_PAR_SEPARATE_STATS), stream);
+}
+
+extern "C" int excel_par_forward_labels(const float* imgs, int h, int w, const float* masks, const int32_t* nchan, const int32_t* cls_idx,
+                                        int B, int Smax, int Cmax, int H, int W, const int32_t* dilations, int ndil, int n_iter, float w1,
+                                        float w2, float* out, uint8_t* labels_u8, void* workspace, int flags, void* stream) {
+    EXCEL_CHECK_ARG(!labels_u8 || !cls_idx || Smax >= Cmax - 1, "par_forward_labels: cls_idx rows must hold Cmax - 1 classes");
+    return par_forward_impl(imgs, h, w, masks, nchan, cls_idx, B, Smax, Cmax, H, W, dilations, ndil, n_iter, w1, w2, out, labels_u8, workspace,
+                            flags, stream);
 }
 
 extern "C" size_t excel_par_ragged_workspace_bytes(long long total_pix, int Cmax) {
@@ -801,9 +822,9 @@
            align_up((size_t)3 * total_pix * sizeof(float), 256);
 }
 
-extern "C" int excel_par_forward_ragged(const float* imgs, int h, int w, const float* masks, const int32_t* nchan, const int32_t* table,
-                                        const excel_ragged_info* info, int Cmax, const int32_t* dilations, int ndil, int n_iter, float w1,
-                                        float w2, float* out, void* workspace, void* stream) {
+static int par_forward_ragged_impl(const float* imgs, int h, int w, const float* masks, const int32_t* nchan, const int32_t* cls_idx,
+                                   const int32_t* table, const excel_ragged_info* info, int Smax, int Cmax, const int32_t* dilations, int ndil,
+                                   int n_iter, float w1, float w2, float* out, uint8_t* labels_u8, void* workspace, int flags, void* stream) {
     EXCEL_CHECK_ARG(imgs && masks && out && workspace && dilations && table && info, "par_forward_ragged: null argument");
     EXCEL_CHECK_ARG(n_iter >= 1 && Cmax > 0 && h > 0 && w > 0 && info->B > 0, "par_forward_ragged: bad n_iter / shape");
     const size_t tp = (size_t)info->total_pix;
@@ -817,10 +838,30 @@
                     "par_forward_ragged: needs dilations [1,2,4,8,12,24], 16-byte aligned buffers and max(Cmax,5) * H * Wp * 4 < 2^31 per image "
                     "(Wp = W rounded up to 4)");
     TRY(excel_launch_bilinear_ac_ragged(imgs, guide, h, w, geo, info->total_tiles, st));
-    TRY(excel_launch_par_affinity(guide, stats, geo, info->total_tiles, dilations, ndil, w1, w2, st, 1));
-    return par_jacobi(masks, out, pp, n_iter, [&](const float* cur, float* dst) {
-        return excel_launch_par_iterate_guide(guide, stats, cur, dst, nchan, Cmax, geo, info->total_tiles, dilations, ndil, w1, w2, st);
+    const bool fused = !(flags & EXCEL_PAR_SEPARATE_STATS);
+    if (!fused) TRY(excel_launch_par_affinity(guide, stats, geo, info->total_tiles, dilations, ndil, w1, w2, st, 1));
+    const int planes = (labels_u8 && (flags & EXCEL_PAR_NO_PLANES)) ? 0 : 1;
+    return par_jacobi(masks, out, pp, n_iter, [&](const float* cur, float* dst, int it) {
+        const bool last = it == n_iter - 1;
+        return excel_launch_par_iterate_guide(guide, stats, cur, dst, nchan, Cmax, geo, info->total_tiles, dilations, ndil, w1, w2, st,
+                                              fused && it == 0, last ? labels_u8 : nullptr, cls_idx, Smax, planes);
     });
+}
+
+extern "C" int excel_par_forward_ragged(const float* imgs, int h, int w, const float* masks, const int32_t* nchan, const int32_t* table,
+                                        const excel_ragged_info* info, int Cmax, const int32_t* dilations, int ndil, int n_iter, float w1,
+                                        float w2, float* out, void* workspace, void* stream) {
+    return par_forward_ragged_impl(imgs, h, w, masks, nchan, nullptr, table, info, 0, Cmax, dilations, ndil, n_iter, w1, w2, out, nullptr,
+                                   workspace, 0, stream);
+}
+
+extern "C" int excel_par_forward_ragged_labels(const float* imgs, int h, int w, const float* masks, const int32_t* nchan, const int32_t* cls_idx,
+                                               const int32_t* table, const excel_ragged_info* info, int Smax, int Cmax,
+                                               const int32_t* dilations, int ndil, int n_iter, float w1, float w2, float* out,
+                                               uint8_t* labels_u8, void* workspace, int flags, void* stream) {
+    EXCEL_CHECK_ARG(!labels_u8 || !cls_idx || Smax >= Cmax - 1, "par_forward_ragged_labels: cls_idx rows must hold Cmax - 1 classes");
+    return par_forward_ragged_impl(imgs, h, w, masks, nchan, cls_idx, table, info, Smax, Cmax, dilations, ndil, n_iter, w1, w2, out, labels_u8,
+                                   workspace, flags & (EXCEL_PAR_SEPARATE_STATS | EXCEL_PAR_NO_PLANES), stream);
 }
 
 extern "C" int excel_argmax_label_ragged(const float* cams, const int32_t* nchan, const int32_t* cls_idx, const int32_t* table,
diff --git a/excel_amd/csrc/excel_internal.h b/excel_amd/csrc/excel_internal.h
--- a/excel_amd/csrc/excel_internal.h
+++ b/excel_amd/csrc/excel_internal.h
@@ -97,8 +97,9 @@
                               hipStream_t st, int compact = 0);
 int excel_par_guide_supported(const void* guide, const void* stats, const void* in, const void* out, int Cmax, long long max_plane, int Wp,
                               const int* dil, int ndil);
-int excel_launch_par_iterate_guide(const float* guide, const float* stats, const float* in, float* out, const int* nchan, int Cmax,
-                                   const TileGeo& geo, int total_tiles, const int* dil, int ndil, float w1, float w2, hipStream_t st);
+int excel_launch_par_iterate_guide(const float* guide, float* stats, const float* in, float* out, const int* nchan, int Cmax,
+                                   const TileGeo& geo, int total_tiles, const int* dil, int ndil, float w1, float w2, hipStream_t st,
+                                   int first = 0, unsigned char* lab8 = nullptr, const int* cls_idx = nullptr, int Smax = 0, int planes = 1);
 int excel_launch_par_iterate(const float* aff, const float* in, float* out, const int* nchan, int B, int Cmax, int H, int W,
                              const int* dil, int ndil, hipStream_t st);
 int excel_launch_bilinear_ac_ragged(const float* in, float* out, int h, int w, const TileGeo& geo, int total_tiles, hipStream_t st);
diff --git a/excel_amd/csrc/par.hip b/excel_amd/csrc/par.hip
--- a/excel_amd/csrc/par.hip
+++ b/excel_amd/csrc/par.hip
@@ -145,11 +145,19 @@
     return v;
 }
 
-template <bool RAGGED>
+struct ParFuse {
+    float* stats_w;
+    float w1;
+    unsigned char* lab8;
+    const int* cls_idx;
+    int Smax, planes;
+};
+template <bool RAGGED, bool FIRST, bool LAB>
 __global__ __launch_bounds__(512, 4) void par_iterate_guide_kernel(const float* __restrict__ guide, const float* __restrict__ stats,
                                                                     const float* __restrict__ in, float* __restrict__ out,
-                                                                    const int* __restrict__ nchan, ParDil dl, int Cmax, TileGeo geo, int dbg) {
-    constexpr int ND = 6, HALO = 24, TR = 16 + 2 * HALO, TP = PG_TP, NG = 3 * ND;
+                                                                    const int* __restrict__ nchan, ParDil dl, int Cmax, TileGeo geo, int dbg,
+                                                                    ParFuse fx) {
+    constexpr int ND = 6, HALO = 24, TR = 16 + 2 * HALO, TP = PG_TP, NG = 3 * ND, NT = 8 * ND;
     __shared__ __attribute__((aligned(1024))) float tile[2 * TR * TP];
     Tile tg;
     if (RAGGED) {
@@ -165,9 +173,10 @@
     }
     const int b = tg.b, x0 = tg.x0, y0 = tg.y0, H = tg.H, W = tg.W, Wp = tg.Wp;
     const long long HW = tg.HW;
-    const int tid = threadIdx.x, lane = tid & 63, tx = tid & 31, ty = tid >> 5;
+    const int tid = threadIdx.x;
+    int lane = tid & 63, tx = tid & 31, ty = tid >> 5;
     const int wave = __builtin_amdgcn_readfirstlane(tid >> 6);
-    const int px = x0 + 2 * tx, py = y0 + ty;
+    int px = x0 + 2 * tx, py = y0 + ty;
     const int nch = nchan ? min(nchan[b], Cmax) : Cmax;
     const long long pix = (long long)min(py, H - 1) * Wp + min(px, Wp - 2);
     const float* st_b = stats + 5 * tg.base + pix;
@@ -175,7 +184,7 @@
     typedef __attribute__((address_space(3))) unsigned char* lds_bptr;
     const __amdgpu_buffer_rsrc_t rs_g = __builtin_amdgcn_make_buffer_rsrc((void*)(guide + 3 * tg.base), 0, (int)(3 * HW * 4), 0x00020000);
     const __amdgpu_buffer_rsrc_t rs_m = __builtin_amdgcn_make_buffer_rsrc((void*)(in + (long long)Cmax * tg.base), 0, (int)((long long)Cmax * HW * 4), 0x00020000);
-    const int xoffA = min(max(x0 - HALO + lane, 0), W - 1) * 4, xoffB = min(max(x0 - HALO + 64 + lane, 0), W - 1) * 4;
+    int xoffA = min(max(x0 - HALO + lane, 0), W - 1) * 4, xoffB = min(max(x0 - HALO + 64 + lane, 0), W - 1) * 4;
     const unsigned tile_b = lds_addr(tile);
     constexpr int RPW = TR / 8;
 #ifdef PAR_ALL_INTERIOR
@@ -183,7 +192,7 @@
 #else
     const bool interior = x0 - HALO >= 0 && x0 + 64 + HALO <= W;
 #endif
-    const int x4off = min(x0 - HALO + 4 * (lane & 31), Wp - 4) * 4;
+    int x4off = min(x0 - HALO + 4 * (lane & 31), Wp - 4) * 4;
     auto stage = [&](int p, int buf) {
         const bool is_g = p < 3;
         const int plane_off = (is_g ? p : p - 3) * (int)(HW * 4);
@@ -222,7 +231,7 @@
 #pragma unroll
         for (int k = 0; k < 8; ++k) wall[di][k] = f32x2{0.f, 0.f};
 
-    const unsigned org = tile_b + (ty * TP + 2 * tx) * 4;
+    unsigned org = tile_b + (ty * TP + 2 * tx) * 4;
     auto taps = [&](auto depth_c, int buf, auto&& fn, auto&& pin) {
         constexpr int DEPTH = decltype(depth_c)::value, NS = DEPTH + 1;
         unsigned base = org + buf * (TR * TP * 4);
@@ -277,50 +286,126 @@
     };
     const int np = 3 + nch;
     auto stat_load = [&](int plane) -> f32x2 { return *reinterpret_cast<const f32x2*>(st_b + (long long)plane * HW); };
-    f32x2 st_nxt = stat_load(0), st_nx2 = f32x2{0.f, 0.f};
-    __builtin_amdgcn_sched_barrier(0);
-    stage(0, 0);
+    bool valid = px < W && py < H;
+    if constexpr (FIRST) {
+        float* st_px = fx.stats_w + 5 * tg.base + (long long)py * Wp + px;
+        stage(0, 0);
 #pragma unroll 1
-    for (int p = 0; p < 3; ++p) {
-        asm volatile("s_waitcnt vmcnt(0)" : "+v"(st_nxt) :: "memory");
-        __builtin_amdgcn_s_barrier();
-        const f32x2 nk2 = -st_nxt;
-        st_nxt = stat_load(p + 1);
-        if (p == 2) st_nx2 = stat_load(4);
-        f32x2 ctr;
-        asm volatile("ds_read_b64 %0, %1 offset:%2" : "=v"(ctr) : "v"(org + (p & 1) * (TR * TP * 4)), "n"((HALO * TP + HALO) * 4) : "memory");
-        __builtin_amdgcn_sched_barrier(0);
-        stage(p + 1, (p + 1) & 1);
-        asm volatile("s_waitcnt lgkmcnt(0)" : "+v"(ctr) :: "memory");
-        if (EXCEL_DBG(dbg) & 1) continue;
-        f32x2 nctr = -ctr;
-        if (EXCEL_DBG(dbg) & 16) nctr += 1e-30f * far_taps(guide + 3 * tg.base + (long long)p * HW);
-        asm volatile("" : "+v"(nctr));
-        taps(std::integral_constant<int, 1>{}, p & 1, [&](int di, int k, const f32x2 nb) {
-            const f32x2 dv = nb + nctr;
-            wall[di][k] = __builtin_elementwise_fma(dv * dv, nk2, wall[di][k]);
-        }, [] {});
-    }
-    if (!(EXCEL_DBG(dbg) & 2)) {
-        f32x2 nm2 = -st_nxt;
-        asm volatile("" : "+v"(nm2));
-        const f32x2 is2 = st_nx2;
+        for (int p = 0; p < 3; ++p) {
+            asm volatile("s_waitcnt vmcnt(0)" ::: "memory");
+            __builtin_amdgcn_s_barrier();
+            f32x2 ctr;
+            asm volatile("ds_read_b64 %0, %1 offset:%2" : "=v"(ctr) : "v"(org + (p & 1) * (TR * TP * 4)), "n"((HALO * TP + HALO) * 4) : "memory");
+            __builtin_amdgcn_sched_barrier(0);
+            stage(p + 1, (p + 1) & 1);
+            asm volatile("s_waitcnt lgkmcnt(0)" : "+v"(ctr) :: "memory");
+            f32x2 sum = {0.f, 0.f};
+            taps(std::integral_constant<int, 1>{}, p & 1, [&](int, int, const f32x2 nb) { sum += nb; }, [&] { asm volatile("" : "+v"(sum)); });
+            const f32x2 mean = {sum[0] / (float)NT, sum[1] / (float)NT};
+            f32x2 nmean = -mean;
+            asm volatile("" : "+v"(nmean));
+            f32x2 var = {0.f, 0.f};
+            taps(std::integral_constant<int, 1>{}, p & 1, [&](int, int, const f32x2 nb) { const f32x2 dv = nb + nmean; var = __builtin_elementwise_fma(dv, dv, var); },
+                 [&] { asm volatile("" : "+v"(var)); });
+            f32x2 k2;
+#pragma unroll
+            for (int q = 0; q < 2; ++q) {
+                const float den = sqrtf(var[q] / (float)(NT - 1)) + 1e-8f;
+                const float k = 1.f / (den * fx.w1);
+                k2[q] = __fmul_rn(k * k, PAR_LOG2E_3);
+            }
+            if (valid) *reinterpret_cast<f32x2*>(st_px + (long long)p * HW) = k2;
+            f32x2 nk2 = -k2, nctr = -ctr;
+            asm volatile("" : "+v"(nctr));
+            taps(std::integral_constant<int, 1>{}, p & 1, [&](int di, int k, const f32x2 nb) {
+                const f32x2 dv = nb + nctr;
+                wall[di][k] = __builtin_elementwise_fma(dv * dv, nk2, wall[di][k]);
+            }, [] {});
+        }
+        f32x2 m = {-INFINITY, -INFINITY};
 #pragma unroll
         for (int di = 0; di < ND; ++di)
 #pragma unroll
+            for (int k = 0; k < 8; ++k) { m[0] = fmaxf(m[0], wall[di][k][0]); m[1] = fmaxf(m[1], wall[di][k][1]); }
+        f32x2 nm = -m;
+        if (valid) *reinterpret_cast<f32x2*>(st_px + 3 * HW) = m;
+        asm volatile("" : "+v"(nm));
+        f32x2 ssum = {0.f, 0.f};
+#pragma unroll
+        for (int di = 0; di < ND; ++di)
+#pragma unroll
             for (int k = 0; k < 8; ++k) {
-                const f32x2 z = wall[di][k] + nm2;
+                const f32x2 z = wall[di][k] + nm;
+                ssum += f32x2{__builtin_amdgcn_exp2f(z[0]), __builtin_amdgcn_exp2f(z[1])};
+            }
+        f32x2 is2 = {1.f / ssum[0], 1.f / ssum[1]};
+        if (valid) *reinterpret_cast<f32x2*>(st_px + 4 * HW) = is2;
+        asm volatile("" : "+v"(is2), "+v"(nm));
+#pragma unroll
+        for (int di = 0; di < ND; ++di)
+#pragma unroll
+            for (int k = 0; k < 8; ++k) {
+                const f32x2 z = wall[di][k] + nm;
                 const f32x2 e = {__builtin_amdgcn_exp2f(z[0]), __builtin_amdgcn_exp2f(z[1])};
                 const float ps = dl.pos_sm[di * 8 + k];
                 wall[di][k] = __builtin_elementwise_fma(e, is2, f32x2{ps, ps});
             }
-    }
-    const bool valid = px < W && py < H;
+        int t2 = tid;
+        asm volatile("" : "+v"(t2));
+        lane = t2 & 63; tx = t2 & 31; ty = t2 >> 5;
+        px = x0 + 2 * tx; py = y0 + ty;
+        xoffA = min(max(x0 - HALO + lane, 0), W - 1) * 4; xoffB = min(max(x0 - HALO + 64 + lane, 0), W - 1) * 4;
+        x4off = min(x0 - HALO + 4 * (lane & 31), Wp - 4) * 4;
+        org = tile_b + (ty * TP + 2 * tx) * 4;
+        valid = px < W && py < H;
+    } else {
+        f32x2 st_nxt = stat_load(0), st_nx2 = f32x2{0.f, 0.f};
+        __builtin_amdgcn_sched_barrier(0);
+        stage(0, 0);
+#pragma unroll 1
+        for (int p = 0; p < 3; ++p) {
+            asm volatile("s_waitcnt vmcnt(0)" : "+v"(st_nxt) :: "memory");
+            __builtin_amdgcn_s_barrier();
+            const f32x2 nk2 = -st_nxt;
+            st_nxt = stat_load(p + 1);
+            if (p == 2) st_nx2 = stat_load(4);
+            f32x2 ctr;
+            asm volatile("ds_read_b64 %0, %1 offset:%2" : "=v"(ctr) : "v"(org + (p & 1) * (TR * TP * 4)), "n"((HALO * TP + HALO) * 4) : "memory");
+            __builtin_amdgcn_sched_barrier(0);
+            stage(p + 1, (p + 1) & 1);
+            asm volatile("s_waitcnt lgkmcnt(0)" : "+v"(ctr) :: "memory");
+            if (EXCEL_DBG(dbg) & 1) continue;
+            f32x2 nctr = -ctr;
+            if (EXCEL_DBG(dbg) & 16) nctr += 1e-30f * far_taps(guide + 3 * tg.base + (long long)p * HW);
+            asm volatile("" : "+v"(nctr));
+            taps(std::integral_constant<int, 1>{}, p & 1, [&](int di, int k, const f32x2 nb) {
+                const f32x2 dv = nb + nctr;
+                wall[di][k] = __builtin_elementwise_fma(dv * dv, nk2, wall[di][k]);
+            }, [] {});
+        }
+        if (!(EXCEL_DBG(dbg) & 2)) {
+            f32x2 nm2 = -st_nxt;
+            asm volatile("" : "+v"(nm2));
+            const f32x2 is2 = st_nx2;
+#pragma unroll
+            for (int di = 0; di < ND; ++di)
+#pragma unroll
+                for (int k = 0; k < 8; ++k) {
+                    const f32x2 z = wall[di][k] + nm2;
+                    const f32x2 e = {__builtin_amdgcn_exp2f(z[0]), __builtin_amdgcn_exp2f(z[1])};
+                    const float ps = dl.pos_sm[di * 8 + k];
+                    wall[di][k] = __builtin_elementwise_fma(e, is2, f32x2{ps, ps});
+                }
+        }
+    }
     float* out_px = out + (long long)Cmax * tg.base + (long long)py * Wp + px;
 #ifndef PAR_STORE_WAIT
 #define PAR_STORE_WAIT 1
 #endif
-    const bool wstore = PAR_STORE_WAIT && __builtin_amdgcn_ballot_w64(valid) != 0 && !EXCEL_DBG(dbg);
+    const bool wplanes = !LAB || fx.planes;
+    const bool wstore = PAR_STORE_WAIT && wplanes && __builtin_amdgcn_ballot_w64(valid) != 0 && !EXCEL_DBG(dbg);
+    f32x2 best = {0.f, 0.f};
+    int bi0 = 0, bi1 = 0;
     for (int p = 3; p < np; ++p) {
         if (p > 3 && wstore) asm volatile("s_waitcnt vmcnt(1)" ::: "memory");
         else asm volatile("s_waitcnt vmcnt(0)" ::: "memory");
@@ -331,7 +416,21 @@
         if (EXCEL_DBG(dbg) & 16) acc = 1e-30f * far_taps(in + (long long)Cmax * tg.base + (long long)(p - 3) * HW);
         taps(std::integral_constant<int, PAR_MASK_DEPTH>{}, p & 1, [&](int di, int k, const f32x2 nb) { acc = __builtin_elementwise_fma(nb, wall[di][k], acc); },
              [&] { asm volatile("" : "+v"(acc)); });
-        if (valid) *reinterpret_cast<f32x2*>(out_px + (long long)(p - 3) * HW) = acc;
+        if constexpr (LAB) {
+            const int c = p - 3;
+            if (c == 0) best = acc;
+            if (c > 0 && acc[0] > best[0]) { best[0] = acc[0]; bi0 = c; }
+            if (c > 0 && acc[1] > best[1]) { best[1] = acc[1]; bi1 = c; }
+        }
+        if (valid && wplanes) *reinterpret_cast<f32x2*>(out_px + (long long)(p - 3) * HW) = acc;
+    }
+    if constexpr (LAB) {
+        const int* cls_row = fx.cls_idx ? fx.cls_idx + (long long)b * fx.Smax : nullptr;
+        if (py < H) {
+            unsigned char* l = fx.lab8 + tg.lab + (long long)py * W + px;
+            if (px < W) l[0] = (unsigned char)((bi0 == 0) ? 0 : (cls_row ? cls_row[bi0 - 1] + 1 : bi0));
+            if (px + 1 < W) l[1] = (unsigned char)((bi1 == 0) ? 0 : (cls_row ? cls_row[bi1 - 1] + 1 : bi1));
+        }
     }
 }
 
@@ -679,10 +778,11 @@
     return (vec && par_dil_ok(dil, ndil) && planes * max_plane * 4 < (1LL << 31)) ? 1 : 0;
 }
 
-int excel_launch_par_iterate_guide(const float* guide, const float* stats, const float* in, float* out, const int* nchan, int Cmax,
-                                   const TileGeo& geo, int total_tiles, const int* dil, int ndil, float w1, float w2, hipStream_t st) {
+int excel_launch_par_iterate_guide(const float* guide, float* stats, const float* in, float* out, const int* nchan, int Cmax,
+                                   const TileGeo& geo, int total_tiles, const int* dil, int ndil, float w1, float w2, hipStream_t st,
+                                   int first, unsigned char* lab8, const int* cls_idx, int Smax, int planes) {
     EXCEL_CHECK_ARG(par_dil_ok(dil, ndil), "par_iterate_guide: unsupported dilation set");
-    ProfScope prof__(PROF_PAR_ITERATE, st);
+    ProfScope prof__(first ? PROF_PAR_AFFINITY : PROF_PAR_ITERATE, st);
     ParDil dl;
     int rc = make_dil(dil, ndil, w1, w2, &dl);
     if (rc) return rc;
@@ -691,11 +791,20 @@
     static const int env_dbg = getenv("EXCEL_PAR_DBG") ? atoi(getenv("EXCEL_PAR_DBG")) : 0;
     dbg = env_dbg;
 #endif
-    if (geo.tab)
-        hipLaunchKernelGGL((par_iterate_guide_kernel<true>), dim3(total_tiles), dim3(512), 0, st, guide, stats, in, out, nchan, dl, Cmax, geo, dbg);
-    else
-        hipLaunchKernelGGL((par_iterate_guide_kernel<false>), dim3(cdiv(geo.W, 64), cdiv(geo.H, 16), geo.B), dim3(512), 0, st, guide, stats,
-                           in, out, nchan, dl, Cmax, geo, dbg);
+    const ParFuse fx = {stats, w1, lab8, cls_idx, Smax, planes};
+    const dim3 grid = geo.tab ? dim3(total_tiles) : dim3(cdiv(geo.W, 64), cdiv(geo.H, 16), geo.B);
+#define CALL(R, F, L) hipLaunchKernelGGL((par_iterate_guide_kernel<R, F, L>), grid, dim3(512), 0, st, guide, stats, in, out, nchan, dl, Cmax, geo, dbg, fx)
+#define PICK(R)                                   \
+    do {                                          \
+        if (first && lab8) CALL(R, true, true);   \
+        else if (first) CALL(R, true, false);     \
+        else if (lab8) CALL(R, false, true);      \
+        else CALL(R, false, false);               \
+    } while (0)
+    if (geo.tab) PICK(true);
+    else PICK(false);
+#undef PICK
+#undef CALL
     EXCEL_CHECK_LAUNCH("par_iterate_guide");
     return EXCEL_OK;
 }
diff --git a/excel_amd/ops.py b/excel_amd/ops.py
--- a/excel_amd/ops.py
+++ b/excel_amd/ops.py
@@ -724,7 +724,11 @@
     return cams
 
 
-def par_forward(imgs, masks, dilations=PAR_DILATIONS, num_iter=20, nchan=None, w1=0.3, w2=0.01, stream_affinities=False, out=None, ws=None):
+PAR_STREAM_AFFINITIES, PAR_SEPARATE_STATS, PAR_NO_PLANES = 1, 2, 4
+
+
+def par_forward(imgs, masks, dilations=PAR_DILATIONS, num_iter=20, nchan=None, w1=0.3, w2=0.01, stream_affinities=False, out=None, ws=None,
+                labels=False, cls_idx=None, want_planes=True, separate_stats=False):
     imgs = f32c(imgs)
     masks = f32c(masks)
     B, Cmax, H, W = masks.shape
@@ -735,9 +739,17 @@
     need = lib().excel_par_workspace_bytes(B, Cmax, H, W, len(dilations))
     if ws is None or ws.numel() < need:
         ws = _ws(need, masks.device)
-    check(lib().excel_par_forward(_p(imgs), h, w, _p(masks), _p(nchan, torch.int32), B, Cmax, H, W, dil, len(dilations), num_iter,
-                                  w1, w2, _p(out), _p(ws, torch.uint8), 1 if stream_affinities else 0, _stream()), "excel_par_forward")
-    return out
+    flags = (PAR_STREAM_AFFINITIES if stream_affinities else 0) | (PAR_SEPARATE_STATS if separate_stats else 0)
+    if labels is False or labels is None:
+        check(lib().excel_par_forward(_p(imgs), h, w, _p(masks), _p(nchan, torch.int32), B, Cmax, H, W, dil, len(dilations), num_iter,
+                                      w1, w2, _p(out), _p(ws, torch.uint8), flags, _stream()), "excel_par_forward")
+        return out
+    smax = cls_idx.shape[1] if cls_idx is not None else Cmax - 1
+    lab = _out(labels if torch.is_tensor(labels) else None, (B, H, W), torch.uint8, masks.device)
+    check(lib().excel_par_forward_labels(_p(imgs), h, w, _p(masks), _p(nchan, torch.int32), _p(cls_idx, torch.int32), B, smax, Cmax, H, W, dil,
+                                         len(dilations), num_iter, w1, w2, _p(out), _p(lab, torch.uint8), _p(ws, torch.uint8),
+                                         flags | (0 if want_planes else PAR_NO_PLANES), _stream()), "excel_par_forward_labels")
+    return (out, lab) if want_planes else lab
 
 
 class RaggedPlan:
@@ -1148,7 +1160,8 @@
     return cams
 
 
-def par_forward_ragged(imgs, masks, plan, Cmax, dilations=PAR_DILATIONS, num_iter=20, nchan=None, w1=0.3, w2=0.01, out=None, ws=None):
+def par_forward_ragged(imgs, masks, plan, Cmax, dilations=PAR_DILATIONS, num_iter=20, nchan=None, w1=0.3, w2=0.01, out=None, ws=None,
+                       labels=False, cls_idx=None, want_planes=True, separate_stats=False):
     imgs = f32c(imgs)
     assert imgs.shape[0] == plan.B and imgs.shape[1] == 3 and masks.numel() == Cmax * plan.total_pix
     h, w = imgs.shape[-2:]
@@ -1157,9 +1170,21 @@
     need = lib().excel_par_ragged_workspace_bytes(plan.total_pix, Cmax)
     if ws is None or ws.numel() < need:
         ws = _ws(need, masks.device)
-    check(lib().excel_par_forward_ragged(_p(imgs), h, w, _p(masks), _p(nchan, torch.int32), _p(plan.table, torch.int32), C.byref(plan.info), Cmax,
-                                         dil, len(dilations), num_iter, w1, w2, _p(out), _p(ws, torch.uint8), _stream()), "excel_par_forward_ragged")
-    return out
+    if (labels is False or labels is None) and not separate_stats:
+        check(lib().excel_par_forward_ragged(_p(imgs), h, w, _p(masks), _p(nchan, torch.int32), _p(plan.table, torch.int32), C.byref(plan.info), Cmax,
+                                             dil, len(dilations), num_iter, w1, w2, _p(out), _p(ws, torch.uint8), _stream()), "excel_par_forward_ragged")
+        return out
+    want_labels = not (labels is False or labels is None)
+    smax = cls_idx.shape[1] if cls_idx is not None else Cmax - 1
+    lab = _out(labels if torch.is_tensor(labels) else None, (plan.total_label_pix,), torch.uint8, masks.device) if want_labels else None
+    flags = (PAR_SEPARATE_STATS if separate_stats else 0) | (0 if want_planes or not want_labels else PAR_NO_PLANES)
+    check(lib().excel_par_forward_ragged_labels(_p(imgs), h, w, _p(masks), _p(nchan, torch.int32), _p(cls_idx, torch.int32),
+                                                _p(plan.table, torch.int32), C.byref(plan.info), smax, Cmax, dil, len(dilations), num_iter, w1, w2,
+                                                _p(out), _p(lab, torch.uint8), _p(ws, torch.uint8), flags, _stream()),
+          "excel_par_forward_ragged_labels")
+    if not want_labels:
+        return out
+    return (out, lab) if want_planes else lab
 
 
 def argmax_label_ragged(cams, plan, Cmax, nchan=None, cls_idx=None, out=None):
diff --git a/excel_amd/pipeline.py b/excel_amd/pipeline.py
--- a/excel_amd/pipeline.py
+++ b/excel_amd/pipeline.py
@@ -180,14 +180,15 @@
         if return_intermediates:
             cams = ops.cam_upsample_bkg(refined, ncls, g, H, W)
             par_out = ops.par_forward(inputs, cams, self.dilations, self.num_iter, nchan=nchan)
+            labels = ops.argmax_label(par_out, nchan, idx)
         else:
             dev = inputs.device
             cams = ops.cam_upsample_bkg(refined, ncls, g, H, W, out=self._buf("cams", B * C * H * W, device=dev).view(B, C, H, W),
                                         zero_unused=False)
             ws = self._buf("par_ws", ops.lib().excel_par_workspace_bytes(B, C, H, W, len(self.dilations)), torch.uint8, dev)
-            par_out = ops.par_forward(inputs, cams, self.dilations, self.num_iter, nchan=nchan, ws=ws,
-                                      out=self._buf("par_out", B * C * H * W, device=dev).view(B, C, H, W))
-        labels = ops.argmax_label(par_out, nchan, idx)
+            labels = ops.par_forward(inputs, cams, self.dilations, self.num_iter, nchan=nchan, ws=ws,
+                                     out=self._buf("par_out", B * C * H * W, device=dev).view(B, C, H, W),
+                                     labels=True, cls_idx=idx, want_planes=False)
         if gts is not None:
             self.hist = self._score(gts, labels, flags)
         if return_intermediates:
@@ -227,9 +228,13 @@
         self.last_cams = cams
         self.last_nchan, self.last_cls_idx = nchan, idx
         ws = self._buf("par_ws", ops.lib().excel_par_ragged_workspace_bytes(plan.total_pix, C), torch.uint8, dev)
-        par_out = ops.par_forward_ragged(inputs, cams, plan, C, self.dilations, self.num_iter, nchan=nchan, ws=ws,
-                                         out=None if keep else self._buf("par_out", C * plan.total_pix, device=dev))
-        labels = ops.argmax_label_ragged(par_out, plan, C, nchan, idx)
+        if keep:
+            par_out = ops.par_forward_ragged(inputs, cams, plan, C, self.dilations, self.num_iter, nchan=nchan, ws=ws)
+            labels = ops.argmax_label_ragged(par_out, plan, C, nchan, idx)
+        else:
+            labels = ops.par_forward_ragged(inputs, cams, plan, C, self.dilations, self.num_iter, nchan=nchan, ws=ws,
+                                            out=self._buf("par_out", C * plan.total_pix, device=dev), labels=True, cls_idx=idx,
+                                            want_planes=False)
         if gts_packed is not None:
             self.hist = self._score(gts_packed, labels, flags, plan=plan)
         if return_intermediates:
@@ -298,8 +303,7 @@
             sb.wait_event(ready)
             for t in (cams, nchan, idx, inputs) + ((gts,) if gts is not None else ()):
                 t.record_stream(sb)
-            par_out = ops.par_forward(inputs, cams, self.dilations, self.num_iter, nchan=nchan)
-            labels = ops.argmax_label(par_out, nchan, idx)
+            labels = ops.par_forward(inputs, cams, self.dilations, self.num_iter, nchan=nchan, labels=True, cls_idx=idx, want_planes=False)
             if gts is not None:
                 self.hist = ops.confusion_accumulate(gts, labels, self.num_classes, self.hist)
         return labels
diff --git a/include/excel_hip.h b/include/excel_hip.h
--- a/include/excel_hip.h
+++ b/include/excel_hip.h
@@ -184,10 +184,16 @@
 
 
 #define EXCEL_PAR_STREAM_AFFINITIES 1
+#define EXCEL_PAR_SEPARATE_STATS 2
+#define EXCEL_PAR_NO_PLANES 4
 size_t excel_par_workspace_bytes(int B, int Cmax, int H, int W, int ndil);
 int excel_par_forward(const float* imgs, int h, int w, const float* masks, const int32_t* nchan, int B, int Cmax, int H, int W,
                       const int32_t* dilations , int ndil, int n_iter, float w1, float w2, float* out,
                       void* workspace, int flags, void* stream);
+
+int excel_par_forward_labels(const float* imgs, int h, int w, const float* masks, const int32_t* nchan, const int32_t* cls_idx, int B,
+                             int Smax, int Cmax, int H, int W, const int32_t* dilations , int ndil, int n_iter, float w1, float w2,
+                             float* out, uint8_t* labels_u8, void* workspace, int flags, void* stream);
 
 int excel_argmax_label(const float* cams, const int32_t* nchan, const int32_t* cls_idx, int B, int Smax, int Cmax,
                        long long HW, uint8_t* labels_u8, int64_t* labels_i64, void* stream);
@@ -222,6 +228,11 @@
 int excel_par_forward_ragged(const float* imgs, int h, int w, const float* masks, const int32_t* nchan, const int32_t* table,
                              const excel_ragged_info* info, int Cmax, const int32_t* dilations , int ndil, int n_iter, float w1,
                              float w2, float* out, void* workspace, void* stream);
+
+int excel_par_forward_ragged_labels(const float* imgs, int h, int w, const float* masks, const int32_t* nchan, const int32_t* cls_idx,
+                                    const int32_t* table, const excel_ragged_info* info, int Smax, int Cmax,
+                                    const int32_t* dilations , int ndil, int n_iter, float w1, float w2, float* out,
+                                    uint8_t* labels_u8, void* workspace, int flags, void* stream);
 
 int excel_argmax_label_ragged(const float* cams, const int32_t* nchan, const int32_t* cls_idx, const int32_t* table,
                               const excel_ragged_info* info, int Smax, int Cmax, uint8_t* labels_u8, void* stream);
```
